# HiromasaYamanishi/furusato_recommend

Measured on AMD Instinct MI355X. Metric: BPR positive-edges/sec (LightGCN-3 d=64, 1000000 x 100000 / 20000000 edges), higher is better.
Workload: dtype f32; 1 GPU; C2: LightGCN 3-layer d=64, synthetic 1000000 users x 100000 items / 20000000 edges (uniform); users=1000000, items=100000, edges=20000000, graph=uniform, dim=64, layers=3, bpr_batch_per_rank=2048, global_batch=2048, ranks=1, parallelism=dp1 (user-sharded, RCCL none gradient exchange)

## Files before the change

### furusato_recommend_amd/_lib.py

```python
from __future__ import annotations

import ctypes
import os
from ctypes import (POINTER, Structure, c_float, c_int, c_int32, c_int64,
                    c_size_t, c_uint64, c_void_p, c_char_p)

import torch

_HERE = os.path.dirname(os.path.abspath(__file__))
LIB_PATH = os.environ.get("MIREC_LIB") or os.path.join(_HERE, "libmirec.so")

MIREC_OK = 0
ERR_WORKSPACE = 4
IN_PRESCALED, IN_RAW, IN_SPARSE, IN_NONE = 0, 1, 2, 3
SUPPORTED_DIMS = (4, 8, 16, 32, 64, 128, 256)


class MirecError(RuntimeError):
    pass


class CSR(Structure):
    _fields_ = [
        ("rowptr", c_void_p), ("col", c_void_p), ("dinv", c_void_p),
        ("n_rows", c_int64), ("nnz", c_int64), ("split", c_int32),
        ("_pad", c_int32), ("n_long", c_int64), ("n_seg", c_int64),
        ("long_rows", c_void_p), ("long_segptr", c_void_p),
        ("seg_row", c_void_p), ("seg_beg", c_void_p),
        ("col_sorted", c_void_p), ("n_sorted", c_int64), ("val", c_void_p),
    ]


class AdamH(Structure):
    _fields_ = [
        ("one_minus_beta1", c_float), ("beta2", c_float),
        ("one_minus_beta2", c_float), ("neg_step_size", c_float),
        ("bc2_sqrt", c_float), ("eps", c_float),
    ]


class Prop(Structure):
    _fields_ = [
        ("dim", c_int32), ("in_mode", c_int32), ("x_in", c_void_p),
        ("slot", c_void_p), ("seed_in", c_void_p), ("seed", c_void_p),
        ("addend", c_void_p), ("seed2", c_void_p), ("divisor", c_float),
        ("_pad", c_float), ("out", c_void_p), ("xs_out", c_void_p),
        ("param", c_void_p), ("exp_avg", c_void_p), ("exp_avg_sq", c_void_p),
        ("adam", AdamH), ("partial", c_void_p), ("row_mask", c_void_p),
        ("in_mask", c_void_p), ("out_mask", c_void_p), ("row_list", c_void_p),
        ("row_count", c_void_p),
        ("row_list_cap", c_int64), ("narrow_max", c_int32), ("_pad2", c_int32),
        ("wide_list", c_void_p), ("wide_count", c_void_p),
        ("scale_src", c_void_p), ("scale_dst", c_void_p), ("scale_next", c_void_p),
    ]


class Drop(Structure):
    _fields_ = [("keep_prob", c_float), ("transposed", c_int32), ("seed", c_uint64)]


class Sweep(Structure):
    _fields_ = [
        ("row0", c_int64), ("n_rows", c_int64), ("n_src", c_int64),
        ("tile_rows", c_int32), ("group_rows", c_int32), ("groups", c_int32),
        ("n_tiles", c_int32), ("band_rows", c_int32), ("_pad", c_int32),
        ("gptr", c_void_p), ("ent", c_void_p),
    ]


class SweepWave(Structure):
    _fields_ = [
        ("row0", c_int64), ("n_rows", c_int64), ("src0", c_int64), ("n_src", c_int64),
        ("n_slots", c_int64),
        ("tile_rows", c_int32), ("wave_rows", c_int32), ("n_tiles", c_int32),
        ("band_rows", c_int32), ("grid", c_int32), ("_pad", c_int32),
        ("wptr", c_void_p), ("slot", c_void_p),
    ]


class SweepPace(Structure):
    _fields_ = [("ws", c_void_p), ("lead_bands", c_int32 * 2), ("every", c_int32 * 2),
                ("nap", c_int32 * 2)]


class RowGradGroup(Structure):
    _fields_ = [
        ("ids", c_void_p), ("grad_out", c_void_p), ("n_targets", c_int64), ("k", c_int32),
        ("mean", c_int32), ("dropout_p", c_float), ("_pad", c_int32), ("seed", c_uint64),
    ]


TABLE_GRAD_MAX_GROUPS = 8


class RowBlock(Structure):
    _fields_ = [("ids", c_void_p), ("rows", c_void_p), ("n", c_int64)]

SIGNATURES = {
    "mirec_strerror": (c_char_p, [c_int]),
    "mirec_abi_version": (c_int, []),
    "mirec_last_hip_error": (c_int, []),
    "mirec_struct_sizes": (c_int, [POINTER(c_size_t), POINTER(c_size_t), POINTER(c_size_t)]),
    "mirec_csr_bipartite": (c_int, [c_void_p, c_void_p, c_int64, c_int64, c_int64,
                                    c_void_p, c_void_p, c_void_p]),
    "mirec_csr_sort_rows": (c_int, [c_void_p, c_void_p, c_int64, c_void_p]),
    "mirec_csr_from_coo": (c_int, [c_void_p, c_void_p, c_int64, c_int64, c_void_p,
                                   c_void_p, c_void_p]),
    "mirec_csr_entry_order": (c_int, [c_void_p, c_int64, c_int64, c_void_p]),
    "mirec_parse_interactions": (c_int, [c_void_p, c_int64, c_int64, c_int32, POINTER(c_int64),
                                         POINTER(c_int64), POINTER(c_int64), POINTER(c_int64),
                                         c_void_p, c_void_p, c_void_p]),
    "mirec_csr_long_rows": (c_int, [c_void_p, c_int64, c_int32, POINTER(c_int64),
                                    POINTER(c_int64), c_void_p, c_void_p, c_void_p,
                                    c_void_p]),
    "mirec_propagate": (c_int, [POINTER(CSR), POINTER(Prop), c_void_p]),
    "mirec_propagate_sweep": (c_int, [POINTER(CSR), POINTER(Prop), POINTER(Sweep), c_void_p]),
    "mirec_sweep_sizeof": (c_size_t, []),
    "mirec_sweep_shape": (c_int, [c_int64, c_int32, c_int32, POINTER(c_int32),
                                  POINTER(c_int32)]),
    "mirec_sweep_build": (c_int, [c_void_p, c_void_p, c_int64, c_int64, c_int64, c_int32,
                                  c_int32, c_void_p, c_void_p]),
    "mirec_sweep_groups": (c_int, [c_int32]),
    "mirec_sweep_wave_sizeof": (c_size_t, []),
    "mirec_sweep_wave_build": (c_int, [c_void_p, c_void_p, c_int64, c_int64, c_int64, c_int64,
                                       c_int32, c_void_p, c_void_p, c_int64, POINTER(c_int64)]),
    "mirec_propagate_sweep_wave": (c_int, [POINTER(CSR), POINTER(Prop), POINTER(SweepWave),
                                           POINTER(SweepWave), c_void_p]),
    "mirec_sweep_pace_sizeof": (c_size_t, []),
    "mirec_sweep_pace_ws_bytes": (c_size_t, []),
    "mirec_propagate_sweep_wave_paced": (c_int, [POINTER(CSR), POINTER(Prop), POINTER(SweepWave),
                                                 POINTER(SweepWave), POINTER(SweepPace),
                                                 c_void_p]),
    "mirec_sweep_wave_stamp": (c_int, [POINTER(CSR), POINTER(Prop), POINTER(SweepWave), c_void_p,
                                       c_int64, c_void_p, c_void_p]),
    "mirec_drop_sizeof": (c_size_t, []),
    "mirec_propagate_drop": (c_int, [POINTER(CSR), POINTER(Prop), POINTER(Drop), c_void_p]),
    "mirec_edge_keep_mask": (c_int, [c_void_p, c_void_p, c_int64, c_uint64, c_float, c_int32,
                                     c_void_p]),
    "mirec_edge_dot": (c_int, [POINTER(CSR), c_void_p, c_void_p, c_int32, c_void_p, c_void_p]),
    "mirec_prescale": (c_int, [c_void_p, c_void_p, c_int64, c_int32, c_void_p, c_void_p]),
    "mirec_shard_pack": (c_int, [c_void_p, c_int64, c_int32, c_int32, c_int32, c_int64, c_int64,
                                 c_void_p, c_void_p]),
    "mirec_shard_unpack": (c_int, [c_void_p, c_int64, c_int32, c_int32, c_int32, c_int64,
                                   c_int64, c_void_p, c_void_p, c_void_p, c_void_p]),
    "mirec_frontier": (c_int, [POINTER(CSR), c_void_p, c_int64, c_void_p, c_void_p, c_void_p,
                               c_int64, c_int64, c_void_p, c_void_p, c_void_p, c_void_p,
                               c_void_p, c_int32, c_void_p]),
    "mirec_mask_compact_pair": (c_int, [c_void_p, c_void_p, c_void_p, c_int64, c_void_p, c_void_p,
                                        c_void_p, c_void_p, c_void_p, c_void_p]),
    "mirec_small_sort_workspace": (c_int, [c_int64, POINTER(c_size_t)]),
    "mirec_small_sort_pairs": (c_int, [c_void_p, c_void_p, c_void_p, c_void_p, c_int64, c_void_p,
                                       c_size_t, c_void_p]),
    "mirec_mask_compact": (c_int, [POINTER(CSR), c_void_p, c_int32, c_void_p, c_void_p,
                                   c_void_p, c_void_p, c_int32, c_void_p]),
    "mirec_distinct_rows_workspace": (c_int64, [c_int64]),
    "mirec_distinct_rows": (c_int, [c_void_p, c_int64, c_int64, c_int64, c_int64, c_void_p,
                                    c_void_p, c_void_p, c_size_t, c_void_p]),
    "mirec_distinct_rows_unseen": (c_int, [c_void_p, c_int64, c_int64, c_int64, c_int64, c_void_p,
                                        c_void_p, c_void_p, c_void_p, c_size_t, c_void_p]),
    "mirec_stamped_rows": (c_int, [c_void_p, c_int64, c_int32, c_int32, c_void_p, c_void_p,
                                   c_void_p, c_size_t, c_void_p]),
    "mirec_scatter_rows": (c_int, [c_void_p, c_void_p, c_int64, c_int32, c_void_p, c_void_p]),
    "mirec_owner_sum_workspace": (c_int64, [c_int32, c_int64]),
    "mirec_owner_sum": (c_int, [POINTER(RowBlock), c_int32, c_int64, c_int64, c_int32, c_void_p,
                                c_size_t, c_void_p, c_void_p]),
    "mirec_gather_rows_counted": (c_int, [c_void_p, c_void_p, c_void_p, c_int64, c_int32,
                                          c_void_p, c_void_p]),
    "mirec_route_pack": (c_int, [c_void_p, c_void_p, c_int64, c_int64, c_int32, c_int32, c_int64,
                                 c_void_p, c_void_p]),
    "mirec_gather_rows_routed": (c_int, [c_void_p, c_int64, c_void_p, c_int32, c_int32, c_int64,
                                         c_int32, c_void_p, c_void_p]),
    "mirec_bpr_forward": (c_int, [c_void_p, c_void_p, c_int64, c_int64, c_int32, c_int64,
                                  c_void_p, c_void_p, c_void_p, c_float, c_void_p, c_void_p,
                                  c_void_p, c_void_p, c_void_p, c_void_p]),
    "mirec_bpr_loss": (c_int, [c_void_p, c_void_p, c_int64, c_float, c_void_p, c_void_p,
                               c_void_p]),
    "mirec_bpr_seed_workspace": (c_int, [c_int64, c_int64, POINTER(c_size_t)]),
    "mirec_bpr_seed": (c_int, [c_void_p, c_void_p, c_int64, c_int64, c_int32, c_int64,
                               c_void_p, c_void_p, c_void_p, c_void_p, c_void_p, c_void_p,
                               c_float, c_float, c_int32, c_void_p, c_void_p, c_void_p,
                               c_void_p, c_void_p, c_size_t, c_void_p]),
    "mirec_bpr_seed_reset": (c_int, [c_void_p, c_void_p, c_int64, c_void_p]),
    "mirec_seed_dense": (c_int, [c_void_p, c_void_p, c_int64, c_void_p, c_void_p, c_void_p,
                                 c_int32, c_void_p, c_int32, c_void_p]),
    "mirec_seed_pack": (c_int, [c_void_p, c_int64, c_int64, c_void_p, c_void_p]),
    "mirec_seed_merge_workspace": (c_int, [c_int64, c_int64, POINTER(c_size_t)]),
    "mirec_seed_merge": (c_int, [c_void_p, c_void_p, c_void_p, c_int64, c_int32, c_int64,
                                 c_void_p, c_void_p, c_void_p, c_void_p, c_void_p, c_size_t,
                                 c_void_p]),
    "mirec_ssm_forward": (c_int, [c_void_p, c_void_p, c_int64, c_int64, c_int32, c_int64, c_int32,
                                  c_void_p, c_void_p, c_void_p, c_float, c_float, c_void_p,
                                  c_void_p, c_void_p, c_void_p, c_void_p, c_void_p, c_void_p,
                                  c_void_p]),
    "mirec_ssm_keys": (c_int, [c_void_p, c_void_p, c_void_p, c_int64, c_int32, c_int64, c_void_p,
                               c_void_p]),
    "mirec_ssm_seed_workspace": (c_int, [c_int64, c_int32, c_int64, POINTER(c_size_t)]),
    "mirec_ssm_seed": (c_int, [c_void_p, c_void_p, c_int64, c_int64, c_int32, c_int64, c_int32,
                               c_void_p, c_void_p, c_void_p, c_void_p, c_void_p, c_void_p,
                               c_float, c_float, c_int32, c_void_p, c_void_p, c_void_p,
                               c_void_p, c_void_p, c_size_t, c_void_p]),
    "mirec_ssm_sample": (c_int, [POINTER(CSR), c_void_p, c_int64, c_int64, c_int64, c_int32,
                                 c_uint64, c_uint64, c_int32, c_int32, c_void_p, c_void_p,
                                 c_void_p, c_void_p, c_void_p]),
    "mirec_cpu_ssm_sample": (c_int, [c_void_p, c_void_p, c_void_p, c_void_p, c_int64, c_int64,
                                     c_int64, c_int32, c_uint64, c_uint64, c_int32, c_int32,
                                     c_void_p, c_void_p, c_void_p, c_void_p, c_int32]),
    "mirec_ssm_shared_keys": (c_int, [c_void_p, c_void_p, c_void_p, c_int64, c_int64, c_int64,
                                      c_void_p, c_void_p]),
    "mirec_ssm_shared_mask": (c_int, [POINTER(CSR), c_void_p, c_int64, c_void_p, c_void_p,
                                      c_int64, c_int64, c_void_p, c_void_p]),
    "mirec_ssm_shared_forward": (c_int, [c_void_p, c_void_p, c_int64, c_int64, c_int32, c_int64,
                                         c_int64, c_void_p, c_void_p, c_void_p, c_void_p, c_float,
                                         c_float, c_void_p, c_void_p, c_void_p, c_void_p,
                                         c_void_p, c_void_p, c_void_p, c_void_p, c_void_p]),
    "mirec_ssm_shared_loss": (c_int, [c_void_p, c_void_p, c_void_p, c_int64, c_int64, c_float,
                                      c_void_p, c_void_p, c_void_p]),
    "mirec_ssm_shared_seed_workspace": (c_int, [c_int64, c_int64, c_int64, POINTER(c_size_t)]),
    "mirec_ssm_shared_seed": (c_int, [c_void_p, c_void_p, c_int64, c_int64, c_int32, c_int64,
                                      c_int64, c_void_p, c_void_p, c_void_p, c_void_p, c_void_p,
                                      c_float, c_float, c_int32, c_void_p, c_void_p, c_void_p,
                                      c_void_p, c_void_p, c_size_t, c_void_p]),
    "mirec_shared_sample": (c_int, [c_int64, c_int64, c_int64, c_uint64, c_uint64, c_void_p,
                                    c_void_p]),
    "mirec_cpu_shared_sample": (c_int, [c_int64, c_int64, c_int64, c_uint64, c_uint64, c_void_p,
                                        c_int32]),
    "mirec_adam_multi": (c_int, [c_int32, c_void_p, c_void_p, c_void_p, c_void_p, c_void_p,
                                 POINTER(AdamH), c_void_p]),
    "mirec_adam_dense": (c_int, [c_void_p, c_void_p, c_void_p, c_void_p, c_int64,
                                 POINTER(AdamH), c_void_p]),
    "mirec_adam_multi_dev": (c_int, [c_int32, c_void_p, c_void_p, c_void_p, c_void_p, c_void_p,
                                     c_void_p, c_void_p]),
    "mirec_adam_dense_dev": (c_int, [c_void_p, c_void_p, c_void_p, c_void_p, c_int64, c_void_p,
                                     c_void_p]),
    "mirec_sample_fanout": (c_int, [POINTER(CSR), c_void_p, c_int64, c_int32, c_uint64,
                                    c_uint64, c_void_p, c_void_p]),
    "mirec_pack_seed_nodes": (c_int, [c_void_p, c_void_p, c_void_p, c_int64, c_int64, c_void_p,
                                      c_void_p]),
    "mirec_sample_fanout_norep": (c_int, [POINTER(CSR), c_void_p, c_int64, c_int32, c_uint64,
                                          c_uint64, c_void_p, c_void_p]),
    "mirec_gather_rows": (c_int, [c_void_p, c_void_p, c_int64, c_int32, c_void_p, c_void_p]),
    "mirec_scatter_add_rows": (c_int, [c_void_p, c_void_p, c_int64, c_int32, c_void_p,
                                       c_void_p]),
    "mirec_fanout_mean": (c_int, [c_void_p, c_void_p, c_int64, c_int32, c_int32, c_float,
                                  c_uint64, c_void_p, c_void_p]),
    "mirec_fanout_mean_bwd": (c_int, [c_void_p, c_void_p, c_int64, c_int32, c_int32, c_float,
                                      c_uint64, c_void_p, c_void_p]),
    "mirec_fanout_mean_gather": (c_int, [c_void_p, c_void_p, c_int64, c_int32, c_int32,
                                         c_float, c_uint64, c_void_p, c_void_p]),
    "mirec_fanout_mean_gather_bwd": (c_int, [c_void_p, c_void_p, c_int64, c_int32, c_int32,
                                             c_float, c_uint64, c_void_p, c_void_p]),
    "mirec_fanout_mean_gather_bwd_sorted_workspace": (c_int, [c_int64, c_int32, c_int32,
                                                              POINTER(c_size_t)]),
    "mirec_fanout_mean_gather_bwd_sorted": (c_int, [c_void_p, c_void_p, c_int64, c_int32, c_int32,
                                                    c_float, c_uint64, c_int32, c_void_p,
                                                    c_void_p, c_size_t, c_void_p]),
    "mirec_fanout_gat": (c_int, [c_void_p, c_void_p, c_void_p, c_void_p, c_void_p, c_void_p,
                                 c_int64, c_int32, c_int32, c_int32, c_float, c_void_p, c_void_p,
                                 c_void_p]),
    "mirec_fanout_gat_bwd_work_floats": (c_int64, [c_int64, c_int32, c_int32, c_int32]),
    "mirec_fanout_gat_bwd": (c_int, [c_void_p, c_void_p, c_void_p, c_void_p, c_void_p, c_void_p,
                                     c_void_p, c_int64, c_int32, c_int32, c_int32, c_float,
                                     c_void_p, c_void_p, c_void_p, c_void_p, c_void_p, c_void_p]),
    "mirec_csr_gat": (c_int, [POINTER(CSR), c_void_p, c_void_p, c_void_p, c_void_p, c_int32,
                              c_int32, c_float, c_void_p, c_void_p, c_void_p]),
    "mirec_fanout_tattn": (c_int, [c_void_p, c_void_p, c_int64, c_void_p, c_void_p, c_int64,
                                   c_void_p, c_int64, c_int32, c_int32, c_int32, c_float,
                                   c_void_p, c_void_p, c_void_p]),
    "mirec_fanout_tattn_bwd": (c_int, [c_void_p, c_void_p, c_int64, c_void_p, c_void_p, c_int64,
                                       c_void_p, c_void_p, c_int64, c_int32, c_int32, c_int32,
                                       c_float, c_void_p, c_void_p, c_int64, c_void_p, c_void_p,
                                       c_int64, c_void_p]),
    "mirec_csr_tattn": (c_int, [POINTER(CSR), c_void_p, c_void_p, c_int64, c_void_p, c_void_p,
                                c_int64, c_int32, c_int32, c_float, c_void_p, c_void_p]),
    "mirec_row_grad_group_size": (c_int64, []),
    "mirec_table_grad_workspace": (c_int, [POINTER(RowGradGroup), c_int32, c_int32, c_int32,
                                           POINTER(c_size_t)]),
    "mirec_table_grad_sorted": (c_int, [POINTER(RowGradGroup), c_int32, c_int32, c_int32,
                                        c_void_p, c_void_p, c_int32, c_void_p, c_size_t,
                                        c_void_p]),
    "mirec_table_grad_sorted_rows": (c_int, [POINTER(RowGradGroup), c_int32, c_int32, c_int32,
                                             c_int32, c_void_p, c_void_p, c_void_p, c_void_p,
                                             c_size_t, c_void_p]),
    "mirec_table_grad_atomic": (c_int, [c_void_p, c_int32, c_int32, c_int32, c_void_p, c_void_p,
                                        c_int32, c_void_p]),
    "mirec_table_grad_dense": (c_int, [c_void_p, c_void_p, c_int64, c_void_p, c_void_p, c_int32,
                                       c_int64, c_int32, c_void_p, c_void_p]),
    "mirec_adam_table_sumsq_floats": (c_int64, [c_int64, c_int32]),
    "mirec_owner_adam": (c_int, [POINTER(RowBlock), c_int32, c_int64, c_int64, c_int32, c_void_p,
                                 c_void_p, c_void_p, c_void_p, c_int64, POINTER(AdamH), c_void_p,
                                 c_void_p, c_void_p, c_size_t, c_void_p]),
    "mirec_adam_table": (c_int, [c_void_p, c_void_p, c_void_p, c_void_p, c_int64, c_void_p,
                                 c_void_p, c_int32, c_int64, c_int32, POINTER(AdamH), c_void_p,
                                 c_void_p, c_void_p]),
    "mirec_adam_table_dev": (c_int, [c_void_p, c_void_p, c_void_p, c_void_p, c_int64, c_void_p,
                                     c_void_p, c_int32, c_int64, c_int32, c_void_p, c_void_p,
                                     c_void_p, c_void_p]),
    "mirec_norm_coef": (c_int, [c_void_p, c_int32, c_void_p, c_int32, c_int32, c_void_p,
                                c_void_p]),
    "mirec_attention_fwd": (c_int, [c_void_p, c_int64, c_int32, c_int32, c_int32, c_void_p,
                                    c_void_p]),
# ... 3 lines not shown
                                           c_void_p, c_void_p]),
    "mirec_attention_varlen_bwd": (c_int, [c_void_p, c_void_p, c_void_p, c_int64, c_int32,
                                           c_int32, c_void_p, c_void_p]),
    "mirec_attention_bucketed_fwd": (c_int, [c_void_p, c_void_p, c_void_p, c_int32, c_int32,
                                             c_void_p, c_void_p]),
    "mirec_attention_bucketed_bwd": (c_int, [c_void_p, c_void_p, c_void_p, c_void_p, c_int32,
                                             c_int32, c_void_p, c_void_p]),
    "mirec_attention_wave_supported": (c_int, [c_int32]),
    "mirec_attention_ordered_fwd": (c_int, [c_void_p, c_void_p, c_void_p, c_int64, c_int32,
                                            c_int32, c_void_p, c_void_p]),
    "mirec_attention_ordered_bwd": (c_int, [c_void_p, c_void_p, c_void_p, c_void_p, c_int64,
                                            c_int32, c_int32, c_void_p, c_void_p]),
    "mirec_attention_length_order": (c_int, [c_void_p, c_int64, c_void_p, c_void_p, c_void_p,
                                             c_int64, c_int32, c_void_p]),
    "mirec_attention_packed_bwd": (c_int, [c_void_p, c_void_p, c_void_p, c_void_p, c_int64,
                                           c_int32, c_int32, c_void_p, c_int64, c_void_p]),
    "mirec_attention_packed_bwd_lse": (c_int, [c_void_p, c_void_p, c_void_p, c_void_p,
                                               c_void_p, c_int64, c_int32, c_int32, c_void_p,
                                               c_int64, c_void_p]),
    "mirec_attention_wave_fwd": (c_int, [c_void_p, c_void_p, c_void_p, c_int64, c_int32, c_int32,
                                         c_int32, c_void_p, c_void_p, c_int64, c_void_p]),
    "mirec_attention_wave_bwd": (c_int, [c_void_p, c_void_p, c_void_p, c_void_p, c_void_p,
                                         c_void_p, c_int64, c_int32, c_int32, c_int32, c_void_p,
                                         c_void_p, c_void_p]),
    "mirec_resnorm_fwd": (c_int, [c_void_p, c_void_p, c_void_p, c_void_p, c_void_p, c_int64,
                                  c_int32, c_int32, c_float, c_uint64, c_void_p, c_float,
                                  c_void_p, c_void_p, c_void_p, c_void_p, c_void_p]),
    "mirec_gemm_resnorm": (c_int, [c_void_p, c_void_p, c_int64, c_int32, c_int32, c_void_p,
                                   c_void_p, c_void_p, c_void_p, c_int32, c_float, c_uint64,
                                   c_void_p, c_float, c_void_p, c_void_p, c_void_p, c_void_p,
                                   c_void_p]),
    "mirec_gemm_nn_resnorm_bwd_work_floats": (c_int64, [c_int64, c_int32]),
    "mirec_gemm_nn_resnorm_bwd": (c_int, [c_void_p, c_void_p, c_int64, c_int32, c_int32,
                                          c_void_p, c_void_p, c_void_p, c_void_p, c_void_p,
                                          c_int32, c_float, c_uint64, c_void_p, c_void_p,
                                          c_void_p, c_void_p, c_void_p, c_void_p, c_void_p,
                                          c_void_p]),
    "mirec_resnorm_reduce_partials": (c_int, [c_void_p, c_int64, c_int32, c_void_p, c_void_p,
                                              c_void_p, c_void_p]),
    "mirec_resnorm_work_floats": (c_int64, [c_int64, c_int32]),
    "mirec_segment_mean": (c_int, [c_void_p, c_void_p, c_void_p, c_int64, c_int32, c_void_p,
                                   c_void_p]),
    "mirec_segment_mean_bwd": (c_int, [c_void_p, c_void_p, c_void_p, c_int64, c_int64, c_int32,
                                       c_void_p, c_void_p]),
    "mirec_bpr_rows_loss": (c_int, [c_void_p, c_void_p, c_void_p, c_int64, c_int32, c_void_p,
                                    c_float, c_void_p, c_void_p, c_void_p]),
    "mirec_bpr_rows_loss_bwd": (c_int, [c_void_p, c_void_p, c_void_p, c_void_p, c_int64, c_int32,
                                        c_void_p, c_float, c_void_p, c_void_p, c_void_p, c_void_p,
                                        c_void_p]),
    "mirec_slice_norms_work_floats": (c_int64, []),
    "mirec_slice_norms": (c_int, [c_void_p, c_int64, c_int64, c_void_p, c_void_p, c_void_p]),
    "mirec_norm_terms": (c_int, [c_void_p, c_void_p, c_void_p, c_int32, c_void_p, c_void_p,
                                 c_int32, c_void_p, c_void_p, c_void_p]),
    "mirec_norm_terms_bwd": (c_int, [c_void_p, c_void_p, c_void_p, c_void_p, c_int32, c_void_p,
                                     c_void_p, c_void_p, c_int32, c_void_p, c_void_p]),
    "mirec_norm_terms_bwd_acc": (c_int, [c_void_p, c_void_p, c_void_p, c_void_p, c_int32,
                                         c_void_p, c_void_p, c_void_p]),
    "mirec_seq_sample": (c_int, [c_void_p, c_int64, c_void_p, c_int32, c_void_p, c_int64,
                                 c_uint64, c_uint64, c_void_p, c_void_p]),
    "mirec_seq_pack": (c_int, [c_void_p, c_int64, c_void_p, c_int32, c_void_p, c_void_p,
                               c_void_p, c_int64, c_void_p, c_void_p, c_void_p, c_void_p,
                               c_void_p]),
    "mirec_zero_tail_rows": (c_int, [c_void_p, c_void_p, c_int64, c_int64, c_int32, c_void_p]),
    "mirec_gemm_nt": (c_int, [c_void_p, c_void_p, c_void_p, c_void_p, c_int64, c_int32, c_int32,
                              c_void_p]),
    "mirec_gemm_nn_ex": (c_int, [c_void_p, c_void_p, c_void_p, c_void_p, c_void_p, c_int32,
                                 c_int64, c_int32, c_int32, c_void_p]),
    "mirec_gemm_nt_ex": (c_int, [c_void_p, c_void_p, c_int32, c_void_p, c_void_p, c_void_p,
                                 c_void_p, c_void_p, c_int32, c_int32, c_int64, c_int32, c_int32,
                                 c_void_p]),
    "mirec_gemm_tn_ex": (c_int, [c_void_p, c_void_p, c_void_p, c_void_p, c_int32, c_void_p,
                                 c_void_p, c_int64, c_int32, c_int32, c_void_p, c_void_p]),
    "mirec_gemm_tn_work_floats": (c_int64, [c_int64, c_int32, c_int32]),
    "mirec_col_sums_work_floats": (c_int64, [c_int64, c_int32]),
    "mirec_col_sums": (c_int, [c_void_p, c_int64, c_int32, c_void_p, c_void_p, c_void_p]),
    "mirec_gemm_tn": (c_int, [c_void_p, c_void_p, c_void_p, c_void_p, c_int64, c_int32, c_int32,
                              c_void_p, c_void_p]),
    "mirec_resnorm_bwd": (c_int, [c_void_p, c_void_p, c_void_p, c_void_p, c_void_p, c_void_p,
                                  c_int64, c_int32, c_int32, c_float, c_uint64, c_void_p,
                                  c_void_p, c_void_p, c_void_p, c_void_p, c_void_p, c_void_p,
                                  c_void_p]),
    "mirec_score_topk_workspace": (c_int64, [c_int64, c_int64, c_int32]),
    "mirec_score_topk": (c_int, [c_void_p, c_int64, c_void_p, c_int64, c_int32, c_void_p,
                                 c_void_p, c_int64, c_int32, c_void_p, c_void_p, c_void_p,
                                 c_size_t, c_void_p]),
    "mirec_score_rank_workspace": (c_int64, [c_int64, c_int64, c_int64, c_int32]),
    "mirec_score_rank": (c_int, [c_void_p, c_int64, c_void_p, c_int64, c_int32, c_void_p,
                                 c_void_p, c_void_p, c_void_p, c_int64, c_void_p, c_void_p,
                                 c_void_p, c_void_p, c_void_p, c_void_p, c_size_t, c_void_p]),
    "mirec_topk_masked": (c_int, [c_void_p, c_int64, c_int64, c_void_p, c_void_p, c_int64,
                                  c_int32, c_void_p, c_void_p, c_void_p]),
    "mirec_bpr_sample_capped_workspace": (c_int, [c_int64, c_int64, POINTER(c_size_t)]),
    "mirec_bpr_sample_capped": (c_int, [POINTER(CSR), c_int64, c_int64, c_int64, c_int32,
                                        c_uint64, c_uint64, c_int32, c_int32, c_void_p,
                                        c_void_p, c_void_p, c_void_p, c_void_p, c_void_p,
                                        c_void_p, c_void_p, c_size_t, c_void_p]),
    "mirec_bpr_sample": (c_int, [POINTER(CSR), c_int64, c_int64, c_int64, c_uint64,
                                 c_uint64, c_int32, c_int32, c_void_p, c_void_p, c_void_p,
                                 c_void_p, c_void_p]),
    "mirec_bpr_sample_ex": (c_int, [POINTER(CSR), c_void_p, c_int64, c_int64, c_int64, c_uint64,
                                    c_uint64, c_int32, c_int32, c_void_p, c_void_p, c_void_p,
                                    c_void_p, c_void_p]),
    "mirec_bpr_sample_capped_ex": (c_int, [POINTER(CSR), c_void_p, c_int64, c_int64, c_int64,
                                           c_int32, c_uint64, c_uint64, c_int32, c_int32, c_void_p,
                                           c_void_p, c_void_p, c_void_p, c_void_p, c_void_p,
                                           c_void_p, c_void_p, c_size_t, c_void_p]),
    "mirec_pos_cdf_build": (c_int, [c_void_p, c_int64, c_void_p, c_void_p]),
    "mirec_cpu_bpr_sample": (c_int, [c_void_p, c_void_p, c_void_p, c_void_p, c_int64, c_int64,
                                     c_int64, c_uint64, c_uint64, c_int32, c_int32, c_void_p,
                                     c_void_p, c_void_p, c_void_p, c_int32]),
    "mirec_cpu_bpr_sample_capped": (c_int, [c_void_p, c_void_p, c_void_p, c_void_p, c_int64,
                                            c_int64, c_int64, c_int32, c_uint64, c_uint64,
                                            c_int32, c_int32, c_void_p, c_void_p, c_void_p,
                                            c_void_p, c_void_p, c_void_p, c_void_p, c_int32]),
    "mirec_cpu_bpr_step": (c_int, [c_void_p, c_void_p, c_void_p, c_void_p, c_int64, c_int32,
                                   c_int64, c_void_p, c_void_p, c_void_p, c_int64, c_float,
                                   c_void_p, c_void_p, c_int32]),
    "mirec_cpu_bpr_grad": (c_int, [c_void_p, c_void_p, c_int64, c_int32, c_int64, c_void_p,
                                   c_void_p, c_void_p, c_int64, c_float, c_float, c_void_p,
                                   c_int32]),
    "mirec_cpu_adam": (c_int, [c_void_p, c_void_p, c_void_p, c_void_p, c_int64, c_void_p,
                               c_int32]),
}


def _load():
    if not os.path.exists(LIB_PATH):
        raise ImportError(
            f"{LIB_PATH} not found: the HIP engine is not built. Run "
            "`make -C furusato_recommend_amd/csrc` (or __graft_entry__.build()). "
            "There is no CPU fallback.")
    lib = ctypes.CDLL(LIB_PATH)
    for name, (res, args) in SIGNATURES.items():
        fn = getattr(lib, name)
        fn.restype = res
        fn.argtypes = args
    if lib.mirec_abi_version() != 1:
        raise ImportError("libmirec.so ABI version mismatch")
    sizes = [c_size_t(0) for _ in range(3)]
    lib.mirec_struct_sizes(*(ctypes.byref(x) for x in sizes))
    want = (ctypes.sizeof(CSR), ctypes.sizeof(Prop), ctypes.sizeof(AdamH))
    if tuple(x.value for x in sizes) != want:
        raise ImportError(f"struct layout mismatch: lib {[x.value for x in sizes]} vs {want}")
    if lib.mirec_row_grad_group_size() != ctypes.sizeof(RowGradGroup):
        raise ImportError("struct layout mismatch: mirec_row_grad_group_t")
    if lib.mirec_drop_sizeof() != ctypes.sizeof(Drop):
        raise ImportError("struct layout mismatch: mirec_drop_t")
    if lib.mirec_sweep_sizeof() != ctypes.sizeof(Sweep):
        raise ImportError("struct layout mismatch: mirec_sweep_t")
    if lib.mirec_sweep_wave_sizeof() != ctypes.sizeof(SweepWave):
        raise ImportError("struct layout mismatch: mirec_sweep_wave_t")
    if lib.mirec_sweep_pace_sizeof() != ctypes.sizeof(SweepPace):
        raise ImportError("struct layout mismatch: mirec_sweep_pace_t")
    return lib


lib = _load()


def check(rc: int, what: str = "") -> None:
    if rc != MIREC_OK:
        msg = lib.mirec_strerror(rc).decode()
        if rc == 3:
            msg += f" (hipError {lib.mirec_last_hip_error()})"
        raise MirecError(f"{what}: {msg}")


def ptr(t) -> int | None:
    return None if t is None else t.data_ptr()


def stream_handle(device=None) -> int:
    if device is None:
        return _raw_stream(_cur_device())
    return torch.cuda.current_stream(device).cuda_stream


_raw_stream = torch._C._cuda_getCurrentRawStream
_cur_device = torch._C._cuda_getDevice


def adam_hparams(lr: float, beta1: float, beta2: float, eps: float, step: int) -> AdamH:
    bc1 = 1 - beta1 ** step
    bc2 = 1 - beta2 ** step
    return AdamH(one_minus_beta1=1 - beta1, beta2=beta2, one_minus_beta2=1 - beta2,
                 neg_step_size=-(lr / bc1), bc2_sqrt=bc2 ** 0.5, eps=eps)
```

### furusato_recommend_amd/csrc/common.h

```cpp
#pragma once

#include <hip/hip_runtime.h>
#include <stdint.h>

#include "mirec.h"

namespace mirec {

extern thread_local int g_last_hip_error;

#define MIREC_CHECK_ARG(cond)                                                  \
  do {                                                                         \
    if (!(cond)) return MIREC_ERR_ARG;                                         \
  } while (0)

#define MIREC_LAUNCH_CHECK()                                                   \
  do {                                                                         \
    hipError_t e_ = hipGetLastError();                                         \
    if (e_ != hipSuccess) {                                                    \
      ::mirec::g_last_hip_error = (int)e_;                                     \
      return MIREC_ERR_HIP;                                                    \
    }                                                                          \
  } while (0)

#define MIREC_HIP(call)                                                        \
  do {                                                                         \
    hipError_t e_ = (call);                                                    \
    if (e_ != hipSuccess) {                                                    \
      ::mirec::g_last_hip_error = (int)e_;                                     \
      return MIREC_ERR_HIP;                                                    \
    }                                                                          \
  } while (0)

inline bool dim_supported(int d) {
  return d == 4 || d == 8 || d == 16 || d == 32 || d == 64 || d == 128 ||
         d == 256;
}

__device__ __forceinline__ float4 f4_zero() { return make_float4(0.f, 0.f, 0.f, 0.f); }

__device__ __forceinline__ float4 f4_add(float4 a, float4 b) {
  return make_float4(a.x + b.x, a.y + b.y, a.z + b.z, a.w + b.w);
}
__device__ __forceinline__ float4 f4_sub(float4 a, float4 b) {
  return make_float4(a.x - b.x, a.y - b.y, a.z - b.z, a.w - b.w);
}
__device__ __forceinline__ float4 f4_scale(float s, float4 a) {
  return make_float4(s * a.x, s * a.y, s * a.z, s * a.w);
}
__device__ __forceinline__ float4 f4_fma(float s, float4 a, float4 c) {
  return make_float4(fmaf(s, a.x, c.x), fmaf(s, a.y, c.y), fmaf(s, a.z, c.z),
                     fmaf(s, a.w, c.w));
}
__device__ __forceinline__ float4 f4_div(float4 a, float d) {
  return make_float4(a.x / d, a.y / d, a.z / d, a.w / d);
}
__device__ __forceinline__ float f4_dot(float4 a, float4 b) {
  return a.x * b.x + a.y * b.y + a.z * b.z + a.w * b.w;
}
__device__ __forceinline__ float4 ld4(const float *p) {
  return *reinterpret_cast<const float4 *>(p);
}
__device__ __forceinline__ void st4(float *p, float4 v) {
  *reinterpret_cast<float4 *>(p) = v;
}
constexpr int kRowRounds = 4;
inline int row_lg(int64_t d4) {
  int lg = 0;
  while ((int64_t(1) << lg) < d4) ++lg;
  return lg;
}
inline int64_t row_blocks(int64_t n, int lg) {
  const int64_t per = int64_t(256 >> lg) * kRowRounds;
  return (n + per - 1) / per;
}

__device__ __forceinline__ float4 f4_shfl_xor(float4 v, int m) {
  return make_float4(__shfl_xor(v.x, m), __shfl_xor(v.y, m),
                     __shfl_xor(v.z, m), __shfl_xor(v.w, m));
}

template <int LPR>
__device__ __forceinline__ float group_sum(float v) {
#pragma unroll
  for (int m = 1; m < LPR; m <<= 1) v += __shfl_xor(v, m);
  return v;
}

constexpr float kLog2e = 1.4426950408889634f;
__device__ __forceinline__ float exp2_hw(float x) { return __builtin_amdgcn_exp2f(x); }
__device__ __forceinline__ float log2_hw(float x) { return __builtin_amdgcn_logf(x); }

#if defined(__HIP_DEVICE_COMPILE__)
#define MIREC_NO_PK_F32 __attribute__((target("no-packed-fp32-ops")))
#else
#define MIREC_NO_PK_F32
#endif

__host__ __device__ __forceinline__ uint64_t mix64(uint64_t x) {
  x += 0x9E3779B97F4A7C15ull;
  x = (x ^ (x >> 30)) * 0xBF58476D1CE4E5B9ull;
  x = (x ^ (x >> 27)) * 0x94D049BB133111EBull;
  return x ^ (x >> 31);
}

__host__ __device__ __forceinline__ uint64_t edge_drop_key(uint64_t seed) {
  return mix64(seed ^ 0xD6E8FEB86659FD93ull);
}

__host__ __device__ __forceinline__ bool edge_keep(uint64_t key, uint32_t dst, uint32_t src,
                                                   uint32_t thresh_m1) {
  const uint64_t h = mix64(key ^ (((uint64_t)dst << 32) | (uint64_t)src));
  return (uint32_t)(h >> 32) <= thresh_m1;
}

static inline bool edge_drop_thresh(float keep_prob, uint32_t *thresh_m1) {
  if (!(keep_prob > 0.f && keep_prob <= 1.f)) return false;
  uint64_t t = (uint64_t)((double)keep_prob * 4294967296.0);
  if (t < 1) t = 1;
  if (t > 4294967296ull) t = 4294967296ull;
  *thresh_m1 = (uint32_t)(t - 1);
  return true;
}

__device__ __forceinline__ bool keep(uint64_t key, uint64_t idx, uint32_t thresh) {
  const uint64_t h = mix64(key + (idx >> 2));
  return (uint32_t)((h >> (16 * (idx & 3))) & 0xffffu) >= thresh;
}

__device__ __forceinline__ float4 drop4_hq(float4 v, uint64_t hq, uint32_t thresh, float scale) {
  const uint64_t h = mix64(hq);
  v.x = (uint32_t)(h & 0xffffu) >= thresh ? v.x * scale : 0.f;
  v.y = (uint32_t)((h >> 16) & 0xffffu) >= thresh ? v.y * scale : 0.f;
  v.z = (uint32_t)((h >> 32) & 0xffffu) >= thresh ? v.z * scale : 0.f;
  v.w = (uint32_t)(h >> 48) >= thresh ? v.w * scale : 0.f;
  return v;
}

__device__ __forceinline__ float4 drop4(float4 v, uint64_t key, uint64_t idx, uint32_t thresh,
                                        float scale) {
  return drop4_hq(v, key + (idx >> 2), thresh, scale);
}

__device__ __forceinline__ uint64_t run_key(uint64_t key, const uint64_t *key_base) {
  return key_base ? mix64(key ^ *key_base) : key;
}

static inline bool dropout_params(float p, uint64_t seed, uint64_t *key, uint32_t *thresh, float *scale) {
  if (!(p >= 0.f && p < 1.f)) return false;
  *key = mix64(seed ^ 0xA24BAED4963EE407ull);
  *thresh = (uint32_t)((double)p * 65536.0 + 0.5);
  *scale = p > 0.f ? 1.f / (1.f - p) : 1.f;
  if (p > 0.f && *thresh == 0u) *thresh = 1u;
  if (*thresh > 65535u) *thresh = 65535u;
  return true;
}

__device__ __forceinline__ void adam1(float &p, float &m, float &v, float g,
                                      const mirec_adam_hparams_t &h) {
  m = fmaf(h.one_minus_beta1, g - m, m);
  v = fmaf(v, h.beta2, h.one_minus_beta2 * (g * g));
  const float denom = sqrtf(v) / h.bc2_sqrt + h.eps;
  p = fmaf(h.neg_step_size, m / denom, p);
}

typedef __bf16 bf16x8 __attribute__((ext_vector_type(8)));
typedef __bf16 bf16x2 __attribute__((ext_vector_type(2)));
typedef float f32x2 __attribute__((ext_vector_type(2)));
typedef uint32_t u32x4 __attribute__((ext_vector_type(4)));

struct Split3 {
  bf16x8 h, m, l;
};

__device__ __forceinline__ uint32_t pk_bf16(float a, float b) {
  return __builtin_bit_cast(uint32_t, __builtin_convertvector((f32x2){a, b}, bf16x2));
}

__device__ __forceinline__ Split3 split3(const float (&x)[8]) {
  u32x4 H, M, L;
#pragma unroll
  for (int p = 0; p < 4; ++p) {
    const float a = x[2 * p], b = x[2 * p + 1];
    const uint32_t ph = pk_bf16(a, b);
    const float ra = a - __uint_as_float(ph << 16), rb = b - __uint_as_float(ph & 0xffff0000u);
    const uint32_t pm = pk_bf16(ra, rb);
    const float sa = ra - __uint_as_float(pm << 16), sb = rb - __uint_as_float(pm & 0xffff0000u);
    H[p] = ph;
    M[p] = pm;
    L[p] = pk_bf16(sa, sb);
  }
  return Split3{__builtin_bit_cast(bf16x8, H), __builtin_bit_cast(bf16x8, M),
                __builtin_bit_cast(bf16x8, L)};
}

typedef float f32x16 __attribute__((ext_vector_type(16)));

__device__ __forceinline__ f32x16 mfma_x6(const Split3 &a, const Split3 &b, f32x16 c) {
  c = __builtin_amdgcn_mfma_f32_32x32x16_bf16(a.l, b.h, c, 0, 0, 0);
  c = __builtin_amdgcn_mfma_f32_32x32x16_bf16(a.h, b.l, c, 0, 0, 0);
  c = __builtin_amdgcn_mfma_f32_32x32x16_bf16(a.m, b.m, c, 0, 0, 0);
  c = __builtin_amdgcn_mfma_f32_32x32x16_bf16(a.m, b.h, c, 0, 0, 0);
  c = __builtin_amdgcn_mfma_f32_32x32x16_bf16(a.h, b.m, c, 0, 0, 0);
  c = __builtin_amdgcn_mfma_f32_32x32x16_bf16(a.h, b.h, c, 0, 0, 0);
  return c;
}

__device__ __forceinline__ int x6_k(int h, int e) { return 4 * h + (e & 3) + 8 * (e >> 2); }

}
```

### furusato_recommend_amd/csrc/frontier.hip

```cpp
#include <algorithm>

#include "common.h"

namespace mirec {

constexpr int kWaves = 4;

__device__ __forceinline__ bool test_and_set(uint8_t *bm, int64_t i) {
  const uint32_t b = 1u << (8 * (i & 3));
  return (atomicOr(reinterpret_cast<uint32_t *>(bm) + (i >> 2), b) & b) == 0u;
}

__device__ __forceinline__ int32_t block_reserve(int c, int32_t *count) {
  __shared__ int wsum[kWaves];
  __shared__ int base;
  const int lane = threadIdx.x & 63, wid = threadIdx.x >> 6;
  __syncthreads();
  int incl = c;
#pragma unroll
  for (int d = 1; d < 64; d <<= 1) {
    const int t = __shfl_up(incl, d);
    if (lane >= d) incl += t;
  }
  if (lane == 63) wsum[wid] = incl;
  __syncthreads();
  if (threadIdx.x == 0) {
    int t = 0;
#pragma unroll
    for (int k = 0; k < kWaves; ++k) t += wsum[k];
    base = t > 0 ? atomicAdd(count, t) : 0;
  }
  __syncthreads();
  int off = base + incl - c;
  for (int k = 0; k < wid; ++k) off += wsum[k];
  return off;
}

__device__ __forceinline__ int64_t key_node(int64_t i, const int32_t *keys, int64_t n_keys,
                                            const int32_t *users, const int32_t *pos,
                                            const int32_t *neg, int64_t batch, int64_t n_users) {
  if (keys != nullptr) return i < n_keys ? (int64_t)keys[i] : -1;
  if (i >= 3 * batch) return -1;
  return i < batch ? (int64_t)users[i]
                   : (i < 2 * batch ? n_users + pos[i - batch] : n_users + neg[i - 2 * batch]);
}

__global__ __launch_bounds__(256) void frontier_self_kernel(
    int64_t n_rows, const int32_t *__restrict__ keys, int64_t n_keys,
    const int32_t *__restrict__ users, const int32_t *__restrict__ pos,
    const int32_t *__restrict__ neg, int64_t batch, int64_t n_users, uint8_t *bm_self,
    uint8_t *bm_hop, int32_t *self_list, int32_t *self_count) {
  const int64_t i = (int64_t)blockIdx.x * blockDim.x + threadIdx.x;
  const int64_t node = key_node(i, keys, n_keys, users, pos, neg, batch, n_users);
  const bool valid = node >= 0 && node < n_rows;
  const bool first = valid && test_and_set(bm_self, node);
  if (valid) bm_hop[node] = 1;
  const int32_t off = block_reserve(first ? 1 : 0, self_count);
  if (first) self_list[off] = (int32_t)node;
}

__global__ __launch_bounds__(256) void frontier_clear_kernel(uint4 *__restrict__ maps, int64_t n16,
                                                             int32_t *__restrict__ self_count,
                                                             int32_t *__restrict__ zero,
                                                             int32_t n_zero) {
  const int64_t i = (int64_t)blockIdx.x * blockDim.x + threadIdx.x;
  for (int64_t j = i; j < n16; j += (int64_t)gridDim.x * blockDim.x) maps[j] = make_uint4(0, 0, 0, 0);
  if (i == 0 && self_count != nullptr) *self_count = 0;
  if (i < n_zero) zero[i] = 0;
}

__global__ __launch_bounds__(256) void frontier_expand_kernel(
    const int64_t *__restrict__ rowptr, const int32_t *__restrict__ col, int32_t split,
    const int32_t *__restrict__ self_list, const int32_t *__restrict__ self_count,
    uint8_t *bm_hop) {
  const int lane = threadIdx.x & 63;
  const int64_t i = (int64_t)blockIdx.x * kWaves + (threadIdx.x >> 6);
  if (i >= *self_count) return;
  const int64_t node = self_list[i];
  const int64_t beg = rowptr[node], end = rowptr[node + 1];
  if (split > 0 && end - beg > split) return;
  for (int64_t e = beg + lane; e < end; e += 64) bm_hop[col[e]] = 1;
}

__global__ __launch_bounds__(256) void frontier_keys_kernel(
    const int64_t *__restrict__ rowptr, const int32_t *__restrict__ col, int64_t n_rows,
    int32_t split, const int32_t *__restrict__ keys, int64_t n_keys,
    const int32_t *__restrict__ users, const int32_t *__restrict__ pos,
    const int32_t *__restrict__ neg, int64_t batch, int64_t n_users, uint8_t *bm_self,
    uint8_t *bm_hop) {
  const int lane = threadIdx.x & 63;
  const int64_t i = (int64_t)blockIdx.x * kWaves + (threadIdx.x >> 6);
  const int64_t node = key_node(i, keys, n_keys, users, pos, neg, batch, n_users);
  if (node < 0 || node >= n_rows) return;
  if (lane == 0) {
    bm_self[node] = 1;
    bm_hop[node] = 1;
  }
  const int64_t beg = rowptr[node], end = rowptr[node + 1];
  if (split > 0 && end - beg > split) return;
  for (int64_t e = beg + lane; e < end; e += 64) bm_hop[col[e]] = 1;
}

__global__ __launch_bounds__(256) void frontier_segments_kernel(
    const int64_t *__restrict__ rowptr, const int32_t *__restrict__ col,
    const int32_t *__restrict__ seg_row, const int64_t *__restrict__ seg_beg, int64_t n_seg,
    int32_t split, const uint8_t *bm_self, uint8_t *bm_hop) {
  const int lane = threadIdx.x & 63;
  const int64_t sg = (int64_t)blockIdx.x * kWaves + (threadIdx.x >> 6);
  if (sg >= n_seg) return;
  const int64_t row = seg_row[sg];
  if (bm_self[row] == 0) return;
  const int64_t beg = seg_beg[sg];
  const int64_t end = min(beg + (int64_t)split, rowptr[row + 1]);
  for (int64_t e = beg + lane; e < end; e += 64) bm_hop[col[e]] = 1;
}

__global__ __launch_bounds__(256) void mask_compact_kernel(
    const uint8_t *__restrict__ bm, const int64_t *__restrict__ rowptr, int64_t n,
    int32_t narrow_max, int32_t *list, int32_t *count, int32_t *wide_list,
    int32_t *wide_count) {
  const int64_t t = (int64_t)blockIdx.x * blockDim.x + threadIdx.x;
  const int64_t b0 = t * 16;
  uint32_t w[4] = {0u, 0u, 0u, 0u};
  if (b0 + 16 <= n) {
    const uint4 v = *reinterpret_cast<const uint4 *>(bm + b0);
    w[0] = v.x; w[1] = v.y; w[2] = v.z; w[3] = v.w;
  } else if (b0 < n) {
    for (int k = 0; b0 + k < n; ++k)
      if (bm[b0 + k]) w[k >> 2] |= 1u << (8 * (k & 3));
  }
  uint32_t set = 0u, wide = 0u;
#pragma unroll
  for (int k = 0; k < 16; ++k) {
    if ((w[k >> 2] >> (8 * (k & 3))) & 0xffu) {
      set |= 1u << k;
      if (wide_list != nullptr && rowptr[b0 + k + 1] - rowptr[b0 + k] > narrow_max)
        wide |= 1u << k;
    }
  }
  const uint32_t narrow = set & ~wide;
  int32_t off = block_reserve(__popc(narrow), count);
  int32_t woff = wide_list != nullptr ? block_reserve(__popc(wide), wide_count) : 0;
#pragma unroll
  for (int k = 0; k < 16; ++k) {
    if ((narrow >> k) & 1u) list[off++] = (int32_t)(b0 + k);
    if ((wide >> k) & 1u) wide_list[woff++] = (int32_t)(b0 + k);
  }
}

__device__ __forceinline__ uint32_t map_bits32(const uint8_t *__restrict__ bm, int64_t b0,
                                               int64_t n) {
  uint32_t set = 0u;
  if (b0 + 32 <= n) {
    const uint4 v0 = *reinterpret_cast<const uint4 *>(bm + b0);
    const uint4 v1 = *reinterpret_cast<const uint4 *>(bm + b0 + 16);
    const uint32_t w[8] = {v0.x, v0.y, v0.z, v0.w, v1.x, v1.y, v1.z, v1.w};
#pragma unroll
    for (int k = 0; k < 32; ++k)
      if ((w[k >> 2] >> (8 * (k & 3))) & 0xffu) set |= 1u << k;
  } else {
    for (int k = 0; b0 + k < n; ++k)
      if (bm[b0 + k]) set |= 1u << k;
  }
  return set;
}

__global__ __launch_bounds__(256) void mask_compact_pair_kernel(
    const uint8_t *__restrict__ bm_a, const uint8_t *__restrict__ bm_b,
    const uint32_t *__restrict__ wide_bits, int64_t n, int32_t *__restrict__ list_a,
    int32_t *__restrict__ wide_a, int32_t *__restrict__ list_b, int32_t *__restrict__ wide_b,
    int32_t *__restrict__ counts) {
  __shared__ int4 wsum[kWaves];
  __shared__ int4 base;
  const int64_t t = (int64_t)blockIdx.x * blockDim.x + threadIdx.x;
  const int64_t b0 = t * 32;
  uint32_t sa = 0u, sb = 0u, wd = 0u;
  if (b0 < n) {
    sa = map_bits32(bm_a, b0, n);
    sb = map_bits32(bm_b, b0, n);
    wd = wide_bits[t];
  }
  const uint32_t na = sa & ~wd, wa = sa & wd, nb = sb & ~wd, wb = sb & wd;
  const int lane = threadIdx.x & 63, wid = threadIdx.x >> 6;
  int4 c = make_int4(__popc(na), __popc(wa), __popc(nb), __popc(wb)), incl = c;
#pragma unroll
  for (int d = 1; d < 64; d <<= 1) {
    const int x = __shfl_up(incl.x, d), y = __shfl_up(incl.y, d);
    const int z = __shfl_up(incl.z, d), w = __shfl_up(incl.w, d);
    if (lane >= d) incl = make_int4(incl.x + x, incl.y + y, incl.z + z, incl.w + w);
  }
  if (lane == 63) wsum[wid] = incl;
  __syncthreads();
  if (threadIdx.x == 0) {
    int4 tot = make_int4(0, 0, 0, 0);
#pragma unroll
    for (int k = 0; k < kWaves; ++k)
      tot = make_int4(tot.x + wsum[k].x, tot.y + wsum[k].y, tot.z + wsum[k].z, tot.w + wsum[k].w);
    base = make_int4(tot.x ? atomicAdd(counts, tot.x) : 0, tot.y ? atomicAdd(counts + 1, tot.y) : 0,
                     tot.z ? atomicAdd(counts + 2, tot.z) : 0,
                     tot.w ? atomicAdd(counts + 3, tot.w) : 0);
  }
  __syncthreads();
  int4 off = make_int4(base.x + incl.x - c.x, base.y + incl.y - c.y, base.z + incl.z - c.z,
                       base.w + incl.w - c.w);
  for (int k = 0; k < wid; ++k)
    off = make_int4(off.x + wsum[k].x, off.y + wsum[k].y, off.z + wsum[k].z, off.w + wsum[k].w);
#pragma unroll 4
  for (int k = 0; k < 32; ++k) {
    const int32_t v = (int32_t)(b0 + k);
    if ((na >> k) & 1u) list_a[off.x++] = v;
    if ((wa >> k) & 1u) wide_a[off.y++] = v;
    if ((nb >> k) & 1u) list_b[off.z++] = v;
    if ((wb >> k) & 1u) wide_b[off.w++] = v;
  }
}

constexpr int kDrBlock = 4096;

__global__ __launch_bounds__(256) void dr_mark_kernel(const int32_t *__restrict__ ids, int64_t n,
                                                      int64_t n_rows, int64_t lo, int64_t hi,
                                                      const uint8_t *__restrict__ have,
                                                      uint8_t *__restrict__ bm) {
  const int64_t i = (int64_t)blockIdx.x * blockDim.x + threadIdx.x;
  if (i >= n) return;
  const int64_t id = ids[i];
  if (id >= 0 && id < n_rows && (id < lo || id >= hi) && (have == nullptr || !have[id]))
    bm[id] = 1;
}

__device__ __forceinline__ uint32_t dr_bits(const uint8_t *__restrict__ bm, int64_t n_rows,
                                            int64_t b0) {
  uint32_t w[4] = {0u, 0u, 0u, 0u};
  if (b0 + 16 <= n_rows) {
    const uint4 v = *reinterpret_cast<const uint4 *>(bm + b0);
    w[0] = v.x; w[1] = v.y; w[2] = v.z; w[3] = v.w;
  } else {
    for (int k = 0; b0 + k < n_rows; ++k)
      if (bm[b0 + k]) w[k >> 2] |= 1u << (8 * (k & 3));
  }
  uint32_t set = 0u;
#pragma unroll
  for (int k = 0; k < 16; ++k)
    if ((w[k >> 2] >> (8 * (k & 3))) & 0xffu) set |= 1u << k;
  return set;
}

__device__ __forceinline__ int dr_block_scan(int c, int *tot) {
  __shared__ int wsum[4];
  const int lane = threadIdx.x & 63, w = threadIdx.x >> 6;
// ... 191 lines not shown
    }
  }
  float4 x[kRowRounds];
#pragma unroll
  for (int k = 0; k < kRowRounds; ++k) x[k] = id[k] >= 0 ? table[(int64_t)id[k] * d4 + c] : f4_zero();
#pragma unroll
  for (int k = 0; k < kRowRounds; ++k)
    if (id[k] != -1) out[(r0 + k * per) * d4 + c] = x[k];
}

}

extern "C" int64_t mirec_distinct_rows_workspace(int64_t n_rows) {
  using namespace mirec;
  if (n_rows < 0) return -1;
  const int64_t map = (n_rows + 15) / 16 * 16;
  const int64_t nb = (n_rows + kDrBlock - 1) / kDrBlock;
  return map + 4 * (nb + 1);
}

extern "C" int mirec_distinct_rows(const int32_t *ids, int64_t n, int64_t n_rows, int64_t lo,
                                   int64_t hi, int32_t *out, int32_t *count, void *workspace,
                                   size_t workspace_bytes, mirec_stream_t stream) {
  return mirec_distinct_rows_unseen(ids, n, n_rows, lo, hi, nullptr, out, count, workspace,
                                 workspace_bytes, stream);
}

extern "C" int mirec_distinct_rows_unseen(const int32_t *ids, int64_t n, int64_t n_rows, int64_t lo,
                                       int64_t hi, uint8_t *have, int32_t *out, int32_t *count,
                                       void *workspace, size_t workspace_bytes,
                                       mirec_stream_t stream) {
  using namespace mirec;
  MIREC_CHECK_ARG(n >= 0 && n_rows >= 0 && out && count && workspace);
  MIREC_CHECK_ARG(n == 0 || ids);
  MIREC_CHECK_ARG(((uintptr_t)workspace & 15u) == 0);
  const int64_t need = mirec_distinct_rows_workspace(n_rows);
  if ((int64_t)workspace_bytes < need) return MIREC_ERR_WORKSPACE;
  hipStream_t st = reinterpret_cast<hipStream_t>(stream);
  uint8_t *bm = static_cast<uint8_t *>(workspace);
  const int64_t map = (n_rows + 15) / 16 * 16;
  int32_t *cnt = reinterpret_cast<int32_t *>(bm + map);
  const int64_t nb = (n_rows + kDrBlock - 1) / kDrBlock;
  if (nb == 0) {
    MIREC_HIP(hipMemsetAsync(count, 0, 4, st));
    return MIREC_OK;
  }
  MIREC_HIP(hipMemsetAsync(bm, 0, (size_t)map, st));
  if (n > 0) {
    hipLaunchKernelGGL(dr_mark_kernel, dim3((unsigned)((n + 255) / 256)), dim3(256), 0, st, ids, n,
                       n_rows, lo, hi, have, bm);
    MIREC_LAUNCH_CHECK();
  }
  hipLaunchKernelGGL(dr_count_kernel, dim3((unsigned)nb), dim3(256), 0, st, bm, n_rows, cnt);
  MIREC_LAUNCH_CHECK();
  hipLaunchKernelGGL(dr_scan_kernel, dim3(1), dim3(256), 0, st, cnt, nb, count);
  MIREC_LAUNCH_CHECK();
  hipLaunchKernelGGL(dr_write_kernel, dim3((unsigned)nb), dim3(256), 0, st, bm, n_rows, cnt, out,
                     have);
  MIREC_LAUNCH_CHECK();
  return MIREC_OK;
}

extern "C" int mirec_stamped_rows(const int32_t *stamp, int64_t n_rows, int32_t gen,
                                  int32_t parts, int32_t *rows, int32_t *counts, void *workspace,
                                  size_t workspace_bytes, mirec_stream_t stream) {
  using namespace mirec;
  MIREC_CHECK_ARG(n_rows >= 0 && parts >= 1 && rows && counts && workspace);
  MIREC_CHECK_ARG(n_rows == 0 || stamp);
  MIREC_CHECK_ARG(((uintptr_t)workspace & 15u) == 0);
  const int64_t need = mirec_distinct_rows_workspace(n_rows);
  if ((int64_t)workspace_bytes < need) return MIREC_ERR_WORKSPACE;
  hipStream_t st = reinterpret_cast<hipStream_t>(stream);
  const int64_t nb = (n_rows + kDrBlock - 1) / kDrBlock;
  if (nb == 0) {
    MIREC_HIP(hipMemsetAsync(counts, 0, 4 * (size_t)(1 + parts), st));
    return MIREC_OK;
  }
  uint8_t *bm = static_cast<uint8_t *>(workspace);
  int32_t *cnt = reinterpret_cast<int32_t *>(bm + (n_rows + 15) / 16 * 16);
  hipLaunchKernelGGL(sr_mark_kernel, dim3((unsigned)((n_rows + 255) / 256)), dim3(256), 0, st,
                     stamp, n_rows, gen, bm);
  MIREC_LAUNCH_CHECK();
  hipLaunchKernelGGL(dr_count_kernel, dim3((unsigned)nb), dim3(256), 0, st, bm, n_rows, cnt);
  MIREC_LAUNCH_CHECK();
  hipLaunchKernelGGL(dr_scan_kernel, dim3(1), dim3(256), 0, st, cnt, nb, counts);
  MIREC_LAUNCH_CHECK();
  hipLaunchKernelGGL(dr_write_kernel, dim3((unsigned)nb), dim3(256), 0, st, bm, n_rows, cnt, rows,
                     nullptr);
  MIREC_LAUNCH_CHECK();
  hipLaunchKernelGGL(sr_parts_kernel, dim3(1), dim3(256), 0, st, rows, n_rows, parts, counts);
  MIREC_LAUNCH_CHECK();
  return MIREC_OK;
}

extern "C" int mirec_gather_rows_counted(const float *src, const int32_t *rows,
                                         const int32_t *count, int64_t capacity, int32_t dim,
                                         float *out, mirec_stream_t stream) {
  using namespace mirec;
  MIREC_CHECK_ARG(capacity >= 0 && dim > 0 && dim % 4 == 0 && count);
  MIREC_CHECK_ARG(capacity == 0 || (src && rows && out));
  MIREC_CHECK_ARG(((uintptr_t)src & 15u) == 0 && ((uintptr_t)out & 15u) == 0);
  if (capacity == 0) return MIREC_OK;
  hipStream_t st = reinterpret_cast<hipStream_t>(stream);
  const int lg = row_lg(dim / 4);
  MIREC_CHECK_ARG(lg <= 8);
  hipLaunchKernelGGL(gather_counted_kernel, dim3((unsigned)row_blocks(capacity, lg)), dim3(256), 0,
                     st, reinterpret_cast<const float4 *>(src), rows, count, dim / 4, lg,
                     reinterpret_cast<float4 *>(out));
  MIREC_LAUNCH_CHECK();
  return MIREC_OK;
}

extern "C" int mirec_route_pack(const int32_t *ids, const int32_t *count, int64_t capacity,
                                int64_t n_rows, int32_t parts, int32_t cap, int64_t stride,
                                int32_t *blocks, mirec_stream_t stream) {
  using namespace mirec;
  MIREC_CHECK_ARG(count && blocks && capacity >= 0 && n_rows >= 0 && cap >= 0);
  MIREC_CHECK_ARG(capacity == 0 || ids);
  MIREC_CHECK_ARG(parts >= 1 && parts <= kRouteMaxParts && stride >= (int64_t)cap + 1);
  MIREC_CHECK_ARG(n_rows >= parts);
  hipStream_t st = reinterpret_cast<hipStream_t>(stream);
  const int64_t nb = std::min<int64_t>(std::max<int64_t>((capacity + 255) / 256, 1), 4096);
  hipLaunchKernelGGL(rp_pack_kernel, dim3((unsigned)nb), dim3(256), 0, st, ids, count, n_rows,
                     parts, cap, stride, blocks);
  MIREC_LAUNCH_CHECK();
  return MIREC_OK;
}

extern "C" int mirec_gather_rows_routed(const float *table, int64_t n_rows, const int32_t *blocks,
                                        int32_t parts, int32_t cap, int64_t stride, int32_t dim,
                                        float *out, mirec_stream_t stream) {
  using namespace mirec;
  MIREC_CHECK_ARG(table && blocks && out && n_rows >= 0 && cap >= 0 && dim > 0 && dim % 4 == 0);
  MIREC_CHECK_ARG(parts >= 1 && parts <= kRouteMaxParts && stride >= (int64_t)cap + 1);
  MIREC_CHECK_ARG(((uintptr_t)table & 15u) == 0 && ((uintptr_t)out & 15u) == 0);
  const int64_t slots = (int64_t)parts * cap;
  if (slots == 0) return MIREC_OK;
  hipStream_t st = reinterpret_cast<hipStream_t>(stream);
  const int lg = row_lg(dim / 4);
  MIREC_CHECK_ARG(lg <= 8);
  hipLaunchKernelGGL(rp_gather_kernel, dim3((unsigned)row_blocks(slots, lg)), dim3(256), 0, st,
                     reinterpret_cast<const float4 *>(table), n_rows, blocks, parts, cap, stride,
                     dim / 4, lg, reinterpret_cast<float4 *>(out));
  MIREC_LAUNCH_CHECK();
  return MIREC_OK;
}

extern "C" int mirec_frontier(const mirec_csr_t *c, const int32_t *keys, int64_t n_keys,
                              const int32_t *users, const int32_t *pos, const int32_t *neg,
                              int64_t batch, int64_t n_users, uint8_t *bm_self,
                              uint8_t *bm_hop, int32_t *self_list, int32_t *self_count,
                              int32_t *zero_counts, int32_t n_zero_counts,
                              mirec_stream_t stream) {
  using namespace mirec;
  MIREC_CHECK_ARG(c && c->rowptr && c->col && bm_self && bm_hop);
  MIREC_CHECK_ARG(keys != nullptr || (users && pos && neg && batch >= 0 && n_users >= 0));
  MIREC_CHECK_ARG(self_list == nullptr || self_count != nullptr);
  MIREC_CHECK_ARG(n_zero_counts >= 0 && n_zero_counts <= 256 &&
                  (n_zero_counts == 0 || zero_counts != nullptr));
  hipStream_t st = reinterpret_cast<hipStream_t>(stream);
  const size_t bytes = (size_t)((c->n_rows + 3) / 4) * 4;
  const size_t bytes16 = (bytes + 15) / 16 * 16;
  int32_t *sc = self_list != nullptr ? self_count : nullptr;
  if (bm_hop == bm_self + bytes16 && ((uintptr_t)bm_self & 15u) == 0) {
    const int64_t n16 = (int64_t)(2 * bytes16 / 16);
    const unsigned blocks = (unsigned)std::max<int64_t>(1, std::min<int64_t>((n16 + 255) / 256, 1024));
    hipLaunchKernelGGL(frontier_clear_kernel, dim3(blocks), dim3(256), 0, st,
                       reinterpret_cast<uint4 *>(bm_self), n16, sc, zero_counts, n_zero_counts);
    MIREC_LAUNCH_CHECK();
  } else {
    MIREC_HIP(hipMemsetAsync(bm_self, 0, bytes, st));
    MIREC_HIP(hipMemsetAsync(bm_hop, 0, bytes, st));
    if (sc != nullptr) MIREC_HIP(hipMemsetAsync(sc, 0, 4, st));
    if (n_zero_counts > 0) MIREC_HIP(hipMemsetAsync(zero_counts, 0, 4 * (size_t)n_zero_counts, st));
  }
  const int64_t n = keys != nullptr ? n_keys : 3 * batch;
  const int32_t split = c->n_seg > 0 ? c->split : 0;
  if (self_list != nullptr) {
    if (n > 0) {
      hipLaunchKernelGGL(frontier_self_kernel, dim3((n + 255) / 256), dim3(256), 0, st, c->n_rows,
                         keys, n_keys, users, pos, neg, batch, n_users, bm_self, bm_hop,
                         self_list, self_count);
      MIREC_LAUNCH_CHECK();
      hipLaunchKernelGGL(frontier_expand_kernel, dim3((n + kWaves - 1) / kWaves), dim3(256), 0,
                         st, c->rowptr, c->col, split, self_list, self_count, bm_hop);
      MIREC_LAUNCH_CHECK();
    }
  } else if (n > 0) {
    hipLaunchKernelGGL(frontier_keys_kernel, dim3((n + kWaves - 1) / kWaves), dim3(256), 0, st,
                       c->rowptr, c->col, c->n_rows, split, keys, n_keys, users, pos, neg, batch,
                       n_users, bm_self, bm_hop);
    MIREC_LAUNCH_CHECK();
  }
  if (c->n_seg > 0 && n > 0) {
    hipLaunchKernelGGL(frontier_segments_kernel, dim3((c->n_seg + kWaves - 1) / kWaves), dim3(256),
                       0, st, c->rowptr, c->col, c->seg_row, c->seg_beg, c->n_seg, c->split,
                       bm_self, bm_hop);
    MIREC_LAUNCH_CHECK();
  }
  return MIREC_OK;
}

extern "C" int mirec_mask_compact(const mirec_csr_t *c, const uint8_t *bm, int32_t narrow_max,
                                  int32_t *list, int32_t *count, int32_t *wide_list,
                                  int32_t *wide_count, int32_t counts_zeroed,
                                  mirec_stream_t stream) {
  using namespace mirec;
  MIREC_CHECK_ARG(c && c->rowptr && bm && list && count && c->n_rows >= 0);
  MIREC_CHECK_ARG(wide_list == nullptr || wide_count != nullptr);
  MIREC_CHECK_ARG(((uintptr_t)bm & 15u) == 0);
  hipStream_t st = reinterpret_cast<hipStream_t>(stream);
  if (counts_zeroed) {
  } else if (wide_count == count + 1) {
    MIREC_HIP(hipMemsetAsync(count, 0, 8, st));
  } else {
    MIREC_HIP(hipMemsetAsync(count, 0, 4, st));
    if (wide_count != nullptr) MIREC_HIP(hipMemsetAsync(wide_count, 0, 4, st));
  }
  const int64_t threads = (c->n_rows + 15) / 16;
  if (threads > 0) {
    hipLaunchKernelGGL(mask_compact_kernel, dim3((threads + 255) / 256), dim3(256), 0, st, bm,
                       c->rowptr, c->n_rows, narrow_max, list, count, wide_list, wide_count);
    MIREC_LAUNCH_CHECK();
  }
  return MIREC_OK;
}

extern "C" int mirec_mask_compact_pair(const uint8_t *bm_a, const uint8_t *bm_b,
                                       const uint32_t *wide_bits, int64_t n_rows,
                                       int32_t *list_a, int32_t *wide_a, int32_t *list_b,
                                       int32_t *wide_b, int32_t *counts, mirec_stream_t stream) {
  using namespace mirec;
  MIREC_CHECK_ARG(bm_a && bm_b && wide_bits && list_a && wide_a && list_b && wide_b && counts &&
                  n_rows >= 0);
  MIREC_CHECK_ARG((((uintptr_t)bm_a | (uintptr_t)bm_b) & 15u) == 0);
  const int64_t threads = (n_rows + 31) / 32;
  if (threads == 0) return MIREC_OK;
  hipLaunchKernelGGL(mask_compact_pair_kernel, dim3((unsigned)((threads + 255) / 256)), dim3(256),
                     0, reinterpret_cast<hipStream_t>(stream), bm_a, bm_b, wide_bits, n_rows,
                     list_a, wide_a, list_b, wide_b, counts);
  MIREC_LAUNCH_CHECK();
  return MIREC_OK;
}

extern "C" int mirec_scatter_rows(const float *src, const int32_t *ids, int64_t n, int32_t dim,
                                  float *dst, mirec_stream_t stream) {
  using namespace mirec;
  MIREC_CHECK_ARG(n >= 0 && dim > 0 && dim % 4 == 0);
  if (n == 0) return MIREC_OK;
  MIREC_CHECK_ARG(src && ids && dst);
  MIREC_CHECK_ARG(((uintptr_t)src & 15u) == 0 && ((uintptr_t)dst & 15u) == 0);
  const int lg = row_lg(dim / 4);
  MIREC_CHECK_ARG(lg <= 8);
  hipLaunchKernelGGL(scatter_rows_kernel, dim3((unsigned)row_blocks(n, lg)), dim3(256), 0,
                     reinterpret_cast<hipStream_t>(stream), reinterpret_cast<const float4 *>(src),
                     ids, n, dim / 4, lg, reinterpret_cast<float4 *>(dst));
  MIREC_LAUNCH_CHECK();
  return MIREC_OK;
}
```

### furusato_recommend_amd/csrc/prop.hip

```cpp
#include "common.h"

namespace mirec {

struct PropK {
  const int64_t *rowptr;
  const int32_t *col;
  const float *dinv;
  int64_t n_rows;
  int64_t n_seg;
  const int32_t *seg_row;
  const int64_t *seg_beg;
  int32_t split;
  const float *x_in;
  const int32_t *slot;
  const float *seed_in;
  const float *seed;
  const float *addend;
  const float *seed2;
  float divisor;
  float *out;
  float *xs_out;
  float *param;
  float *m;
  float *v;
// ... 142 lines not shown
    adam1(p.x, m.x, v.x, o.x, a.adam);
    adam1(p.y, m.y, v.y, o.y, a.adam);
    adam1(p.z, m.z, v.z, o.z, a.adam);
    adam1(p.w, m.w, v.w, o.w, a.adam);
    st4(a.param + off, p);
    st4(a.m + off, m);
    st4(a.v + off, v);
    if (a.out != nullptr) st4(a.out + off, o);
    if (a.xs_out != nullptr) st4(a.xs_out + off, f4_scale(dn, p));
  } else {
    st4(a.out + off, o);
  }
}

constexpr int kWavesPerBlock = 4;

template <int D, int UNROLL, int MODE, bool MASKED, bool ROWMASK, bool WEIGHTED, bool SCALED,
          bool DROPOUT>
__device__ __forceinline__ void prop_work(const PropK &a, int64_t w, int64_t nrows,
                                          int64_t row_waves) {
  constexpr int LPR = D / 4;
  constexpr int G = 64 / LPR;
  constexpr int NARROW_UNROLL = UNROLL < 4 ? 4 : UNROLL;
  const int lane = threadIdx.x & 63;
  const int sub = lane % LPR;
  const int grp = lane / LPR;
  if (w < row_waves) {
    const int64_t idx = w * G + grp;
    bool have = idx < nrows;
    int32_t row = 0;
    if (have) row = (ROWMASK && a.row_list != nullptr) ? a.row_list[idx] : (int32_t)idx;
    if (ROWMASK && have) have = bit_set(a.row_mask, row);
    int64_t beg = 0, end = 0;
    if (have) {
      beg = a.rowptr[row];
      end = a.rowptr[row + 1];
      if (a.split > 0 && end - beg > a.split) {
        have = false;
        beg = end = 0;
      }
    }
    const int64_t deg = have ? end - beg : 0;
    if (G > 1 && __ballot(deg > a.narrow_max) == 0ull) {
      float4 s = gather<D, NARROW_UNROLL, MODE, MASKED, WEIGHTED, true, SCALED, DROPOUT>(
          a, beg, end, lane, row);
      if (have) row_epilogue<D, SCALED>(a, row, s, sub);
      return;
    }
#pragma unroll 1
    for (int g = 0; g < G; ++g) {
      const int src = g * LPR;
      if (!__shfl((int)have, src)) continue;
      const int32_t r = __shfl(row, src);
      const int64_t rb = __shfl((long long)beg, src);
      const int64_t re = __shfl((long long)end, src);
      float4 s =
          gather<D, UNROLL, MODE, MASKED, WEIGHTED, false, SCALED, DROPOUT>(a, rb, re, lane, r);
      s = combine_groups<D>(s);
      if (lane < LPR) row_epilogue<D, SCALED>(a, r, s, sub);
    }
  } else {
    const int64_t sg = w - row_waves;
    if (sg >= a.n_seg) return;
    const int64_t row = a.seg_row[sg];
    if (ROWMASK && !bit_set(a.row_mask, row)) return;
    const int64_t beg = a.seg_beg[sg];
    const int64_t end = min(beg + (int64_t)a.split, a.rowptr[row + 1]);
    float4 s =
        gather<D, UNROLL, MODE, MASKED, WEIGHTED, false, SCALED, DROPOUT>(a, beg, end, lane,
                                                                          (int32_t)row);
    s = combine_groups<D>(s);
    if (lane < LPR) st4(a.partial + sg * D + sub * 4, s);
  }
}

template <int D, int UNROLL, int MODE, bool MASKED, bool WEIGHTED, bool SCALED, bool DROPOUT>
__device__ __forceinline__ void block_row(const PropK &a, int32_t row) {
  constexpr int LPR = D / 4;
  __shared__ float4 red[kWavesPerBlock - 1][LPR];
  const int lane = threadIdx.x & 63;
  const int wid = threadIdx.x >> 6;
  const int sub = lane % LPR;
  const int64_t beg = a.rowptr[row], end = a.rowptr[row + 1];
  if (a.split > 0 && end - beg > a.split) return;
  const int64_t q = (end - beg + kWavesPerBlock - 1) / kWavesPerBlock;
  const int64_t wb = min(beg + wid * q, end), we = min(wb + q, end);
  float4 s =
      gather<D, UNROLL, MODE, MASKED, WEIGHTED, false, SCALED, DROPOUT>(a, wb, we, lane, row);
  s = combine_groups<D>(s);
  if (wid > 0 && lane < LPR) red[wid - 1][sub] = s;
  __syncthreads();
  if (wid == 0 && lane < LPR) {
#pragma unroll
    for (int k = 0; k < kWavesPerBlock - 1; ++k) s = f4_add(s, red[k][sub]);
    row_epilogue<D, SCALED>(a, row, s, sub);
  }
  __syncthreads();
}

template <int D, int UNROLL, int MODE, bool MASKED, bool WEIGHTED, bool SCALED, bool DROPOUT>
__device__ __forceinline__ void wave_row(const PropK &a, int32_t row) {
  constexpr int LPR = D / 4;
  const int lane = threadIdx.x & 63;
  const int64_t beg = a.rowptr[row], end = a.rowptr[row + 1];
  if (a.split > 0 && end - beg > a.split) return;
  float4 s =
      gather<D, UNROLL, MODE, MASKED, WEIGHTED, false, SCALED, DROPOUT>(a, beg, end, lane, row);
  s = combine_groups<D>(s);
  if (lane < LPR) row_epilogue<D, SCALED>(a, row, s, lane % LPR);
}

constexpr int64_t kListBlocks = 8192;

template <int D, int UNROLL, int MODE_W, bool MASKED, bool ROWMASK>
__global__ __launch_bounds__(256) __attribute__((amdgpu_waves_per_eu(7, 8)))
MIREC_NO_PK_F32 void prop_kernel(PropK a) {
  constexpr int MODE = MODE_W & 3;
  constexpr bool WEIGHTED = (MODE_W & kWeighted) != 0;
  constexpr bool SCALED = (MODE_W & kScaled) != 0;
  constexpr bool DROPOUT = (MODE_W & kDropout) != 0;
  constexpr int G = 64 / (D / 4);
  const int wid = __builtin_amdgcn_readfirstlane(threadIdx.x >> 6);
  if (!ROWMASK || a.row_list == nullptr) {
    prop_work<D, UNROLL, MODE, MASKED, ROWMASK, WEIGHTED, SCALED, DROPOUT>(
        a, (int64_t)blockIdx.x * kWavesPerBlock + wid, a.n_rows, a.row_waves);
    return;
  }
  constexpr int WPB = (MODE == MIREC_IN_SPARSE) ? kWavesPerBlock : 1;
  const int64_t n_wide = a.wide_list != nullptr ? (int64_t)*a.wide_count : 0;
  const int64_t wide_blocks = (n_wide + WPB - 1) / WPB;
  const int64_t nrows = *a.row_count;
  const int64_t row_waves = (nrows + G - 1) / G;
  const int64_t waves = row_waves + a.n_seg;
  const int64_t total = wide_blocks + (waves + kWavesPerBlock - 1) / kWavesPerBlock;
#pragma unroll 1
  for (int64_t b = blockIdx.x; b < total; b += gridDim.x) {
    if (b < wide_blocks) {
      if constexpr (WPB == 1) {
        block_row<D, UNROLL, MODE, MASKED, WEIGHTED, SCALED, DROPOUT>(a, a.wide_list[b]);
      } else {
        const int64_t i = b * WPB + wid;
        if (i < n_wide)
          wave_row<D, UNROLL, MODE, MASKED, WEIGHTED, SCALED, DROPOUT>(a, a.wide_list[i]);
      }
    } else {
      const int64_t w = (b - wide_blocks) * kWavesPerBlock + wid;
      if (w < waves)
        prop_work<D, UNROLL, MODE, MASKED, ROWMASK, WEIGHTED, SCALED, DROPOUT>(a, w, nrows,
                                                                               row_waves);
    }
  }
}

template <int D, bool SCALED>
__global__ __launch_bounds__(256) MIREC_NO_PK_F32 void prop_finalize(PropK a, const int32_t *long_rows,
                                                     const int64_t *long_segptr, int64_t n_long) {
  constexpr int LPR = D / 4;
  constexpr int NG = 256 / LPR;
  constexpr int kF = 4;
  __shared__ float4 red[NG][LPR];
  const int sub = threadIdx.x % LPR, grp = threadIdx.x / LPR;
  const int64_t li = blockIdx.x;
  if (li >= n_long) return;
  const int64_t row = long_rows[li];
  if (a.row_mask != nullptr && !bit_set(a.row_mask, row)) return;
  const int64_t s0 = long_segptr[li], s1 = long_segptr[li + 1];
  float4 s = f4_zero();
  for (int64_t sg = s0 + grp; sg < s1; sg += (int64_t)kF * NG) {
    float4 x[kF];
#pragma unroll
    for (int u = 0; u < kF; ++u) {
      const int64_t q = sg + (int64_t)u * NG;
      x[u] = q < s1 ? ld4(a.partial + q * D + sub * 4) : f4_zero();
    }
#pragma unroll
    for (int u = 0; u < kF; ++u)
      if (sg + (int64_t)u * NG < s1) s = f4_add(s, x[u]);
  }
  red[grp][sub] = s;
  __syncthreads();
  if (grp != 0) return;
  float4 t = red[0][sub];
#pragma unroll
  for (int k = 1; k < NG; ++k) t = f4_add(t, red[k][sub]);
  row_epilogue<D, SCALED>(a, row, t, sub);
}

constexpr int kSweepThreads = 512;
constexpr int kSweepLdsMax = 64 * 1024;

struct SweepK {
  const int64_t *gptr;
  const long long *ent;
  int64_t row0;
  int64_t n_rows;
  int32_t tile_rows;
  int32_t group_rows;
  int32_t groups;
  int32_t band_rows;
  int32_t n_bands;
};

template <int D, int U, bool SCALED>
__device__ __forceinline__ void sweep_work(const PropK &a, const SweepK &s) {
  constexpr int LPR = D / 4;
  static_assert(LPR % U == 0 && LPR <= 64, "a chunk of LPR entries is U-row batches");
  extern __shared__ float4 sweep_acc[];
  const int lane = threadIdx.x & 63;
  const int sub = threadIdx.x % LPR;
  const int grp = threadIdx.x / LPR;
  const int gbase = (lane / LPR) * LPR;
  const int64_t tile_row0 = (int64_t)blockIdx.x * s.tile_rows;
  const int tile_len = (int)min((int64_t)s.tile_rows, s.n_rows - tile_row0);
  const bool active = grp < s.groups;
  const int lr0 = active ? min(grp * s.group_rows, tile_len) : 0;
  const int lr1 = active ? min(lr0 + s.group_rows, tile_len) : 0;
  for (int lr = lr0; lr < lr1; ++lr) sweep_acc[lr * LPR + sub] = f4_zero();
  int64_t pos = 0, end = 0;
  if (active) {
    const int64_t sidx = (int64_t)blockIdx.x * s.groups + grp;
    pos = s.gptr[sidx];
    end = s.gptr[sidx + 1];
  }
  constexpr long long kNone = 0x7fffffffll;
  const int64_t last = max(end - 1, (int64_t)0);
  long long cur = __builtin_nontemporal_load(s.ent + min(pos + sub, last));
  if (pos + sub >= end) cur = kNone;
  int band = 0;
  int64_t hi = s.band_rows;
  float4 pv[U];
  int pr[U];
#pragma unroll
  for (int u = 0; u < U; ++u) {
    pv[u] = f4_zero();
    pr[u] = -1;
  }
  int n_chunks = (int)((end - pos + LPR - 1) / LPR);
#pragma unroll
  for (int m = LPR; m < 64; m <<= 1) n_chunks = max(n_chunks, __shfl_xor(n_chunks, m));
  n_chunks = __builtin_amdgcn_readfirstlane(n_chunks);
#pragma unroll 1
  for (int c = 0; c < n_chunks; ++c) {
    long long nxt = __builtin_nontemporal_load(s.ent + min(pos + LPR + sub, last));
    if (pos + LPR + sub >= end) nxt = kNone;
    const int ccol = (int)(cur & 0xffffffffll);
    const int crow = (int)(cur >> 32);
#pragma unroll
    for (int k = 0; k < LPR; k += U) {
      const int nc = __shfl(ccol, gbase + k);
      while (band + 1 < s.n_bands && __ballot((int64_t)nc < hi) == 0ull) {
        __builtin_amdgcn_s_barrier();
        ++band;
        hi += s.band_rows;
      }
      float4 v[U];
      int r[U];
#pragma unroll
      for (int u = 0; u < U; ++u) {
        const int j = __shfl(ccol, gbase + k + u);
        const int rr = __shfl(crow, gbase + k + u);
        const bool ok = pos + k + u < end;
        r[u] = ok ? rr : -1;
        v[u] = ld4(a.x_in + (int64_t)(ok ? j : 0) * D + sub * 4);
      }
#pragma unroll
      for (int u = 0; u < U; ++u) {
        if (pr[u] >= 0) {
          float4 *p = &sweep_acc[pr[u] * LPR + sub];
          *p = f4_add(*p, pv[u]);
        }
      }
#pragma unroll
      for (int u = 0; u < U; ++u) {
        pv[u] = v[u];
        pr[u] = r[u];
      }
    }
    pos += LPR;
    cur = nxt;
  }
  while (band + 1 < s.n_bands) {
    __builtin_amdgcn_s_barrier();
    ++band;
  }
#pragma unroll
  for (int u = 0; u < U; ++u) {
    if (pr[u] >= 0) {
      float4 *p = &sweep_acc[pr[u] * LPR + sub];
      *p = f4_add(*p, pv[u]);
    }
  }
  for (int lr = lr0; lr < lr1; ++lr)
    row_epilogue<D, SCALED>(a, s.row0 + tile_row0 + lr, sweep_acc[lr * LPR + sub], sub);
}

template <int D, int U, bool SCALED>
__global__ __launch_bounds__(kSweepThreads) __attribute__((amdgpu_waves_per_eu(4, 4)))
MIREC_NO_PK_F32 void prop_sweep_kernel(PropK a, SweepK s) {
  sweep_work<D, U, SCALED>(a, s);
}

struct SweepWaveK {
  const int64_t *wptr;
  const long long *slot;
  int64_t n_slots;
  int64_t row0;
// ... 119 lines not shown
          pace();
          __builtin_amdgcn_s_barrier();
          ++band;
          hi += s.band_rows;
          stamp(band);
        }
        float4 v[U];
        int r[U];
#pragma unroll
        for (int u = 0; u < U; ++u) {
          const int src = k * U * G + u * G + g;
          const int j = __shfl(ccol, src);
          r[u] = __shfl(crow, src);
          v[u] = ld4(a.x_in + (int64_t)j * D + sub * 4);
        }
#pragma unroll
        for (int u = 0; u < U; ++u) {
          if (pr[u] >= 0) {
            float4 *p = &sweep_acc[pr[u] * LPR + sub];
            *p = f4_add(*p, pv[u]);
          }
        }
#pragma unroll
        for (int u = 0; u < U; ++u) {
          pv[u] = v[u];
          pr[u] = r[u];
        }
      }
      pos += 64;
      cur = nxt;
    }
    while (band + 1 < s.n_bands) {
      pace();
      __builtin_amdgcn_s_barrier();
      ++band;
      stamp(band);
    }
#pragma unroll
    for (int u = 0; u < U; ++u) {
      if (pr[u] >= 0) {
        float4 *p = &sweep_acc[pr[u] * LPR + sub];
        *p = f4_add(*p, pv[u]);
      }
    }
    for (int lr = lr0 + g; lr < lr1; lr += G)
      row_epilogue<D, SCALED>(a, s.row0 + tile_row0 + lr, sweep_acc[lr * LPR + sub], sub);
    if constexpr (AUX == kAuxStamp) {
      stamp(s.n_bands);
      if (wid == 0) {
        long long *o = x.stamps + (int64_t)tile * (s.n_bands + 1);
        for (int b = lane; b <= s.n_bands; b += 64) o[b] = stamp_lds[b];
        if (lane == 0) {
          x.meta[2 * tile] = (int32_t)blockIdx.x;
          x.meta[2 * tile + 1] = (int32_t)__builtin_amdgcn_s_getreg(kXccIdReg);
        }
      }
    }
    __syncthreads();
  }
  if constexpr (AUX == kAuxPace) {
    if (wid == 0 && lane == 0) {
      (void)__hip_atomic_fetch_add(pace_sum, 0u - (unsigned)told, __ATOMIC_RELAXED,
                                   __HIP_MEMORY_SCOPE_AGENT);
      (void)__hip_atomic_fetch_add(pace_reg, 0u - 1u, __ATOMIC_RELAXED, __HIP_MEMORY_SCOPE_AGENT);
      asm volatile("s_waitcnt vmcnt(0)" ::: "memory");
      unsigned *done = x.ws + 2 * kPaceLabels * kPaceLineWords;
      const unsigned left = __hip_atomic_fetch_add(done, 1u, __ATOMIC_RELAXED,
                                                   __HIP_MEMORY_SCOPE_AGENT);
      if (left == gridDim.x - 1) {
        for (int i = 0; i <= 2 * kPaceLabels; ++i)
          __hip_atomic_store(x.ws + i * kPaceLineWords, 0u, __ATOMIC_RELAXED,
                             __HIP_MEMORY_SCOPE_AGENT);
      }
    }
  }
}

template <int D, int U, bool SCALED>
__global__ __launch_bounds__(kSweepThreads) __attribute__((amdgpu_waves_per_eu(4, 4)))
MIREC_NO_PK_F32 void prop_sweep_wave_kernel(PropK a, SweepWaveK s) {
  sweep_wave_work<D, U, SCALED>(a, s);
}

template <int D, int U, bool SCALED, int AUX>
__global__ __launch_bounds__(kSweepThreads) __attribute__((amdgpu_waves_per_eu(4, 4)))
MIREC_NO_PK_F32 void prop_sweep_wave_aux_kernel(PropK a, SweepWaveK s, SweepAuxK x) {
  sweep_wave_work<D, U, SCALED, AUX>(a, s, x);
}

using PropFn = void (*)(PropK);

template <int D, int UNROLL>
static PropFn prop_kernel_for(int mode, bool masked, bool rowmask, bool weighted, bool scaled,
                              bool dropout) {
  if (mode == MIREC_IN_SPARSE) masked = true;
  if (mode == MIREC_IN_NONE) weighted = dropout = false;
#define MIREC_PROP_CASE(MODE_W, MASKED)                               \
  case (MODE_W) * 2 + (MASKED):                                       \
    return rowmask ? prop_kernel<D, UNROLL, (MODE_W), MASKED, true>   \
                   : prop_kernel<D, UNROLL, (MODE_W), MASKED, false>;
  switch ((mode | (weighted ? kWeighted : 0) | (scaled ? kScaled : 0) |
           (dropout ? kDropout : 0)) * 2 + masked) {
    MIREC_PROP_CASE(MIREC_IN_PRESCALED | kWeighted, false)
    MIREC_PROP_CASE(MIREC_IN_PRESCALED, false)
    MIREC_PROP_CASE(MIREC_IN_PRESCALED | kWeighted, true)
    MIREC_PROP_CASE(MIREC_IN_PRESCALED, true)
    MIREC_PROP_CASE(MIREC_IN_RAW | kWeighted, false)
    MIREC_PROP_CASE(MIREC_IN_RAW, false)
    MIREC_PROP_CASE(MIREC_IN_RAW | kWeighted, true)
    MIREC_PROP_CASE(MIREC_IN_RAW, true)
    MIREC_PROP_CASE(MIREC_IN_SPARSE | kWeighted, true)
    MIREC_PROP_CASE(MIREC_IN_SPARSE, true)
    MIREC_PROP_CASE(MIREC_IN_PRESCALED | kScaled, false)
    MIREC_PROP_CASE(MIREC_IN_PRESCALED | kScaled, true)
    MIREC_PROP_CASE(MIREC_IN_RAW | kScaled, false)
    MIREC_PROP_CASE(MIREC_IN_RAW | kScaled, true)
    MIREC_PROP_CASE(MIREC_IN_SPARSE | kScaled, true)
    MIREC_PROP_CASE(MIREC_IN_NONE | kScaled, false)
    MIREC_PROP_CASE(MIREC_IN_PRESCALED | kDropout, false)
    MIREC_PROP_CASE(MIREC_IN_PRESCALED | kDropout, true)
    MIREC_PROP_CASE(MIREC_IN_RAW | kDropout, false)
    MIREC_PROP_CASE(MIREC_IN_RAW | kDropout, true)
    MIREC_PROP_CASE(MIREC_IN_SPARSE | kDropout, true)
    default:
    MIREC_PROP_CASE(MIREC_IN_NONE, false)
  }
#undef MIREC_PROP_CASE
}

template <int D, int UNROLL>
static int launch_prop(const mirec_csr_t *c, PropK k, int64_t list_cap, int mode,
                       hipStream_t st, bool dropout = false) {
  constexpr int G = 64 / (D / 4);
  const int64_t rows = k.row_list != nullptr ? list_cap : c->n_rows;
  k.row_waves = (rows + G - 1) / G;
  const int64_t work = k.row_waves + c->n_seg;
  const bool scaled = !dropout && k.scale_next != nullptr;
  int64_t blocks = (work + kWavesPerBlock - 1) / kWavesPerBlock;
  if (k.row_list != nullptr) {
    if (k.wide_list != nullptr) blocks += list_cap;
    blocks = std::min(blocks, kListBlocks);
  }
  if (blocks > 0) {
    const PropFn kernel =
        prop_kernel_for<D, UNROLL>(mode, k.in_mask != nullptr, k.row_mask != nullptr,
                                   !dropout && k.val != nullptr, scaled, dropout);
    hipLaunchKernelGGL(kernel, dim3((unsigned)blocks), dim3(256), 0, st, k);
    MIREC_LAUNCH_CHECK();
  }
  if (c->n_long > 0) {
    const auto fin = scaled ? prop_finalize<D, true> : prop_finalize<D, false>;
    hipLaunchKernelGGL(fin, dim3((unsigned)c->n_long), dim3(256), 0, st, k, c->long_rows,
                       c->long_segptr, c->n_long);
    MIREC_LAUNCH_CHECK();
  }
  return MIREC_OK;
}

__global__ __launch_bounds__(256) void prescale_kernel(const float *__restrict__ x,
                                                       const float *__restrict__ dinv, int64_t n4,
                                                       int32_t d4, float *__restrict__ out) {
  const int64_t stride = (int64_t)gridDim.x * blockDim.x;
  for (int64_t i = (int64_t)blockIdx.x * blockDim.x + threadIdx.x; i < n4; i += stride)
    st4(out + 4 * i, f4_scale(dinv[i / d4], ld4(x + 4 * i)));
}

constexpr int kDotChunk = 256;

__device__ __forceinline__ int32_t row_of_entry(const int64_t *rowptr, int32_t lo, int32_t hi,
                                                int64_t e) {
  while (lo < hi) {
    const int32_t mid = lo + (hi - lo + 1) / 2;
    if (rowptr[mid] <= e)
      lo = mid;
    else
      hi = mid - 1;
  }
  return lo;
}

template <int D, int UNROLL>
__global__ __launch_bounds__(256) MIREC_NO_PK_F32 void edge_dot_kernel(
    const int64_t *__restrict__ rowptr, const int32_t *__restrict__ col, int64_t n_rows,
    int64_t nnz, const float *__restrict__ a, const float *__restrict__ b,
    float *__restrict__ out) {
  constexpr int LPR = D / 4;
  constexpr int G = 64 / LPR;
  const int lane = threadIdx.x & 63;
  const int grp = lane / LPR;
  const int sub = lane % LPR;
  const int64_t wave = (int64_t)blockIdx.x * kWavesPerBlock + (threadIdx.x >> 6);
  const int64_t e0 = wave * kDotChunk;
  if (e0 >= nnz) return;
  const int64_t e1 = min(e0 + (int64_t)kDotChunk, nnz);
  const int32_t r_lo = row_of_entry(rowptr, 0, (int32_t)(n_rows - 1), e0);
  const int32_t r_hi = row_of_entry(rowptr, r_lo, (int32_t)(n_rows - 1), e1 - 1);
  for (int64_t base = e0; base < e1; base += 64) {
    const int cnt = (int)min((int64_t)64, e1 - base);
    const int myc = lane < cnt ? col[base + lane] : 0;
    const int myrow = lane < cnt ? row_of_entry(rowptr, r_lo, r_hi, base + lane) : r_lo;
    float res = 0.f;
    for (int k = 0; k < cnt; k += G * UNROLL) {
      float4 va[UNROLL], vb[UNROLL];
#pragma unroll
      for (int u = 0; u < UNROLL; ++u) {
        const int idx = k + u * G + grp;
        const int j = __shfl(myc, idx & 63);
        const int r = __shfl(myrow, idx & 63);
        if (idx < cnt) {
          va[u] = ld4(a + (int64_t)r * D + sub * 4);
          vb[u] = ld4(b + (int64_t)j * D + sub * 4);
        } else {
          va[u] = f4_zero();
          vb[u] = f4_zero();
        }
      }
#pragma unroll
      for (int u = 0; u < UNROLL; ++u) {
        const float d = group_sum<LPR>(f4_dot(va[u], vb[u]));
        const float t = __shfl(d, (lane & (G - 1)) * LPR);
        if (lane >= k + u * G && lane < k + (u + 1) * G) res = t;
      }
    }
    if (lane < cnt) out[base + lane] = res;
  }
}

template <int D, int UNROLL>
static int launch_edge_dot(const mirec_csr_t *c, const float *a, const float *b, float *out,
                           hipStream_t st) {
  const int64_t waves = (c->nnz + kDotChunk - 1) / kDotChunk;
  const int64_t blocks = (waves + kWavesPerBlock - 1) / kWavesPerBlock;
  hipLaunchKernelGGL((edge_dot_kernel<D, UNROLL>), dim3((unsigned)blocks), dim3(256), 0, st,
                     c->rowptr, c->col, c->n_rows, c->nnz, a, b, out);
  MIREC_LAUNCH_CHECK();
  return MIREC_OK;
}

static bool sweep_launch_qualifies(const mirec_csr_t *c, const mirec_prop_t *p) {
  if (p->dim != 64) return false;
  if (c->val != nullptr) return false;
  if (p->in_mode != MIREC_IN_PRESCALED) return false;
  if (p->in_mask != nullptr || p->row_mask != nullptr || p->row_list != nullptr) return false;
  return c->n_seg == 0;
}

static bool sweep_qualifies(const mirec_csr_t *c, const mirec_prop_t *p, const mirec_sweep_t *sw) {
  if (sw == nullptr || !sweep_launch_qualifies(c, p)) return false;
  if (sw->gptr == nullptr || sw->ent == nullptr || sw->n_rows <= 0 || sw->n_tiles <= 0)
    return false;
  if (sw->row0 < 0 || sw->row0 + sw->n_rows != c->n_rows || sw->n_src > c->n_rows) return false;
  if (sw->tile_rows <= 0 || sw->group_rows <= 0 || sw->band_rows <= 0) return false;
  if (sw->groups <= 0 || sw->groups > kSweepThreads / (64 / 4)) return false;
  if ((int64_t)sw->groups * sw->group_rows < sw->tile_rows) return false;
  if ((int64_t)sw->n_tiles * sw->tile_rows < sw->n_rows) return false;
  if ((int64_t)sw->tile_rows * 64 * 4 > kSweepLdsMax) return false;
  return true;
}

template <int D, int UNROLL>
static int launch_head(const mirec_csr_t *c, const PropK &k, int64_t row0, hipStream_t st) {
  mirec_csr_t head = *c;
  head.n_rows = row0;
  PropK kh = k;
  kh.n_rows = row0;
  return launch_prop<D, UNROLL>(&head, kh, 0, MIREC_IN_PRESCALED, st);
}

template <int D, int UNROLL>
static int launch_sweep(const mirec_csr_t *c, const PropK &k, const mirec_sweep_t *sw,
                        hipStream_t st) {
  SweepK s;
  s.gptr = sw->gptr;
  s.ent = reinterpret_cast<const long long *>(sw->ent);
  s.row0 = sw->row0;
  s.n_rows = sw->n_rows;
  s.tile_rows = sw->tile_rows;
  s.group_rows = sw->group_rows;
  s.groups = sw->groups;
  s.band_rows = sw->band_rows;
  s.n_bands = (int32_t)std::max<int64_t>(1, (sw->n_src + sw->band_rows - 1) / sw->band_rows);
  const size_t lds = (size_t)sw->tile_rows * D * sizeof(float);
  const auto kernel =
      k.scale_next != nullptr ? prop_sweep_kernel<D, 4, true> : prop_sweep_kernel<D, 4, false>;
  hipLaunchKernelGGL(kernel, dim3((unsigned)sw->n_tiles), dim3(kSweepThreads), lds, st, k, s);
  MIREC_LAUNCH_CHECK();
  if (sw->row0 == 0) return MIREC_OK;
  return launch_head<D, UNROLL>(c, k, sw->row0, st);
}

static bool sweep_wave_valid(const mirec_csr_t *c, const mirec_sweep_wave_t *w, int64_t row0,
                             int64_t n_rows) {
  if (w == nullptr || w->wptr == nullptr || w->slot == nullptr || w->n_slots <= 0) return false;
  if (w->row0 != row0 || w->n_rows != n_rows || n_rows <= 0 || w->n_tiles <= 0) return false;
  if (w->src0 < 0 || w->n_src <= 0 || w->src0 + w->n_src > c->n_rows) return false;
  if (w->tile_rows <= 0 || w->wave_rows <= 0 || w->band_rows <= 0) return false;
  if ((int64_t)w->wave_rows * MIREC_SWEEP_WAVES < w->tile_rows) return false;
  if ((int64_t)w->n_tiles * w->tile_rows < n_rows) return false;
  if ((int64_t)(w->n_tiles - 1) * w->tile_rows >= n_rows) return false;
  if ((int64_t)w->tile_rows * 64 * 4 > kSweepLdsMax) return false;
  return w->grid > 0 && w->grid <= w->n_tiles;
}

struct SweepStamp {
  const mirec_sweep_wave_t *layout;
  int64_t *stamps;
  int64_t stamps_len;
  int32_t *meta;
};

static int32_t sweep_wave_bands(const mirec_sweep_wave_t *w) {
  return (int32_t)std::max<int64_t>(1, (w->n_src + w->band_rows - 1) / w->band_rows);
}

template <int D>
static int launch_sweep_wave(const PropK &k, const mirec_sweep_wave_t *w, hipStream_t st,
                             const mirec_sweep_pace_t *pace = nullptr, int block = 0,
                             const SweepStamp *stamp = nullptr) {
  SweepWaveK s;
  s.wptr = w->wptr;
  s.slot = reinterpret_cast<const long long *>(w->slot);
  s.n_slots = w->n_slots;
  s.row0 = w->row0;
  s.n_rows = w->n_rows;
  s.src0 = w->src0;
  s.tile_rows = w->tile_rows;
  s.wave_rows = w->wave_rows;
  s.n_tiles = w->n_tiles;
  s.band_rows = w->band_rows;
  s.n_bands = sweep_wave_bands(w);
  size_t lds = (size_t)w->tile_rows * D * sizeof(float);
  const bool scaled = k.scale_next != nullptr;
  if (stamp != nullptr) {
    SweepAuxK x = {};
    x.stamps = reinterpret_cast<long long *>(stamp->stamps);
    x.meta = stamp->meta;
    lds += (size_t)(s.n_bands + 1) * sizeof(long long);
    const auto kernel = scaled ? prop_sweep_wave_aux_kernel<D, 4, true, kAuxStamp>
                               : prop_sweep_wave_aux_kernel<D, 4, false, kAuxStamp>;
    if (lds > (size_t)kSweepLdsMax &&
        hipFuncSetAttribute(reinterpret_cast<const void *>(kernel),
                            hipFuncAttributeMaxDynamicSharedMemorySize, (int)lds) != hipSuccess)
      return MIREC_ERR_HIP;
    hipLaunchKernelGGL(kernel, dim3((unsigned)w->grid), dim3(kSweepThreads), lds, st, k, s, x);
  } else if (pace != nullptr && pace->every[block] > 0) {
    SweepAuxK x = {};
    x.ws = reinterpret_cast<unsigned *>(pace->ws) + block * kPaceRegionWords;
    x.lead = pace->lead_bands[block];
    x.every = pace->every[block];
    x.nap = pace->nap[block];
    const auto kernel = scaled ? prop_sweep_wave_aux_kernel<D, 4, true, kAuxPace>
                               : prop_sweep_wave_aux_kernel<D, 4, false, kAuxPace>;
    hipLaunchKernelGGL(kernel, dim3((unsigned)w->grid), dim3(kSweepThreads), lds, st, k, s, x);
  } else {
    const auto kernel = scaled ? prop_sweep_wave_kernel<D, 4, true>
                               : prop_sweep_wave_kernel<D, 4, false>;
    hipLaunchKernelGGL(kernel, dim3((unsigned)w->grid), dim3(kSweepThreads), lds, st, k, s);
  }
  MIREC_LAUNCH_CHECK();
  return MIREC_OK;
}

}

extern "C" int mirec_sweep_groups(int32_t dim) {
  return dim == 64 ? mirec::kSweepThreads / (64 / 4) : 0;
}

namespace mirec {

static int propagate(const mirec_csr_t *c, const mirec_prop_t *p, const mirec_sweep_t *sw,
                     const mirec_sweep_wave_t *wi, const mirec_sweep_wave_t *wu,
                     mirec_stream_t stream, const mirec_drop_t *drop = nullptr,
                     const mirec_sweep_pace_t *pace = nullptr,
                     const SweepStamp *stamp = nullptr) {
  MIREC_CHECK_ARG(c != nullptr && p != nullptr);
  if (pace != nullptr) {
    MIREC_CHECK_ARG(pace->ws != nullptr);
    for (int b = 0; b < 2; ++b)
      MIREC_CHECK_ARG(pace->every[b] >= 0 && pace->lead_bands[b] >= 0 && pace->nap[b] >= 0 &&
                      pace->nap[b] <= kPaceMaxNapUnits);
  }
  MIREC_CHECK_ARG(c->rowptr != nullptr && c->dinv != nullptr && c->n_rows >= 0);
  MIREC_CHECK_ARG(c->nnz == 0 || c->col != nullptr);
  if (!dim_supported(p->dim)) return MIREC_ERR_DIM;
  MIREC_CHECK_ARG(p->in_mode >= 0 && p->in_mode <= 3);
  if (p->in_mode == MIREC_IN_SPARSE)
    MIREC_CHECK_ARG(p->slot != nullptr && p->seed_in != nullptr);
  else if (p->in_mode != MIREC_IN_NONE)
    MIREC_CHECK_ARG(p->x_in != nullptr);
  MIREC_CHECK_ARG(p->in_mode != MIREC_IN_NONE || p->in_mask == nullptr);
  MIREC_CHECK_ARG((p->seed == nullptr && p->seed2 == nullptr) || p->slot != nullptr);
  MIREC_CHECK_ARG(p->param == nullptr || (p->exp_avg != nullptr && p->exp_avg_sq != nullptr));
  MIREC_CHECK_ARG(p->divisor != 0.f);
  MIREC_CHECK_ARG(p->row_list == nullptr ||
                  (p->row_count != nullptr && p->row_list_cap >= 0 && p->row_mask != nullptr));
  MIREC_CHECK_ARG(p->wide_list == nullptr || (p->row_list != nullptr && p->wide_count != nullptr));
  if (c->n_seg > 0) {
    MIREC_CHECK_ARG(c->split > 0 && c->seg_row && c->seg_beg && c->long_rows && c->long_segptr);
    if (p->partial == nullptr) return MIREC_ERR_WORKSPACE;
  }
  PropK k;
  k.rowptr = c->rowptr;
  k.col = c->col;
  k.dinv = c->dinv;
  k.n_rows = c->n_rows;
  k.n_seg = c->n_seg;
  k.seg_row = c->seg_row;
  k.seg_beg = c->seg_beg;
  k.split = c->n_seg > 0 ? c->split : 0;
  k.x_in = p->x_in;
  k.slot = p->slot;
  k.seed_in = p->seed_in;
  k.seed = p->seed;
  k.addend = p->addend;
  k.seed2 = p->seed2;
  k.divisor = p->divisor;
  k.out = p->out;
  k.xs_out = p->xs_out;
  k.param = p->param;
  k.m = p->exp_avg;
  k.v = p->exp_avg_sq;
  k.adam = p->adam;
  k.partial = p->partial;
  k.row_mask = p->row_mask;
  k.in_mask = p->in_mask;
  k.out_mask = p->out_mask;
  k.row_list = p->row_list;
  k.row_count = p->row_count;
  k.row_waves = 0;
  k.narrow_max = p->narrow_max;
  k.wide_list = p->wide_list;
  k.wide_count = p->wide_count;
  k.val = c->val;
  const bool scaled =
      p->scale_src != nullptr || p->scale_dst != nullptr || p->scale_next != nullptr;
  MIREC_CHECK_ARG(!scaled || c->val == nullptr);
  k.scale_src = k.scale_next = nullptr;
  if (scaled) {
    k.scale_src = p->scale_src != nullptr ? p->scale_src : c->dinv;
    k.dinv = p->scale_dst != nullptr ? p->scale_dst : c->dinv;
    k.scale_next = p->scale_next != nullptr ? p->scale_next : c->dinv;
  }
  const bool dropout = drop != nullptr && drop->keep_prob != 0.f;
  if (dropout) {
    uint32_t thresh_m1 = 0;
    MIREC_CHECK_ARG(edge_drop_thresh(drop->keep_prob, &thresh_m1));
    MIREC_CHECK_ARG(c->val == nullptr && !scaled);
    k.drop_key = edge_drop_key(drop->seed);
    k.drop_thresh_m1 = thresh_m1;
    k.drop_transposed = drop->transposed != 0;
    k.scale_next = nullptr;
    k.drop_scale = 1.f / drop->keep_prob;
  }
  const int64_t cap = p->row_list_cap;
  hipStream_t st = reinterpret_cast<hipStream_t>(stream);
  if (stamp != nullptr) {
    const mirec_sweep_wave_t *w = stamp->layout;
    MIREC_CHECK_ARG(w != nullptr && stamp->stamps != nullptr && stamp->meta != nullptr);
    MIREC_CHECK_ARG(sweep_launch_qualifies(c, p) && w->row0 >= 0 && w->n_rows > 0 &&
                    w->row0 + w->n_rows <= c->n_rows &&
                    sweep_wave_valid(c, w, w->row0, w->n_rows));
    MIREC_CHECK_ARG(stamp->stamps_len >= (int64_t)w->n_tiles * (sweep_wave_bands(w) + 1));
    return launch_sweep_wave<64>(k, w, st, nullptr, 0, stamp);
  }
  if (sweep_qualifies(c, p, sw)) return launch_sweep<64, 4>(c, k, sw, st);
  if (wi != nullptr && sweep_launch_qualifies(c, p) &&
      sweep_wave_valid(c, wi, wi->row0, c->n_rows - wi->row0)) {
    const int rc = launch_sweep_wave<64>(k, wi, st, pace, 0);
    if (rc != MIREC_OK || wi->row0 == 0) return rc;
    if (sweep_wave_valid(c, wu, 0, wi->row0)) return launch_sweep_wave<64>(k, wu, st, pace, 1);
    return launch_head<64, 4>(c, k, wi->row0, st);
  }
  switch (p->dim) {
    case 4: return launch_prop<4, 1>(c, k, cap, p->in_mode, st, dropout);
    case 8: return launch_prop<8, 1>(c, k, cap, p->in_mode, st, dropout);
    case 16: return launch_prop<16, 1>(c, k, cap, p->in_mode, st, dropout);
    case 32: return launch_prop<32, 2>(c, k, cap, p->in_mode, st, dropout);
    case 64: return launch_prop<64, 4>(c, k, cap, p->in_mode, st, dropout);
    case 128: return launch_prop<128, 4>(c, k, cap, p->in_mode, st, dropout);
    case 256: return launch_prop<256, 8>(c, k, cap, p->in_mode, st, dropout);
  }
  return MIREC_ERR_DIM;
}

}

extern "C" int mirec_propagate(const mirec_csr_t *c, const mirec_prop_t *p,
                               mirec_stream_t stream) {
  return mirec_propagate_sweep(c, p, nullptr, stream);
}

extern "C" int mirec_propagate_sweep(const mirec_csr_t *c, const mirec_prop_t *p,
                                     const mirec_sweep_t *sw, mirec_stream_t stream) {
  return mirec::propagate(c, p, sw, nullptr, nullptr, stream);
}

extern "C" int mirec_propagate_sweep_wave(const mirec_csr_t *c, const mirec_prop_t *p,
                                          const mirec_sweep_wave_t *items,
                                          const mirec_sweep_wave_t *users,
                                          mirec_stream_t stream) {
  return mirec::propagate(c, p, nullptr, items, users, stream);
}

extern "C" size_t mirec_sweep_pace_sizeof(void) { return sizeof(mirec_sweep_pace_t); }

extern "C" size_t mirec_sweep_pace_ws_bytes(void) {
  return 2 * (size_t)mirec::kPaceRegionWords * sizeof(unsigned);
}

extern "C" int mirec_propagate_sweep_wave_paced(const mirec_csr_t *c, const mirec_prop_t *p,
                                                const mirec_sweep_wave_t *items,
                                                const mirec_sweep_wave_t *users,
                                                const mirec_sweep_pace_t *pace,
                                                mirec_stream_t stream) {
  return mirec::propagate(c, p, nullptr, items, users, stream, nullptr, pace);
}

extern "C" int mirec_sweep_wave_stamp(const mirec_csr_t *c, const mirec_prop_t *p,
                                      const mirec_sweep_wave_t *layout, int64_t *stamps,
                                      int64_t stamps_len, int32_t *meta, mirec_stream_t stream) {
  const mirec::SweepStamp s = {layout, stamps, stamps_len, meta};
  return mirec::propagate(c, p, nullptr, nullptr, nullptr, stream, nullptr, nullptr, &s);
}

extern "C" size_t mirec_drop_sizeof(void) { return sizeof(mirec_drop_t); }

extern "C" int mirec_propagate_drop(const mirec_csr_t *c, const mirec_prop_t *p,
                                    const mirec_drop_t *drop, mirec_stream_t stream) {
  return mirec::propagate(c, p, nullptr, nullptr, nullptr, stream, drop);
}

extern "C" int mirec_edge_keep_mask(const int64_t *rowptr, const int32_t *col, int64_t n_rows,
                                    uint64_t seed, float keep_prob, int32_t transposed,
                                    uint8_t *keep) {
  using namespace mirec;
  MIREC_CHECK_ARG(rowptr != nullptr && n_rows >= 0);
  uint32_t thresh_m1 = 0;
  MIREC_CHECK_ARG(edge_drop_thresh(keep_prob, &thresh_m1));
  if (n_rows == 0 || rowptr[n_rows] == rowptr[0]) return MIREC_OK;
  MIREC_CHECK_ARG(col != nullptr && keep != nullptr);
  const uint64_t key = edge_drop_key(seed);
  for (int64_t i = 0; i < n_rows; ++i) {
    for (int64_t e = rowptr[i]; e < rowptr[i + 1]; ++e) {
      const uint32_t r = (uint32_t)i, c = (uint32_t)col[e];
      keep[e] = edge_keep(key, transposed ? c : r, transposed ? r : c, thresh_m1) ? 1 : 0;
    }
  }
  return MIREC_OK;
}

extern "C" int mirec_edge_dot(const mirec_csr_t *c, const float *a, const float *b, int32_t dim,
                              float *out, mirec_stream_t stream) {
  using namespace mirec;
  MIREC_CHECK_ARG(c != nullptr && c->rowptr != nullptr && c->n_rows >= 0 && c->nnz >= 0);
  if (!dim_supported(dim)) return MIREC_ERR_DIM;
  if (c->nnz == 0) return MIREC_OK;
  MIREC_CHECK_ARG(c->n_rows > 0 && c->col != nullptr && a != nullptr && b != nullptr &&
                  out != nullptr);
  hipStream_t st = reinterpret_cast<hipStream_t>(stream);
  switch (dim) {
    case 4: return launch_edge_dot<4, 1>(c, a, b, out, st);
    case 8: return launch_edge_dot<8, 1>(c, a, b, out, st);
    case 16: return launch_edge_dot<16, 1>(c, a, b, out, st);
    case 32: return launch_edge_dot<32, 2>(c, a, b, out, st);
    case 64: return launch_edge_dot<64, 4>(c, a, b, out, st);
    case 128: return launch_edge_dot<128, 4>(c, a, b, out, st);
    case 256: return launch_edge_dot<256, 4>(c, a, b, out, st);
  }
  return MIREC_ERR_DIM;
}

extern "C" int mirec_prescale(const float *x, const float *dinv, int64_t n_rows, int32_t dim,
                              float *out, mirec_stream_t stream) {
  using namespace mirec;
  MIREC_CHECK_ARG(x && dinv && out && n_rows >= 0);
  if (!dim_supported(dim)) return MIREC_ERR_DIM;
  const int64_t n4 = n_rows * dim / 4;
  if (n4 == 0) return MIREC_OK;
  const int64_t blocks = std::min<int64_t>((n4 + 255) / 256, 256 * 16);
  hipLaunchKernelGGL(prescale_kernel, dim3(blocks), dim3(256), 0,
                     reinterpret_cast<hipStream_t>(stream), x, dinv, n4, dim / 4, out);
  MIREC_LAUNCH_CHECK();
  return MIREC_OK;
}
```

### furusato_recommend_amd/engine.py

```python
from __future__ import annotations

import ctypes
import math
import os

import torch

from . import _lib
from ._lib import (IN_NONE, IN_PRESCALED, IN_RAW, IN_SPARSE, Prop, adam_hparams,
                   check, lib, ptr)
from .graph import Graph

SWEEP_FORM = "wave"
SWEEP_USERS = True
LAYER_SUM_ROWS = "self"
SWEEP_PACE = {"items": (8, 16, 16), "users": (4, 4, 16)}


def prop_launch_bytes(in_mode: int, n_nodes: int, nnz: int, dim: int, *, slot=False,
                      xs_out=False, addend=False, out=False, adam=False, weighted=False,
                      scaled=False) -> int:
    N, D = n_nodes, dim
    row = N * D * 4
    b = (N + 1) * 8 + N * 4
    if in_mode == IN_PRESCALED:
        b += nnz * (D * 4 + 4)
    elif in_mode == IN_RAW:
        b += nnz * (D * 4 + 4 + 4)
    elif in_mode == IN_SPARSE:
        b += nnz * (4 + 4 + 4)
    if weighted and in_mode != IN_NONE:
        b += nnz * 4
    if slot:
        b += N * 4
    if scaled:
        b += N * 4
    b += row * (int(xs_out) + int(addend) + int(out))
    if adam:
        b += 6 * row
    return b


_raw_writes = 0


def _note_raw_write():
    global _raw_writes
    _raw_writes += 1


class AdamState:

    def __init__(self, param: torch.Tensor, lr: float, betas=(0.9, 0.999), eps: float = 1e-8):
        self.param = param
        self.lr = float(lr)
        self.betas = (float(betas[0]), float(betas[1]))
        self.eps = float(eps)
        self.n_steps = 0
        self.exp_avg = torch.zeros_like(param)
        self.exp_avg_sq = torch.zeros_like(param)
        self.stale_rows = False

    def next_hparams(self):
        self.n_steps += 1
        return adam_hparams(self.lr, self.betas[0], self.betas[1], self.eps, self.n_steps)

    def zero_grad(self, set_to_none: bool = True):
        if self.param.grad is not None:
            if set_to_none:
                self.param.grad = None
            else:
                self.param.grad.zero_()

    @torch.no_grad()
    def step(self):
        g = self.param.grad
        if g is None:
            return
        hp = self.next_hparams()
        _note_raw_write()
        check(lib.mirec_adam_dense(self.param.data_ptr(), g.contiguous().data_ptr(),
                                   self.exp_avg.data_ptr(), self.exp_avg_sq.data_ptr(),
                                   self.param.numel(), ctypes.byref(hp), _lib.stream_handle()),
              "adam_dense")

    def _launch(self, hp):
        g = self.param.grad.contiguous()
        check(lib.mirec_adam_dense(self.param.data_ptr(), g.data_ptr(),
                                   self.exp_avg.data_ptr(), self.exp_avg_sq.data_ptr(),
                                   self.param.numel(), ctypes.byref(hp), _lib.stream_handle()),
              "adam_dense")

    def state_dict(self, param_id: int = 0) -> dict:
        if self.stale_rows:
            raise RuntimeError("Adam moments are sharded over the data-parallel ranks: call "
                               "gather_optimizer_state() on every rank before state_dict()")
        return {
            "state": {param_id: {"step": torch.tensor(float(self.n_steps)),
                                 "exp_avg": self.exp_avg, "exp_avg_sq": self.exp_avg_sq}},
            "param_groups": [{"lr": self.lr, "betas": self.betas, "eps": self.eps,
                              "weight_decay": 0, "amsgrad": False, "maximize": False,
                              "foreach": None, "capturable": False, "differentiable": False,
                              "fused": None, "params": [param_id]}],
        }

    def load_state_dict(self, sd: dict) -> None:
        st = next(iter(sd["state"].values())) if sd["state"] else None
        if st is not None:
            self.n_steps = int(float(st["step"]))
            self.exp_avg.copy_(st["exp_avg"])
            self.exp_avg_sq.copy_(st["exp_avg_sq"])
        g = sd["param_groups"][0]
        self.lr, self.betas, self.eps = float(g["lr"]), tuple(g["betas"]), float(g["eps"])


class AdamGroup:

    LARGE = 1 << 20

    def __init__(self, states):
        self.states = list(states)

    def __iter__(self):
        return iter(self.states)

    def __len__(self):
        return len(self.states)

    def zero_grad(self, set_to_none: bool = True):
        for s in self.states:
            s.zero_grad(set_to_none)

    @torch.no_grad()
    def step(self):
        groups = {}
        for s in self.states:
            if s.param.grad is None:
                continue
            hp = s.next_hparams()
            if s.param.numel() >= self.LARGE:
                s._launch(hp)
                continue
            key = (s.n_steps, s.lr, s.betas, s.eps)
            groups.setdefault(key, (hp, []))[1].append(s)
        if not groups and not any(s.param.grad is not None for s in self.states):
            return
        _note_raw_write()
        for hp, members in groups.values():
            n = len(members)
            grads = [m.param.grad.contiguous() for m in members]
            arr = lambda xs: (ctypes.c_void_p * n)(*[x.data_ptr() for x in xs])
            numel = (ctypes.c_int64 * n)(*[m.param.numel() for m in members])
            check(lib.mirec_adam_multi(n, arr([m.param for m in members]), arr(grads),
                                       arr([m.exp_avg for m in members]),
                                       arr([m.exp_avg_sq for m in members]), numel,
                                       ctypes.byref(hp), _lib.stream_handle()), "adam_multi")

    def next_shared_hparams(self, require_grad: bool = True):
        keys = {(s.n_steps, s.lr, s.betas, s.eps) for s in self.states}
        if len(keys) != 1 or (require_grad and any(s.param.grad is None for s in self.states)):
            raise RuntimeError("device-scalar Adam needs one shared step for every parameter")
        hps = [s.next_hparams() for s in self.states]
        return hps[0]

    @torch.no_grad()
    def step_device(self, h_dev: torch.Tensor):
        _note_raw_write()
        large = [s for s in self.states if s.param.numel() >= self.LARGE]
        small = [s for s in self.states if s.param.numel() < self.LARGE]
        for s in large:
            g = s.param.grad.contiguous()
            check(lib.mirec_adam_dense_dev(s.param.data_ptr(), g.data_ptr(), s.exp_avg.data_ptr(),
                                           s.exp_avg_sq.data_ptr(), s.param.numel(),
                                           h_dev.data_ptr(), _lib.stream_handle()),
                  "adam_dense_dev")
        if small:
            n = len(small)
            grads = [m.param.grad.contiguous() for m in small]
            arr = lambda xs: (ctypes.c_void_p * n)(*[x.data_ptr() for x in xs])
            numel = (ctypes.c_int64 * n)(*[m.param.numel() for m in small])
            check(lib.mirec_adam_multi_dev(n, arr([m.param for m in small]), arr(grads),
                                           arr([m.exp_avg for m in small]),
                                           arr([m.exp_avg_sq for m in small]), numel,
                                           h_dev.data_ptr(), _lib.stream_handle()),
                  "adam_multi_dev")


class PropagationEngine:

    def __init__(self, graph: Graph, dim: int, n_layers: int, max_batch: int,
                 prune: bool = True, n_neg: int = 1, n_shared: int = 0):
        if int(n_neg) < 1:
            raise ValueError(f"n_neg must be at least 1, got {n_neg!r}")
        if int(n_shared) < 0:
            raise ValueError(f"n_shared must not be negative, got {n_shared!r}")
        if dim not in _lib.SUPPORTED_DIMS:
            raise ValueError(f"recdim={dim} not supported by the HIP engine "
                             f"(supported: {_lib.SUPPORTED_DIMS})")
        if graph.device.type != "cuda":
            raise RuntimeError("PropagationEngine needs a HIP device (no CPU fallback)")
        self.g = graph
        self.dim = int(dim)
        self.L = int(n_layers)
        self.max_batch = int(max_batch)
        self.prune = bool(prune)
        self.n_neg = int(n_neg)
        self.n_shared = int(n_shared)
        self.loss_name = "bpr"
        dev = graph.device
        N, D = graph.n_nodes, self.dim
        f32 = dict(dtype=torch.float32, device=dev)
        i32 = dict(dtype=torch.int32, device=dev)
        self.acc = torch.empty(N, D, **f32)
        self.x0s = torch.empty(N, D, **f32) if self.L > 0 else None
        self.xs = [torch.empty(N, D, **f32), torch.empty(N, D, **f32)] if self.L > 1 else \
            [torch.empty(N, D, **f32)] if self.L == 1 else []
        self.slot = torch.full((N,), -1, **i32)
        words = (N + 15) // 16 * 4
        self._bm = torch.zeros(2, words, **i32)
        self.bm_self, self.bm_hop = self._bm[0], self._bm[1]
        B3 = max((2 + self.n_neg) * self.max_batch, 2 * self.max_batch + self.n_shared)
        self.self_list = torch.zeros(B3, **i32)
        self.self_count = torch.zeros(1, **i32)
        self._self_cap = 0
        cap = N if self.prune else 1
        self.s_lists = (torch.zeros(cap, **i32), torch.zeros(cap, **i32))
        self.hop_lists = (torch.zeros(cap, **i32), torch.zeros(cap, **i32))
        self.list_counts = torch.zeros(4, **i32)
        self.use_hop_list = True
        self.reuse_prescaled = True
        self.layer_sum_rows = LAYER_SUM_ROWS
        self.use_sweep = True
        self._group_sizes = (None, None, None)
        self._wave_sizes = {"items": (None, None), "users": (None, None), "max_grid": None}
        self.sweep_wave = self.sweep_wave_users = None
        self._sweep_form, self._sweep_users = SWEEP_FORM, SWEEP_USERS
        self.sweep_pace = SWEEP_PACE
        self._pace_ws = None
        self._wave_layouts()
        self.sparse_filter = "auto"
        self._masks_ready = False
        self.narrow_max = 64
        self.seed_p = torch.empty(B3, D, **f32)
        self.seed_e = torch.empty(B3, D, **f32)
        self.coef = torch.empty(self.n_neg * self.max_batch, **f32)
        self.coef_pos = self.g_u = None
        self._shared = None
        self.softplus = torch.empty(self.max_batch, **f32)
        self.reg = torch.empty(self.max_batch, **f32)
        self.keys = torch.empty(B3, **i32)
        self.vals = torch.empty(B3, **i32)
        self.keys_sorted = torch.empty(B3, **i32)
        self.loss = torch.zeros(1, **f32)
        self.partial = graph.partial_buffer(D)
        self._ws = None
        self._ws_bytes = 0
        self._ensure_ws(self.max_batch)
        self.prop_events = None
        self._seeds = None
        self._merged = None
        self._x0s_token = None
        self._acc_full = None
        self.edge_dropout = None
        self._drop = None

    @staticmethod
    def dropout_seed(seed: int, step: int) -> int:
        return ((int(seed) & 0xFFFFFFFF) << 32) | (int(step) & 0xFFFFFFFF)

    def set_dropout(self, keep_prob: float | None, seed: int = 0):
        if keep_prob is None:
            self._drop = None
            return
        kp = float(keep_prob)
        if not (0.0 < kp <= 1.0):
            raise ValueError(f"edge dropout: keep_prob must lie in (0, 1], got {keep_prob!r}")
        if self.g.val is not None or self.g.scale_src is not None:
            raise ValueError("edge dropout is not combined with edge weights or an "
                             "r-adjusted normalisation")
        self._drop = (kp, int(seed) & (2 ** 64 - 1))
        self._acc_full = None

    def _ensure_ws(self, batch: int):
        nb = ctypes.c_size_t(0)
        check(lib.mirec_bpr_seed_workspace(batch, self.g.n_nodes, ctypes.byref(nb)),
              "bpr_seed_workspace")
        if nb.value > self._ws_bytes:
            self._ws = torch.empty(nb.value, dtype=torch.uint8, device=self.g.device)
            self._ws_bytes = nb.value

    def _ensure_ssm(self, batch: int, n_neg: int):
        if self.g_u is None:
            f32 = dict(dtype=torch.float32, device=self.g.device)
            self.coef_pos = torch.empty(self.max_batch, **f32)
            self.g_u = torch.empty(self.max_batch, self.dim, **f32)
        nb = ctypes.c_size_t(0)
        check(lib.mirec_ssm_seed_workspace(batch, n_neg, self.g.n_nodes, ctypes.byref(nb)),
              "ssm_seed_workspace")
        if nb.value > self._ws_bytes:
            self._ws = torch.empty(nb.value, dtype=torch.uint8, device=self.g.device)
            self._ws_bytes = nb.value

    def _ensure_ssm_shared(self, batch: int, m: int):
        if self._shared is None:
            dev, B, M = self.g.device, self.max_batch, self.n_shared
            f32 = dict(dtype=torch.float32, device=dev)
            self._shared = dict(coef=torch.empty(B * M, **f32), coef_pos=torch.empty(B, **f32),
                                g=torch.empty(B + M, self.dim, **f32),
                                reg=torch.empty(M, **f32),
                                mask=torch.empty(B * M, dtype=torch.uint8, device=dev))
        nb = ctypes.c_size_t(0)
        check(lib.mirec_ssm_shared_seed_workspace(batch, m, self.g.n_nodes, ctypes.byref(nb)),
              "ssm_shared_seed_workspace")
        if nb.value > self._ws_bytes:
            self._ws = torch.empty(nb.value, dtype=torch.uint8, device=self.g.device)
            self._ws_bytes = nb.value
        return self._shared

    def _prop(self, *, in_mode, x_in=None, seed_in=None, seed=None, addend=None, seed2=None,
              divisor=1.0, out=None, xs_out=None, adam=None, param=None, graph=None,
              row_mask=None, in_mask=None, row_list=None, row_count=None, row_list_cap=0,
              out_mask=None, wide_list=None, wide_count=None, direction="fwd", stamp=None):
        g = graph or self.g
        p = Prop()
        if g.scale_src is not None:
            a, b = g.scale_src.data_ptr(), g.scale_dst.data_ptr()
            if direction == "fwd":
                p.scale_src, p.scale_dst, p.scale_next = a, b, a
            elif direction in ("bwd", "bwd_last"):
                p.scale_src, p.scale_dst = b, a
                p.scale_next = a if direction == "bwd_last" else b
            else:
                raise ValueError(f"direction: 'fwd', 'bwd' or 'bwd_last', got {direction!r}")
        p.dim = self.dim
        p.in_mode = in_mode
        p.x_in = ptr(x_in)
        p.slot = self.slot.data_ptr() if (seed_in is not None or seed is not None
                                          or seed2 is not None) else None
        p.seed_in = ptr(seed_in)
        p.seed = ptr(seed)
        p.addend = ptr(addend)
        p.seed2 = ptr(seed2)
        p.divisor = float(divisor)
        p.out = ptr(out)
        p.xs_out = ptr(xs_out)
        if adam is not None:
            state, hp = adam
            p.param = param.data_ptr()
            p.exp_avg = state.exp_avg.data_ptr()
            p.exp_avg_sq = state.exp_avg_sq.data_ptr()
            p.adam = hp
        part = g.partial_buffer(self.dim)
        p.partial = ptr(part)
        p.row_mask = ptr(row_mask)
        p.in_mask = ptr(in_mask)
        p.out_mask = ptr(out_mask)
        p.row_list = ptr(row_list)
        p.row_count = ptr(row_count)
        p.row_list_cap = int(row_list_cap)
        p.wide_list = ptr(wide_list)
        p.wide_count = ptr(wide_count)
        p.narrow_max = int(self.narrow_max)
        ev = self.prop_events
        if ev is not None:
            s, e = torch.cuda.Event(enable_timing=True), torch.cuda.Event(enable_timing=True)
            s.record()
        on = self.use_sweep and g is self.g
        if stamp is not None:
            lay, stamps, meta = stamp
            check(lib.mirec_sweep_wave_stamp(g.csr_ptr(), ctypes.byref(p), lay.ptr(),
                                             stamps.data_ptr(), stamps.numel(), meta.data_ptr(),
                                             _lib.stream_handle()), "sweep_wave_stamp")
        elif self._drop is not None:
            if direction not in ("fwd", "bwd", "bwd_last"):
                raise ValueError(f"direction: 'fwd', 'bwd' or 'bwd_last', got {direction!r}")
            drop = _lib.Drop(keep_prob=self._drop[0], transposed=int(direction != "fwd"),
                             seed=self._drop[1])
            check(lib.mirec_propagate_drop(g.csr_ptr(), ctypes.byref(p), ctypes.byref(drop),
                                           _lib.stream_handle()), "propagate_drop")
        elif on and self._sweep_form == "wave":
            wi, wu = self.sweep_wave, self.sweep_wave_users if self._sweep_users else None
            pace = self._pace_struct()
            check(lib.mirec_propagate_sweep_wave_paced(
                g.csr_ptr(), ctypes.byref(p), wi.ptr() if wi is not None else None,
                wu.ptr() if wu is not None else None,
                ctypes.byref(pace) if pace is not None else None, _lib.stream_handle()),
                "propagate")
        else:
            sw = self.sweep if on else None
            check(lib.mirec_propagate_sweep(g.csr_ptr(), ctypes.byref(p),
                                            sw.ptr() if sw is not None else None,
                                            _lib.stream_handle()), "propagate")
        if ev is not None:
            e.record()
            kind = (in_mode, in_mask is not None, row_mask is not None, out_mask is not None)
            ev.append((s, e, kind, self.launch_bytes(p, g)))

    def _pace_struct(self):
        sp = self.sweep_pace
        if sp is None:
            return None
        if self._pace_ws is None:
            self._pace_ws = torch.zeros(int(lib.mirec_sweep_pace_ws_bytes()) // 4,
                                        dtype=torch.int32, device=self.g.device)
        pace = _lib.SweepPace(ws=self._pace_ws.data_ptr())
        for b, block in enumerate(("items", "users")):
            lead, every, nap = sp.get(block) or (0, 0, 0)
            pace.lead_bands[b], pace.every[b], pace.nap[b] = int(lead), int(every), int(nap)
        return pace

    def sweep_stamp(self, block: str, **launch):
        lay = self.sweep_wave if block == "items" else self.sweep_wave_users
        if lay is None:
            raise RuntimeError(f"no wave-form layout of the {block} block")
        d = lay.desc
        bands = max(1, -(-d.n_src // d.band_rows))
        stamps = torch.zeros(d.n_tiles, bands + 1, dtype=torch.int64, device=self.g.device)
        meta = torch.zeros(d.n_tiles, 2, dtype=torch.int32, device=self.g.device)
        self._prop(stamp=(lay, stamps, meta), **launch)
        return stamps, meta

    def launch_bytes(self, p: Prop, g: Graph) -> int:
        om = bool(p.out_mask)
        return prop_launch_bytes(p.in_mode, g.n_nodes, g.nnz, self.dim,
                                 slot=bool(p.slot and (p.seed or p.seed2)),
                                 xs_out=bool(p.xs_out), addend=bool(p.addend) and not om,
                                 out=bool(p.out) and not om, adam=bool(p.param),
                                 weighted=g.val is not None,
                                 scaled=bool(p.scale_next) and bool(p.xs_out)
                                 and p.scale_next != p.scale_dst)

    def compute_frontier(self, users=None, pos=None, neg=None, keys=None, n_keys: int = 0):
        g = self.g
        lists = self.prune and self.use_hop_list
        zc, nz = (self.list_counts.data_ptr(), 4) if lists else (None, 0)
        if keys is not None:
            n = int(n_keys)
            if self.self_list.shape[0] < n:
                self.self_list = torch.zeros(n, dtype=torch.int32, device=g.device)
            check(lib.mirec_frontier(g.csr_ptr(), keys.data_ptr(), n, None, None, None,
                                     0, g.n_users, self.bm_self.data_ptr(),
                                     self.bm_hop.data_ptr(), self.self_list.data_ptr(),
                                     self.self_count.data_ptr(), zc, nz, _lib.stream_handle()),
                  "frontier")
            self._self_cap = n
        else:
            B = int(users.shape[0])
            if B > self.max_batch:
                raise ValueError(f"batch {B} > engine max_batch {self.max_batch}")
            check(lib.mirec_frontier(g.csr_ptr(), None, 0, users.data_ptr(), pos.data_ptr(),
                                     neg.data_ptr(), B, g.n_users,
                                     self.bm_self.data_ptr(), self.bm_hop.data_ptr(),
                                     self.self_list.data_ptr(), self.self_count.data_ptr(),
                                     zc, nz, _lib.stream_handle()), "frontier")
            self._self_cap = 3 * B
        if lists:
            check(lib.mirec_mask_compact_pair(self.bm_self.data_ptr(), self.bm_hop.data_ptr(),
                                              self._wide_bits().data_ptr(), g.n_nodes,
                                              self.s_lists[0].data_ptr(),
                                              self.s_lists[1].data_ptr(),
                                              self.hop_lists[0].data_ptr(),
                                              self.hop_lists[1].data_ptr(),
                                              self.list_counts.data_ptr(), _lib.stream_handle()),
                  "mask_compact_pair")
        self._masks_ready = True

    def set_sweep_sizes(self, tile_rows: int | None = None, group_rows: int | None = None,
                        band_rows: int | None = None, *, wave_items=None, wave_users=None,
                        max_grid: int | None = None):
        self._group_sizes = (tile_rows, group_rows, band_rows)
        self._wave_sizes = {"items": tuple(wave_items or (tile_rows, band_rows)),
                            "users": tuple(wave_users or (None, None)), "max_grid": max_grid}
        self.sweep_wave = self.sweep_wave_users = None
        self._wave_layouts()

    @property
    def sweep(self):
        return self.g.sweep_layout(self.dim, *self._group_sizes)

    def _wave_layouts(self):
        if self._sweep_form != "wave":
            return
        ws = self._wave_sizes
        if self.sweep_wave is None:
            self.sweep_wave = self.g.sweep_wave_layout(self.dim, "items", *ws["items"],
                                                       max_grid=ws["max_grid"])
        if self._sweep_users and self.sweep_wave is not None and self.sweep_wave_users is None:
            self.sweep_wave_users = self.g.sweep_wave_layout(self.dim, "users", *ws["users"],
                                                             max_grid=ws["max_grid"])

    @property
    def sweep_form(self) -> str:
        return self._sweep_form

    @sweep_form.setter
    def sweep_form(self, form: str):
        if form not in ("wave", "group"):
            raise ValueError(f"sweep_form: 'wave' or 'group', got {form!r}")
        self._sweep_form = form
        self._wave_layouts()

    @property
    def sweep_users(self) -> bool:
        return self._sweep_users

    @sweep_users.setter
    def sweep_users(self, on: bool):
        self._sweep_users = bool(on)
        self._wave_layouts()

    def _wide_bits(self) -> torch.Tensor:
        key = int(self.narrow_max)
        wb = getattr(self, "_wide_bits_cache", None)
        if wb is not None and wb[0] == key:
            return wb[1]
        g = self.g
        rp = g.rowptr
        n = g.n_nodes
        wide = (rp[1:n + 1] - rp[:n]) > key
        words = (n + 31) // 32
        bits = torch.zeros(words * 32, dtype=torch.int64, device=wide.device)
        bits[:n] = wide.to(torch.int64)
        shifts = torch.arange(32, dtype=torch.int64, device=wide.device)
        w = (bits.view(words, 32) << shifts).sum(1)
        w = torch.where(w >= 2 ** 31, w - 2 ** 32, w).to(torch.int32)
        self._wide_bits_cache = (key, w.contiguous())
        return self._wide_bits_cache[1]

    def _lists(self, k, bm, lists, cap):
        if not self.use_hop_list:
            return dict(row_mask=bm)
        c = self.list_counts
        return dict(row_mask=bm, row_list=lists[0], row_count=c[2 * k], row_list_cap=cap,
                    wide_list=lists[1], wide_count=c[2 * k + 1])

    def _dense_seeds(self, seed_p, clear: int):
        if getattr(self, "seed_dense", None) is None:
            self.seed_dense = torch.zeros(self.g.n_nodes, self.dim, dtype=torch.float32,
                                          device=self.g.device)
        check(lib.mirec_seed_dense(self.self_list.data_ptr(), self.self_count.data_ptr(),
                                   self._self_cap, self.slot.data_ptr(),
                                   self._scale(backward=True).data_ptr(),
                                   seed_p.data_ptr(), self.dim, self.seed_dense.data_ptr(),
                                   int(clear), _lib.stream_handle()), "seed_dense")
        return self.seed_dense

    def _sparse_filter(self):
        f = self.sparse_filter
        if f == "auto":
            f = "bytemap" if self._self_cap > (2 + self.n_neg) * self.max_batch else "slot"
        return self.bm_self if f == "bytemap" else None

    def static_row_lists(self, bm: torch.Tensor) -> dict:
        g = self.g
        N = g.n_nodes
        dev = g.device
        nl = torch.zeros(max(N, 1), dtype=torch.int32, device=dev)
        wl = torch.zeros(max(N, 1), dtype=torch.int32, device=dev)
        cnt = torch.zeros(2, dtype=torch.int32, device=dev)
        check(lib.mirec_mask_compact(g.csr_ptr(), bm.data_ptr(), int(self.narrow_max),
                                     nl.data_ptr(), cnt[0].data_ptr(), wl.data_ptr(),
                                     cnt[1].data_ptr(), 0, _lib.stream_handle()), "mask_compact")
        return dict(row_mask=bm, row_list=nl, row_count=cnt[0], row_list_cap=N,
                    wide_list=wl, wide_count=cnt[1])

    def _self_rows(self):
        return self._lists(0, self.bm_self, self.s_lists, min(self._self_cap, self.g.n_nodes))

    def _hop_rows(self):
        return self._lists(1, self.bm_hop, self.hop_lists, self.g.n_nodes)

    @staticmethod
    def _token(emb: torch.Tensor):
        return (emb.data_ptr(), emb._version, _raw_writes)

    def invalidate_prescaled(self):
        self._x0s_token = None
        self._acc_full = None

    def mark_prescaled(self, emb: torch.Tensor):
        self._x0s_token = self._token(emb)
        self._acc_full = None

    def _scale(self, backward: bool = False) -> torch.Tensor:
        g = self.g
        if g.scale_src is None:
            return g.dinv
        return g.scale_dst if backward else g.scale_src

    def prescale(self, x: torch.Tensor, out: torch.Tensor):
        check(lib.mirec_prescale(x.data_ptr(), self._scale().data_ptr(), self.g.n_nodes, self.dim,
                                 out.data_ptr(), _lib.stream_handle()), "prescale")

    def forward(self, emb: torch.Tensor, pruned: bool = False) -> torch.Tensor:
        L = self.L
        self._acc_full = None
        if self.layer_sum_rows not in ("self", "hop"):
            raise ValueError(f"layer_sum_rows: 'self' or 'hop', got {self.layer_sum_rows!r}")
        if L == 0:
            self.acc.copy_(emb)
            self._acc_full = self._token(emb)
            return self.acc
        if pruned and not self._masks_ready:
            raise RuntimeError("forward(pruned=True) needs compute_frontier() first")
        if self._x0s_token != self._token(emb):
            self.prescale(emb, self.x0s)
            self._x0s_token = self._token(emb)
        for l in range(1, L + 1):
            last = l == L
            rows = {}
            if pruned and l == L:
                rows = self._self_rows()
            elif pruned and l == L - 1:
                rows = self._hop_rows()
            if pruned and l < L and self.layer_sum_rows == "self":
                rows["out_mask"] = self.bm_self
            elif pruned and l == L - 2:
                rows["out_mask"] = self.bm_hop
            self._prop(in_mode=IN_PRESCALED,
                       x_in=self.x0s if l == 1 else self.xs[(l - 2) % 2],
                       addend=emb if l == 1 else self.acc,
                       divisor=float(L + 1) if last else 1.0,
                       out=self.acc,
                       xs_out=None if last else self.xs[(l - 1) % 2],
                       **rows)
        if not pruned and self._drop is None:
            self._acc_full = self._token(emb)
        return self.acc

    def forward_cached(self, emb: torch.Tensor) -> torch.Tensor:
        if self._acc_full is not None and self._acc_full == self._token(emb):
            return self.acc
        return self.forward(emb)

    def propagate_once(self, x: torch.Tensor, out: torch.Tensor, graph: Graph | None = None):
        self._prop(in_mode=IN_RAW, x_in=x, out=out, graph=graph)

    def propagate_accumulate(self, g_in: torch.Tensor, addend: torch.Tensor,
                             out: torch.Tensor, graph: Graph | None = None,
                             transposed: bool = False):
        self._prop(in_mode=IN_RAW, x_in=g_in, addend=addend, out=out, graph=graph,
                   direction="bwd" if transposed else "fwd")

    def bpr(self, out: torch.Tensor, emb: torch.Tensor, users, pos, neg, decay: float,
            loss_accum: torch.Tensor | None = None, grad_scale: float = 1.0) -> torch.Tensor:
        B = int(users.shape[0])
        if B > self.max_batch:
            raise ValueError(f"batch {B} > engine max_batch {self.max_batch}")
        if not self._masks_ready:
            self.compute_frontier(users, pos, neg)
        self._ensure_ws(B)
        st = _lib.stream_handle()
        g = self.g
        check(lib.mirec_bpr_forward(out.data_ptr(), emb.data_ptr(), g.n_nodes, g.n_users,
                                    self.dim, B, users.data_ptr(), pos.data_ptr(),
                                    neg.data_ptr(), float(grad_scale), self.coef.data_ptr(),
                                    self.softplus.data_ptr(), self.reg.data_ptr(),
                                    self.keys.data_ptr(), self.vals.data_ptr(), st),
              "bpr_forward")
        check(lib.mirec_bpr_loss(self.softplus.data_ptr(), self.reg.data_ptr(), B,
                                 float(decay), self.loss.data_ptr(), ptr(loss_accum), st),
              "bpr_loss")
        check(lib.mirec_bpr_seed(out.data_ptr(), emb.data_ptr(), g.n_nodes, g.n_users,
                                 self.dim, B, users.data_ptr(), pos.data_ptr(),
                                 neg.data_ptr(), self.coef.data_ptr(), self.keys.data_ptr(),
                                 self.vals.data_ptr(), float(decay), float(grad_scale), self.L,
                                 self.slot.data_ptr(), self.seed_p.data_ptr(),
                                 self.seed_e.data_ptr(), self.keys_sorted.data_ptr(),
                                 self._ws.data_ptr(), self._ws_bytes, st), "bpr_seed")
        self._seeds = (self.seed_p, self.seed_e, self.keys_sorted, 3 * B)
        return self.loss

    def _ssm_shape(self, users, neg):
        B = int(users.shape[0])
        if B > self.max_batch:
            raise ValueError(f"batch {B} > engine max_batch {self.max_batch}")
        if neg.dim() != 2 or int(neg.shape[0]) != B or int(neg.shape[1]) < 1:
            raise ValueError(f"ssm: neg must have shape [{B}, K], got {tuple(neg.shape)}")
        K = int(neg.shape[1])
        if K > self.n_neg:
            raise ValueError(f"ssm: {K} negatives per pair > engine n_neg {self.n_neg}")
        if neg.dtype != torch.int32 or not neg.is_contiguous():
            raise ValueError("ssm: neg must be a contiguous int32 tensor")
        return B, K

    def frontier_ssm(self, users, pos, neg):
        B, K = self._ssm_shape(users, neg)
        check(lib.mirec_ssm_keys(users.data_ptr(), pos.data_ptr(), neg.data_ptr(), B, K,
                                 self.g.n_users, self.keys.data_ptr(), _lib.stream_handle()),
              "ssm_keys")
        self.compute_frontier(keys=self.keys, n_keys=(2 + K) * B)

    def ssm(self, out: torch.Tensor, emb: torch.Tensor, users, pos, neg, decay: float,
            temp: float, loss_accum: torch.Tensor | None = None,
            grad_scale: float = 1.0) -> torch.Tensor:
        B, K = self._ssm_shape(users, neg)
        if not (float(temp) > 0.0 and math.isfinite(float(temp))):
            raise ValueError(f"ssm: temp must be positive and finite, got {temp!r}")
        if not self._masks_ready:
            self.frontier_ssm(users, pos, neg)
        self._ensure_ssm(B, K)
        st = _lib.stream_handle()
        g = self.g
        check(lib.mirec_ssm_forward(out.data_ptr(), emb.data_ptr(), g.n_nodes, g.n_users,
                                    self.dim, B, K, users.data_ptr(), pos.data_ptr(),
                                    neg.data_ptr(), float(temp), float(grad_scale),
                                    self.coef.data_ptr(), self.coef_pos.data_ptr(),
                                    self.softplus.data_ptr(), self.reg.data_ptr(),
                                    self.g_u.data_ptr(), self.keys.data_ptr(),
                                    self.vals.data_ptr(), st), "ssm_forward")
        check(lib.mirec_bpr_loss(self.softplus.data_ptr(), self.reg.data_ptr(), B,
                                 float(decay), self.loss.data_ptr(), ptr(loss_accum), st),
              "bpr_loss")
        check(lib.mirec_ssm_seed(out.data_ptr(), emb.data_ptr(), g.n_nodes, g.n_users, self.dim,
                                 B, K, users.data_ptr(), self.coef.data_ptr(),
                                 self.coef_pos.data_ptr(), self.g_u.data_ptr(),
                                 self.keys.data_ptr(), self.vals.data_ptr(), float(decay),
                                 float(grad_scale), self.L, self.slot.data_ptr(),
                                 self.seed_p.data_ptr(), self.seed_e.data_ptr(),
                                 self.keys_sorted.data_ptr(), self._ws.data_ptr(),
                                 self._ws_bytes, st), "ssm_seed")
        self._seeds = (self.seed_p, self.seed_e, self.keys_sorted, (2 + K) * B)
        return self.loss

    def _ssm_shared_shape(self, users, shared):
        B = int(users.shape[0])
        if B > self.max_batch:
            raise ValueError(f"batch {B} > engine max_batch {self.max_batch}")
        if shared.dim() != 1 or int(shared.shape[0]) < 1:
            raise ValueError(f"ssm_shared: shared must have shape [M], M >= 1, got "
                             f"{tuple(shared.shape)}")
        M = int(shared.shape[0])
        if M > self.n_shared:
            raise ValueError(f"ssm_shared: {M} shared negatives > engine n_shared "
                             f"{self.n_shared}")
        if shared.dtype != torch.int32 or not shared.is_contiguous():
            raise ValueError("ssm_shared: shared must be a contiguous int32 tensor")
        return B, M

    def frontier_ssm_shared(self, users, pos, shared):
        B, M = self._ssm_shared_shape(users, shared)
        check(lib.mirec_ssm_shared_keys(users.data_ptr(), pos.data_ptr(), shared.data_ptr(), B, M,
                                        self.g.n_users, self.keys.data_ptr(),
                                        _lib.stream_handle()), "ssm_shared_keys")
        self.compute_frontier(keys=self.keys, n_keys=2 * B + M)

    def ssm_shared(self, out: torch.Tensor, emb: torch.Tensor, users, pos, shared, decay: float,
                   temp: float, loss_accum: torch.Tensor | None = None,
                   grad_scale: float = 1.0) -> torch.Tensor:
        B, M = self._ssm_shared_shape(users, shared)
        if not (float(temp) > 0.0 and math.isfinite(float(temp))):
            raise ValueError(f"ssm_shared: temp must be positive and finite, got {temp!r}")
        if not self._masks_ready:
            self.frontier_ssm_shared(users, pos, shared)
        b = self._ensure_ssm_shared(B, M)
        st = _lib.stream_handle()
        g = self.g
        check(lib.mirec_ssm_shared_mask(g.csr_ptr(), users.data_ptr(), B, pos.data_ptr(),
                                        shared.data_ptr(), M, g.n_users, b["mask"].data_ptr(),
                                        st), "ssm_shared_mask")
        check(lib.mirec_ssm_shared_forward(out.data_ptr(), emb.data_ptr(), g.n_nodes, g.n_users,
                                           self.dim, B, M, users.data_ptr(), pos.data_ptr(),
                                           shared.data_ptr(), b["mask"].data_ptr(), float(temp),
                                           float(grad_scale), b["coef"].data_ptr(),
                                           b["coef_pos"].data_ptr(), self.softplus.data_ptr(),
                                           self.reg.data_ptr(), b["reg"].data_ptr(),
                                           b["g"].data_ptr(), self.keys.data_ptr(),
                                           self.vals.data_ptr(), st), "ssm_shared_forward")
        check(lib.mirec_ssm_shared_loss(self.softplus.data_ptr(), self.reg.data_ptr(),
                                        b["reg"].data_ptr(), B, M, float(decay),
                                        self.loss.data_ptr(), ptr(loss_accum), st),
              "ssm_shared_loss")
        check(lib.mirec_ssm_shared_seed(out.data_ptr(), emb.data_ptr(), g.n_nodes, g.n_users,
                                        self.dim, B, M, users.data_ptr(),
                                        b["coef_pos"].data_ptr(), b["g"].data_ptr(),
                                        self.keys.data_ptr(), self.vals.data_ptr(), float(decay),
                                        float(grad_scale), self.L, self.slot.data_ptr(),
                                        self.seed_p.data_ptr(), self.seed_e.data_ptr(),
                                        self.keys_sorted.data_ptr(), self._ws.data_ptr(),
                                        self._ws_bytes, st), "ssm_shared_seed")
        self._seeds = (self.seed_p, self.seed_e, self.keys_sorted, 2 * B + M)
        return self.loss

    def export_seeds(self):
        seed_p, seed_e, ks, n = self._seeds
        st = _lib.stream_handle()
        packed = self.keys[:n]
        check(lib.mirec_seed_pack(ks.data_ptr(), n, self.g.n_nodes, packed.data_ptr(), st),
              "seed_pack")
        check(lib.mirec_bpr_seed_reset(self.slot.data_ptr(), ks.data_ptr(), n, st),
              "bpr_seed_reset")
        self._masks_ready = False
        return packed, seed_p[:n], seed_e[:n]

    def import_seeds(self, keys, rows_p, rows_e):
        n = int(keys.shape[0])
        if self._merged is None or self._merged[0].shape[0] < n:
            dev, D = self.g.device, self.dim
            self._merged = (torch.empty(n, D, dtype=torch.float32, device=dev),
                            torch.empty(n, D, dtype=torch.float32, device=dev),
                            torch.empty(n, dtype=torch.int32, device=dev))
        mp, me, mk = self._merged
        nb = ctypes.c_size_t(0)
        check(lib.mirec_seed_merge_workspace(n, self.g.n_nodes, ctypes.byref(nb)),
              "seed_merge_workspace")
        if nb.value > self._ws_bytes:
            self._ws = torch.empty(nb.value, dtype=torch.uint8, device=self.g.device)
            self._ws_bytes = nb.value
        check(lib.mirec_seed_merge(keys.data_ptr(), rows_p.data_ptr(), rows_e.data_ptr(), n,
                                   self.dim, self.g.n_nodes, self.slot.data_ptr(), mp.data_ptr(),
                                   me.data_ptr(), mk.data_ptr(), self._ws.data_ptr(),
                                   self._ws_bytes, _lib.stream_handle()), "seed_merge")
        self.compute_frontier(keys=mk, n_keys=n)
        self._seeds = (mp, me, mk, n)

    def backward(self, emb: torch.Tensor, adam: AdamState | None = None,
                 grad_out: torch.Tensor | None = None, last_rows=None, on_chunk=None):
        if (adam is None) == (grad_out is None):
            raise ValueError("exactly one of adam / grad_out")
        self._acc_full = None
        if self._seeds is None or not self._masks_ready:
            raise RuntimeError("backward() needs bpr() (or import_seeds()) first")
        L = self.L
        seed_p, seed_e, keys_sorted, n_keys = self._seeds
        hp = adam.next_hparams() if adam is not None else None
        final = dict(seed2=seed_e, direction="bwd_last")
        if adam is not None:
            final.update(adam=(adam, hp), param=emb)
            if L > 0 and self.reuse_prescaled:
                final.update(xs_out=self.x0s)
        else:
            final.update(out=grad_out)
        chunks = list(last_rows) if isinstance(last_rows, (list, tuple)) else [last_rows]

        def last_layer(**kw):
            for c, rows in enumerate(chunks):
                self._prop(**kw, **final, **(rows or {}))
                if on_chunk is not None:
                    on_chunk(c)
        if L == 0:
            last_layer(in_mode=IN_NONE, seed=seed_p)
        else:
            for l in range(L - 1, -1, -1):
                first = l == L - 1
                if first:
                    rows = self._hop_rows() if (self.prune and l > 0) else {}
                    if self.sparse_filter == "dense":
                        kw = dict(in_mode=IN_PRESCALED, x_in=self._dense_seeds(seed_p, 0),
                                  in_mask=self.bm_self, **rows)
                    else:
                        kw = dict(in_mode=IN_SPARSE, seed_in=seed_p,
                                  in_mask=self._sparse_filter(), **rows)
                else:
                    kw = dict(in_mode=IN_PRESCALED, x_in=self.xs[(L - 2 - l) % 2],
                              in_mask=self.bm_hop if (self.prune and l == L - 2) else None)
                kw["seed"] = seed_p
                if l == 0:
                    last_layer(**kw)
                else:
                    kw.update(xs_out=self.xs[(L - 1 - l) % 2])
                    self._prop(**kw, direction="bwd")
        if self.sparse_filter == "dense" and L > 0:
            self._dense_seeds(seed_p, 1)
        check(lib.mirec_bpr_seed_reset(self.slot.data_ptr(), keys_sorted.data_ptr(), n_keys,
                                       _lib.stream_handle()), "bpr_seed_reset")
        self._seeds = None
        self._masks_ready = False
        self._x0s_token = self._token(emb) if (adam is not None and L > 0 and last_rows is None
                                               and self.reuse_prescaled) else None

    def adam_step(self, param: torch.Tensor, grad: torch.Tensor, adam: AdamState):
        _note_raw_write()
        self._acc_full = None
        hp = adam.next_hparams()
        check(lib.mirec_adam_dense(param.data_ptr(), grad.data_ptr(), adam.exp_avg.data_ptr(),
                                   adam.exp_avg_sq.data_ptr(), param.numel(), ctypes.byref(hp),
                                   _lib.stream_handle()), "adam_dense")

    def forward_for_batch(self, emb: torch.Tensor, users, pos, neg) -> torch.Tensor:
        self.compute_frontier(users, pos, neg)
        return self.forward(emb, pruned=self.prune)

    def train_step(self, emb: torch.Tensor, adam: AdamState, users, pos, neg, decay: float,
                   loss_accum: torch.Tensor | None = None, dropout=None) -> torch.Tensor:
        if dropout is None:
            out = self.forward_for_batch(emb, users, pos, neg)
            loss = self.bpr(out, emb, users, pos, neg, decay, loss_accum)
            self.backward(emb, adam=adam)
            return loss
        self.set_dropout(*dropout)
        try:
            out = self.forward_for_batch(emb, users, pos, neg)
            loss = self.bpr(out, emb, users, pos, neg, decay, loss_accum)
            self.backward(emb, adam=adam)
        finally:
            self.set_dropout(None)
        return loss

    def train_step_ssm(self, emb: torch.Tensor, adam: AdamState, users, pos, neg, decay: float,
                       temp: float, loss_accum: torch.Tensor | None = None,
                       dropout=None) -> torch.Tensor:
        if dropout is not None:
            self.set_dropout(*dropout)
        try:
            self.frontier_ssm(users, pos, neg)
            out = self.forward(emb, pruned=self.prune)
            loss = self.ssm(out, emb, users, pos, neg, decay, temp, loss_accum)
            self.backward(emb, adam=adam)
        finally:
            if dropout is not None:
                self.set_dropout(None)
        return loss

    def train_step_ssm_shared(self, emb: torch.Tensor, adam: AdamState, users, pos, shared,
                              decay: float, temp: float,
                              loss_accum: torch.Tensor | None = None,
                              dropout=None) -> torch.Tensor:
        if dropout is not None:
            self.set_dropout(*dropout)
        try:
            self.frontier_ssm_shared(users, pos, shared)
            out = self.forward(emb, pruned=self.prune)
            loss = self.ssm_shared(out, emb, users, pos, shared, decay, temp, loss_accum)
            self.backward(emb, adam=adam)
        finally:
            if dropout is not None:
                self.set_dropout(None)
        return loss


def sample_shared(m_items: int, n_sets: int, m: int, seed: int, offset: int, out):
    s, o = ctypes.c_uint64(seed & (2**64 - 1)), ctypes.c_uint64(offset & (2**64 - 1))
    if out.device.type == "cuda":
        check(lib.mirec_shared_sample(int(m_items), int(n_sets), int(m), s, o, out.data_ptr(),
                                      _lib.stream_handle()), "shared_sample")
    else:
        check(lib.mirec_cpu_shared_sample(int(m_items), int(n_sets), int(m), s, o,
                                          out.data_ptr(), 1), "cpu_shared_sample")


def edge_dot(graph: Graph, a: torch.Tensor, b: torch.Tensor, out: torch.Tensor):
    n, D = a.shape
    if D not in _lib.SUPPORTED_DIMS or n != graph.n_nodes or b.shape != a.shape:
        raise ValueError(f"edge_dot: a {tuple(a.shape)}, b {tuple(b.shape)}, "
                         f"graph of {graph.n_nodes} nodes")
    if (a.dtype != torch.float32 or b.dtype != torch.float32 or out.dtype != torch.float32
            or not (a.is_contiguous() and b.is_contiguous() and out.is_contiguous())
            or out.numel() < graph.nnz):
        raise ValueError("edge_dot: contiguous float32 tensors, out of nnz entries required")
    check(lib.mirec_edge_dot(graph.csr_ptr(), a.data_ptr(), b.data_ptr(), D, out.data_ptr(),
                             _lib.stream_handle()), "edge_dot")


def propagate(graph: Graph, x: torch.Tensor, out: torch.Tensor, dropout=None,
              transposed: bool = False):
    n, D = x.shape
    if D not in _lib.SUPPORTED_DIMS or n != graph.n_nodes or out.shape != x.shape:
        raise ValueError(f"propagate: x {tuple(x.shape)}, out {tuple(out.shape)}, "
                         f"graph of {graph.n_nodes} nodes")
    if x.dtype != torch.float32 or not (x.is_contiguous() and out.is_contiguous()):
        raise ValueError("propagate: contiguous float32 tensors required")
    p = Prop()
    p.dim = D
    p.in_mode = IN_RAW
    p.x_in = x.data_ptr()
    p.divisor = 1.0
    p.out = out.data_ptr()
    p.partial = ptr(graph.partial_buffer(D))
    p.narrow_max = 64
    if graph.scale_src is not None:
        p.scale_src = graph.scale_src.data_ptr()
        p.scale_dst = graph.scale_dst.data_ptr()
    if dropout is not None:
        kp, seed = dropout
        if not (0.0 < float(kp) <= 1.0):
            raise ValueError(f"edge dropout: keep_prob must lie in (0, 1], got {kp!r}")
        drop = _lib.Drop(keep_prob=float(kp), transposed=int(bool(transposed)),
                         seed=int(seed) & (2 ** 64 - 1))
        check(lib.mirec_propagate_drop(graph.csr_ptr(), ctypes.byref(p), ctypes.byref(drop),
                                       _lib.stream_handle()), "propagate_drop")
        return
    check(lib.mirec_propagate(graph.csr_ptr(), ctypes.byref(p), _lib.stream_handle()),
          "propagate")


def sample_triples(graph: Graph, batch: int, seed: int, offset: int, users, pos, neg, err,
                   shard: int = 0, n_shards: int = 1):
    check(lib.mirec_bpr_sample_ex(graph.csr_ptr(), ptr(getattr(graph, "pos_cdf", None)),
                                  graph.n_users, graph.m_items, int(batch),
                                  ctypes.c_uint64(seed & (2**64 - 1)),
                                  ctypes.c_uint64(offset & (2**64 - 1)), int(shard),
                                  int(n_shards), users.data_ptr(), pos.data_ptr(),
                                  neg.data_ptr(), err.data_ptr(), _lib.stream_handle()),
          "bpr_sample")


def sample_pairs(graph: Graph, batch: int, n_neg: int, seed: int, offset: int, users, pos, neg,
                 err, shard: int = 0, n_shards: int = 1):
    check(lib.mirec_ssm_sample(graph.csr_ptr(), ptr(getattr(graph, "pos_cdf", None)),
                               graph.n_users, graph.m_items, int(batch), int(n_neg),
                               ctypes.c_uint64(seed & (2**64 - 1)),
                               ctypes.c_uint64(offset & (2**64 - 1)), int(shard),
                               int(n_shards), users.data_ptr(), pos.data_ptr(),
                               neg.data_ptr(), err.data_ptr(), _lib.stream_handle()),
          "ssm_sample")


def sample_epoch_capped(graph: Graph, n_candidates: int, cap: int, seed: int, offset: int = 0,
                        shard: int = 0, n_shards: int = 1, return_candidates: bool = False,
                        n_threads: int | None = None):
    dev = graph.device
    n = int(n_candidates)
    i32 = dict(dtype=torch.int32, device=dev)
    users, pos, neg = (torch.empty(max(n, 1), **i32) for _ in range(3))
    count = torch.zeros(1, **i32)
    err = torch.zeros(1, **i32)
    cu = torch.empty(max(n, 1), **i32) if return_candidates else None
    cp = torch.empty(max(n, 1), **i32) if return_candidates else None
    if dev.type == "cpu":
        check(lib.mirec_cpu_bpr_sample_capped(
# ... 33 lines not shown
```

### include/mirec.h

```cpp
#ifndef MIREC_H
#define MIREC_H

#include <stddef.h>
#include <stdint.h>

#ifdef __cplusplus
extern "C" {
#endif

#define MIREC_ABI_VERSION 1

enum mirec_status {
  MIREC_OK = 0,
  MIREC_ERR_ARG = 1,
  MIREC_ERR_DIM = 2,
  MIREC_ERR_HIP = 3,
  MIREC_ERR_WORKSPACE = 4,
  MIREC_ERR_RANGE = 5
};

typedef void *mirec_stream_t;

const char *mirec_strerror(int code);
int mirec_abi_version(void);
// ... 60 lines not shown
  float bc2_sqrt;
  float eps;
} mirec_adam_hparams_t;

typedef struct mirec_prop {
  int32_t dim;
  int32_t in_mode;
  const float *x_in;
  const int32_t *slot;
  const float *seed_in;
  const float *seed;
  const float *addend;
  const float *seed2;
  float divisor;
  float _pad;
  float *out;
  float *xs_out;
  float *param;
  float *exp_avg;
  float *exp_avg_sq;
  mirec_adam_hparams_t adam;
  float *partial;
  const uint8_t *row_mask;
  const uint8_t *in_mask;
  const uint8_t *out_mask;
  const int32_t *row_list;
  const int32_t *row_count;
  int64_t row_list_cap;
  int32_t narrow_max;
  int32_t _pad2;
  const int32_t *wide_list;
  const int32_t *wide_count;
  const float *scale_src;
  const float *scale_dst;
  const float *scale_next;
} mirec_prop_t;

int mirec_propagate(const mirec_csr_t *csr, const mirec_prop_t *p,
                    mirec_stream_t stream);

int mirec_edge_keep_mask(const int64_t *rowptr, const int32_t *col, int64_t n_rows,
                         uint64_t seed, float keep_prob, int32_t transposed,
                         uint8_t *keep);


typedef struct mirec_drop {
  float keep_prob;
  int32_t transposed;
  uint64_t seed;
} mirec_drop_t;

size_t mirec_drop_sizeof(void);

int mirec_propagate_drop(const mirec_csr_t *csr, const mirec_prop_t *p,
                         const mirec_drop_t *drop, mirec_stream_t stream);

typedef struct mirec_sweep {
  int64_t row0;
  int64_t n_rows;
  int64_t n_src;
  int32_t tile_rows;
  int32_t group_rows;
  int32_t groups;
  int32_t n_tiles;
  int32_t band_rows;
  int32_t _pad;
  const int64_t *gptr;
  const int32_t *ent;
} mirec_sweep_t;

size_t mirec_sweep_sizeof(void);

int mirec_sweep_shape(int64_t n_rows, int32_t tile_rows, int32_t group_rows,
                      int32_t *n_tiles, int32_t *groups);

int mirec_sweep_build(const int64_t *rowptr, const int32_t *col, int64_t row0,
                      int64_t n_rows, int64_t n_src, int32_t tile_rows,
                      int32_t group_rows, int64_t *gptr, int32_t *ent);

int mirec_sweep_groups(int32_t dim);

int mirec_propagate_sweep(const mirec_csr_t *csr, const mirec_prop_t *p,
                          const mirec_sweep_t *sw, mirec_stream_t stream);

#define MIREC_SWEEP_WAVES 8
#define MIREC_SWEEP_LOOKAHEAD 16
#define MIREC_SWEEP_BATCH 16

typedef struct mirec_sweep_wave {
  int64_t row0;
  int64_t n_rows;
  int64_t src0;
  int64_t n_src;
  int64_t n_slots;
  int32_t tile_rows;
  int32_t wave_rows;
  int32_t n_tiles;
  int32_t band_rows;
  int32_t grid;
  int32_t _pad;
  const int64_t *wptr;
  const int64_t *slot;
} mirec_sweep_wave_t;

size_t mirec_sweep_wave_sizeof(void);

int mirec_sweep_wave_build(const int64_t *rowptr, const int32_t *col, int64_t row0,
                           int64_t n_rows, int64_t src0, int64_t n_src,
                           int32_t tile_rows, int64_t *wptr, int64_t *slot,
                           int64_t slot_cap, int64_t *n_slots);

int mirec_propagate_sweep_wave(const mirec_csr_t *csr, const mirec_prop_t *p,
                               const mirec_sweep_wave_t *items,
                               const mirec_sweep_wave_t *users, mirec_stream_t stream);

typedef struct mirec_sweep_pace {
  void *ws;
  int32_t lead_bands[2];
  int32_t every[2];
  int32_t nap[2];
} mirec_sweep_pace_t;

size_t mirec_sweep_pace_sizeof(void);
size_t mirec_sweep_pace_ws_bytes(void);

int mirec_propagate_sweep_wave_paced(const mirec_csr_t *csr, const mirec_prop_t *p,
                                     const mirec_sweep_wave_t *items,
                                     const mirec_sweep_wave_t *users,
                                     const mirec_sweep_pace_t *pace, mirec_stream_t stream);

int mirec_sweep_wave_stamp(const mirec_csr_t *csr, const mirec_prop_t *p,
                           const mirec_sweep_wave_t *layout, int64_t *stamps,
                           int64_t stamps_len, int32_t *meta, mirec_stream_t stream);

int mirec_edge_dot(const mirec_csr_t *csr, const float *a, const float *b,
                   int32_t dim, float *out, mirec_stream_t stream);

int mirec_prescale(const float *x, const float *dinv, int64_t n_rows,
                   int32_t dim, float *out, mirec_stream_t stream);

int mirec_shard_pack(const float *table, int64_t n_rows, int32_t dim, int32_t world,
                     int32_t rank, int64_t slot0, int64_t n_slots, float *stage_rank,
                     mirec_stream_t stream);
int mirec_shard_unpack(const float *stage, int64_t n_rows, int32_t dim, int32_t world,
                       int32_t rank, int64_t slot0, int64_t n_slots, const float *dinv,
                       float *table, float *x0s, mirec_stream_t stream);

int mirec_frontier(const mirec_csr_t *csr, const int32_t *keys, int64_t n_keys,
                   const int32_t *users, const int32_t *pos, const int32_t *neg,
                   int64_t batch, int64_t n_users, uint8_t *bm_self,
                   uint8_t *bm_hop, int32_t *self_list, int32_t *self_count,
                   int32_t *zero_counts, int32_t n_zero_counts, mirec_stream_t stream);

int mirec_mask_compact_pair(const uint8_t *bm_a, const uint8_t *bm_b, const uint32_t *wide_bits,
                            int64_t n_rows, int32_t *list_a, int32_t *wide_a, int32_t *list_b,
                            int32_t *wide_b, int32_t *counts, mirec_stream_t stream);

int mirec_small_sort_workspace(int64_t n, size_t *bytes);
int mirec_small_sort_pairs(const int32_t *keys_in, const int32_t *vals_in, int32_t *keys_out,
                           int32_t *vals_out, int64_t n, void *workspace, size_t workspace_bytes,
                           mirec_stream_t stream);

int mirec_mask_compact(const mirec_csr_t *csr, const uint8_t *bm,
                       int32_t narrow_max, int32_t *list, int32_t *count,
                       int32_t *wide_list, int32_t *wide_count, int32_t counts_zeroed,
                       mirec_stream_t stream);

int64_t mirec_distinct_rows_workspace(int64_t n_rows);
int mirec_distinct_rows(const int32_t *ids, int64_t n, int64_t n_rows, int64_t lo,
                        int64_t hi, int32_t *out, int32_t *count, void *workspace,
                        size_t workspace_bytes, mirec_stream_t stream);
int mirec_distinct_rows_unseen(const int32_t *ids, int64_t n, int64_t n_rows, int64_t lo,
                            int64_t hi, uint8_t *have, int32_t *out, int32_t *count,
                            void *workspace, size_t workspace_bytes, mirec_stream_t stream);

int mirec_stamped_rows(const int32_t *stamp, int64_t n_rows, int32_t gen, int32_t parts,
                       int32_t *rows, int32_t *counts, void *workspace,
                       size_t workspace_bytes, mirec_stream_t stream);

int mirec_scatter_rows(const float *src, const int32_t *ids, int64_t n, int32_t dim,
                       float *dst, mirec_stream_t stream);

typedef struct mirec_row_block {
  const int32_t *ids;
  const float *rows;
  int64_t n;
} mirec_row_block_t;

int64_t mirec_owner_sum_workspace(int32_t n_blocks, int64_t n_own);
int mirec_owner_sum(const mirec_row_block_t *blocks, int32_t n_blocks, int64_t lo,
                    int64_t n_own, int32_t dim, void *workspace, size_t workspace_bytes,
                    float *out, mirec_stream_t stream);

int mirec_gather_rows_counted(const float *src, const int32_t *rows, const int32_t *count,
                              int64_t capacity, int32_t dim, float *out,
                              mirec_stream_t stream);

int mirec_route_pack(const int32_t *ids, const int32_t *count, int64_t capacity, int64_t n_rows,
                     int32_t parts, int32_t cap, int64_t stride, int32_t *blocks,
                     mirec_stream_t stream);
int mirec_gather_rows_routed(const float *table, int64_t n_rows, const int32_t *blocks,
                             int32_t parts, int32_t cap, int64_t stride, int32_t dim, float *out,
                             mirec_stream_t stream);


int mirec_bpr_forward(const float *out, const float *emb, int64_t n_nodes,
                      int64_t n_users, int32_t dim, int64_t batch,
                      const int32_t *users, const int32_t *pos,
                      const int32_t *neg, float grad_scale, float *coef,
                      float *softplus, float *reg, int32_t *keys,
                      int32_t *vals, mirec_stream_t stream);

int mirec_bpr_loss(const float *softplus, const float *reg, int64_t batch,
                   float decay, float *loss_out, float *loss_accum,
                   mirec_stream_t stream);

int mirec_bpr_seed_workspace(int64_t batch, int64_t n_nodes, size_t *bytes);

int mirec_bpr_seed(const float *out, const float *emb, int64_t n_nodes,
                   int64_t n_users, int32_t dim, int64_t batch,
                   const int32_t *users, const int32_t *pos,
                   const int32_t *neg, const float *coef,
                   const int32_t *keys, const int32_t *vals, float decay,
                   float grad_scale, int32_t n_layers, int32_t *slot, float *seed_p,
                   float *seed_e, int32_t *keys_sorted, void *workspace,
                   size_t workspace_bytes, mirec_stream_t stream);

int mirec_bpr_seed_reset(int32_t *slot, const int32_t *keys_sorted, int64_t n,
                         mirec_stream_t stream);

int mirec_seed_dense(const int32_t *list, const int32_t *count, int64_t cap,
                     const int32_t *slot, const float *dinv, const float *seed,
                     int32_t dim, float *dense, int32_t clear, mirec_stream_t stream);

int mirec_seed_pack(const int32_t *keys_sorted, int64_t n, int64_t n_nodes,
                    int32_t *keys_packed, mirec_stream_t stream);

int mirec_seed_merge_workspace(int64_t n, int64_t n_nodes, size_t *bytes);

int mirec_seed_merge(const int32_t *keys_packed, const float *rows_p,
                     const float *rows_e, int64_t n, int32_t dim,
                     int64_t n_nodes, int32_t *slot, float *seed_p,
                     float *seed_e, int32_t *keys_sorted, void *workspace,
                     size_t workspace_bytes, mirec_stream_t stream);


int mirec_ssm_forward(const float *out, const float *emb, int64_t n_nodes,
                      int64_t n_users, int32_t dim, int64_t batch, int32_t n_neg,
                      const int32_t *users, const int32_t *pos, const int32_t *neg,
                      float temp, float grad_scale, float *coef, float *coef_pos,
                      float *terms, float *reg, float *g_u, int32_t *keys,
                      int32_t *vals, mirec_stream_t stream);

int mirec_ssm_keys(const int32_t *users, const int32_t *pos, const int32_t *neg,
                   int64_t batch, int32_t n_neg, int64_t n_users, int32_t *keys,
                   mirec_stream_t stream);

int mirec_ssm_seed_workspace(int64_t batch, int32_t n_neg, int64_t n_nodes, size_t *bytes);

int mirec_ssm_seed(const float *out, const float *emb, int64_t n_nodes, int64_t n_users,
                   int32_t dim, int64_t batch, int32_t n_neg, const int32_t *users,
                   const float *coef, const float *coef_pos, const float *g_u,
                   const int32_t *keys, const int32_t *vals, float decay,
                   float grad_scale, int32_t n_layers, int32_t *slot, float *seed_p,
                   float *seed_e, int32_t *keys_sorted, void *workspace,
                   size_t workspace_bytes, mirec_stream_t stream);


int mirec_ssm_shared_keys(const int32_t *users, const int32_t *pos, const int32_t *shared,
                          int64_t batch, int64_t m, int64_t n_users, int32_t *keys,
                          mirec_stream_t stream);

int mirec_ssm_shared_mask(const mirec_csr_t *csr, const int32_t *users, int64_t batch,
                          const int32_t *pos, const int32_t *shared, int64_t m,
                          int64_t n_users, uint8_t *mask, mirec_stream_t stream);

int mirec_ssm_shared_forward(const float *out, const float *emb, int64_t n_nodes,
                             int64_t n_users, int32_t dim, int64_t batch, int64_t m,
                             const int32_t *users, const int32_t *pos, const int32_t *shared,
                             const uint8_t *mask, float temp, float grad_scale, float *coef,
                             float *coef_pos, float *terms, float *reg, float *reg_shared,
                             float *g, int32_t *keys, int32_t *vals, mirec_stream_t stream);

int mirec_ssm_shared_loss(const float *terms, const float *reg, const float *reg_shared,
                          int64_t batch, int64_t m, float decay, float *loss_out,
                          float *loss_accum, mirec_stream_t stream);

int mirec_ssm_shared_seed_workspace(int64_t batch, int64_t m, int64_t n_nodes, size_t *bytes);

int mirec_ssm_shared_seed(const float *out, const float *emb, int64_t n_nodes, int64_t n_users,
                          int32_t dim, int64_t batch, int64_t m, const int32_t *users,
                          const float *coef_pos, const float *g, const int32_t *keys,
                          const int32_t *vals, float decay, float grad_scale, int32_t n_layers,
                          int32_t *slot, float *seed_p, float *seed_e, int32_t *keys_sorted,
                          void *workspace, size_t workspace_bytes, mirec_stream_t stream);

int mirec_shared_sample(int64_t m_items, int64_t n_sets, int64_t m, uint64_t seed,
                        uint64_t offset, int32_t *out, mirec_stream_t stream);


int mirec_adam_dense(float *param, const float *grad, float *exp_avg,
                     float *exp_avg_sq, int64_t n,
                     const mirec_adam_hparams_t *h, mirec_stream_t stream);

int mirec_adam_multi(int32_t count, float *const *params, const float *const *grads,
                     float *const *exp_avg, float *const *exp_avg_sq,
// ... 375 lines not shown
```

Baseline: 578,400 positive-edges/s.

## Filter sparse-seed propagation with an LDS-resident seed bitmap

Adds a compact per-node seed bitmap, possibly coarsened by a shift to fit a shared-memory budget, which is populated during frontier construction. A new seeded propagation kernel loads it into LDS and uses it to skip neighbour gathers for non-seed columns in later sparse layers. The aim is to replace the global bytemap and slot lookups per edge with cheap LDS bit tests and to compact the lanes that remain. It adds clearing and setting work in the frontier kernels, and it can waste LDS or occupancy when the bitmap is coarse or large.

```diff
diff --git a/furusato_recommend_amd/_lib.py b/furusato_recommend_amd/_lib.py
--- a/furusato_recommend_amd/_lib.py
+++ b/furusato_recommend_amd/_lib.py
@@ -57,6 +57,11 @@
 
 class Drop(Structure):
     _fields_ = [("keep_prob", c_float), ("transposed", c_int32), ("seed", c_uint64)]
+
+
+class SeedBits(Structure):
+    _fields_ = [("bits", c_void_p), ("split", c_int64), ("shift", c_int32 * 2),
+                ("words", c_int32 * 2)]
 
 
 class Sweep(Structure):
@@ -146,6 +151,11 @@
     "mirec_frontier": (c_int, [POINTER(CSR), c_void_p, c_int64, c_void_p, c_void_p, c_void_p,
                                c_int64, c_int64, c_void_p, c_void_p, c_void_p, c_void_p,
                                c_void_p, c_int32, c_void_p]),
+    "mirec_seed_bits_sizeof": (c_size_t, []),
+    "mirec_frontier_bits": (c_int, [POINTER(CSR), c_void_p, c_int64, c_void_p, c_void_p, c_void_p,
+                                    c_int64, c_int64, c_void_p, c_void_p, c_void_p, c_void_p,
+                                    c_void_p, c_int32, POINTER(SeedBits), c_void_p]),
+    "mirec_propagate_seeded": (c_int, [POINTER(CSR), POINTER(Prop), POINTER(SeedBits), c_void_p]),
     "mirec_mask_compact_pair": (c_int, [c_void_p, c_void_p, c_void_p, c_int64, c_void_p, c_void_p,
                                         c_void_p, c_void_p, c_void_p, c_void_p]),
     "mirec_small_sort_workspace": (c_int, [c_int64, POINTER(c_size_t)]),
@@ -455,6 +465,8 @@
         raise ImportError("struct layout mismatch: mirec_sweep_wave_t")
     if lib.mirec_sweep_pace_sizeof() != ctypes.sizeof(SweepPace):
         raise ImportError("struct layout mismatch: mirec_sweep_pace_t")
+    if lib.mirec_seed_bits_sizeof() != ctypes.sizeof(SeedBits):
+        raise ImportError("struct layout mismatch: mirec_seed_bits_t")
     return lib
 
 
diff --git a/furusato_recommend_amd/csrc/common.h b/furusato_recommend_amd/csrc/common.h
--- a/furusato_recommend_amd/csrc/common.h
+++ b/furusato_recommend_amd/csrc/common.h
@@ -64,6 +64,33 @@
 __device__ __forceinline__ void st4(float *p, float4 v) {
   *reinterpret_cast<float4 *>(p) = v;
 }
+struct SeedBitsK {
+  uint32_t *bits;
+  int32_t split;
+  int32_t shift0, shift1;
+  int32_t words0, words1;
+};
+__device__ __forceinline__ uint32_t seed_bit_pos(const SeedBitsK &f, int32_t node) {
+  const bool hi = node >= f.split;
+  const uint32_t b = hi ? (uint32_t)(node - f.split) >> f.shift1 : (uint32_t)node >> f.shift0;
+  return (hi ? (uint32_t)f.words0 * 32u : 0u) + b;
+}
+inline bool seed_bits_valid(const mirec_seed_bits_t *s, int64_t n_rows) {
+  if (s->bits == nullptr || ((uintptr_t)s->bits & 3u) != 0) return false;
+  if (s->split < 0 || s->split > n_rows || n_rows > INT32_MAX) return false;
+  const int64_t n[2] = {s->split, n_rows - s->split};
+  for (int r = 0; r < 2; ++r) {
+    if (s->shift[r] < 0 || s->shift[r] > 31 || s->words[r] < 0 || s->words[r] > (1 << 26))
+      return false;
+    if ((((int64_t)s->words[r] * 32) << s->shift[r]) < n[r]) return false;
+  }
+  return true;
+}
+inline SeedBitsK seed_bits_k(const mirec_seed_bits_t *s) {
+  return SeedBitsK{s->bits, (int32_t)s->split, s->shift[0], s->shift[1], s->words[0],
+                   s->words[1]};
+}
+
 constexpr int kRowRounds = 4;
 inline int row_lg(int64_t d4) {
   int lg = 0;
diff --git a/furusato_recommend_amd/csrc/frontier.hip b/furusato_recommend_amd/csrc/frontier.hip
--- a/furusato_recommend_amd/csrc/frontier.hip
+++ b/furusato_recommend_amd/csrc/frontier.hip
@@ -45,16 +45,22 @@
                    : (i < 2 * batch ? n_users + pos[i - batch] : n_users + neg[i - 2 * batch]);
 }
 
+__device__ __forceinline__ void set_seed_bit(const SeedBitsK &sb, int32_t node) {
+  const uint32_t pos = seed_bit_pos(sb, node);
+  atomicOr(sb.bits + (pos >> 5), 1u << (pos & 31u));
+}
+
 __global__ __launch_bounds__(256) void frontier_self_kernel(
     int64_t n_rows, const int32_t *__restrict__ keys, int64_t n_keys,
     const int32_t *__restrict__ users, const int32_t *__restrict__ pos,
     const int32_t *__restrict__ neg, int64_t batch, int64_t n_users, uint8_t *bm_self,
-    uint8_t *bm_hop, int32_t *self_list, int32_t *self_count) {
+    uint8_t *bm_hop, int32_t *self_list, int32_t *self_count, SeedBitsK sb) {
   const int64_t i = (int64_t)blockIdx.x * blockDim.x + threadIdx.x;
   const int64_t node = key_node(i, keys, n_keys, users, pos, neg, batch, n_users);
   const bool valid = node >= 0 && node < n_rows;
   const bool first = valid && test_and_set(bm_self, node);
   if (valid) bm_hop[node] = 1;
+  if (first && sb.bits != nullptr) set_seed_bit(sb, (int32_t)node);
   const int32_t off = block_reserve(first ? 1 : 0, self_count);
   if (first) self_list[off] = (int32_t)node;
 }
@@ -87,7 +93,7 @@
     int32_t split, const int32_t *__restrict__ keys, int64_t n_keys,
     const int32_t *__restrict__ users, const int32_t *__restrict__ pos,
     const int32_t *__restrict__ neg, int64_t batch, int64_t n_users, uint8_t *bm_self,
-    uint8_t *bm_hop) {
+    uint8_t *bm_hop, SeedBitsK sb) {
   const int lane = threadIdx.x & 63;
   const int64_t i = (int64_t)blockIdx.x * kWaves + (threadIdx.x >> 6);
   const int64_t node = key_node(i, keys, n_keys, users, pos, neg, batch, n_users);
@@ -95,6 +101,7 @@
   if (lane == 0) {
     bm_self[node] = 1;
     bm_hop[node] = 1;
+    if (sb.bits != nullptr) set_seed_bit(sb, (int32_t)node);
   }
   const int64_t beg = rowptr[node], end = rowptr[node + 1];
   if (split > 0 && end - beg > split) return;
@@ -592,7 +599,23 @@
                               uint8_t *bm_hop, int32_t *self_list, int32_t *self_count,
                               int32_t *zero_counts, int32_t n_zero_counts,
                               mirec_stream_t stream) {
-  using namespace mirec;
+  return mirec_frontier_bits(c, keys, n_keys, users, pos, neg, batch, n_users, bm_self, bm_hop,
+                             self_list, self_count, zero_counts, n_zero_counts, nullptr, stream);
+}
+
+extern "C" size_t mirec_seed_bits_sizeof(void) { return sizeof(mirec_seed_bits_t); }
+
+extern "C" int mirec_frontier_bits(const mirec_csr_t *c, const int32_t *keys, int64_t n_keys,
+                                   const int32_t *users, const int32_t *pos, const int32_t *neg,
+                                   int64_t batch, int64_t n_users, uint8_t *bm_self,
+                                   uint8_t *bm_hop, int32_t *self_list, int32_t *self_count,
+                                   int32_t *zero_counts, int32_t n_zero_counts,
+                                   const mirec_seed_bits_t *bits, mirec_stream_t stream) {
+  using namespace mirec;
+  MIREC_CHECK_ARG(c != nullptr && (bits == nullptr || seed_bits_valid(bits, c->n_rows)));
+  SeedBitsK sb = {};
+  if (bits != nullptr) sb = seed_bits_k(bits);
+  const size_t bit_bytes = 4 * ((size_t)sb.words0 + (size_t)sb.words1);
   MIREC_CHECK_ARG(c && c->rowptr && c->col && bm_self && bm_hop);
   MIREC_CHECK_ARG(keys != nullptr || (users && pos && neg && batch >= 0 && n_users >= 0));
   MIREC_CHECK_ARG(self_list == nullptr || self_count != nullptr);
@@ -603,7 +626,13 @@
   const size_t bytes16 = (bytes + 15) / 16 * 16;
   int32_t *sc = self_list != nullptr ? self_count : nullptr;
   if (bm_hop == bm_self + bytes16 && ((uintptr_t)bm_self & 15u) == 0) {
-    const int64_t n16 = (int64_t)(2 * bytes16 / 16);
+    int64_t n16 = (int64_t)(2 * bytes16 / 16);
+    if (bit_bytes > 0) {
+      if ((uint8_t *)sb.bits == bm_hop + bytes16 && bit_bytes % 16 == 0)
+        n16 += (int64_t)(bit_bytes / 16);
+      else
+        MIREC_HIP(hipMemsetAsync(sb.bits, 0, bit_bytes, st));
+    }
     const unsigned blocks = (unsigned)std::max<int64_t>(1, std::min<int64_t>((n16 + 255) / 256, 1024));
     hipLaunchKernelGGL(frontier_clear_kernel, dim3(blocks), dim3(256), 0, st,
                        reinterpret_cast<uint4 *>(bm_self), n16, sc, zero_counts, n_zero_counts);
@@ -613,6 +642,7 @@
     MIREC_HIP(hipMemsetAsync(bm_hop, 0, bytes, st));
     if (sc != nullptr) MIREC_HIP(hipMemsetAsync(sc, 0, 4, st));
     if (n_zero_counts > 0) MIREC_HIP(hipMemsetAsync(zero_counts, 0, 4 * (size_t)n_zero_counts, st));
+    if (bit_bytes > 0) MIREC_HIP(hipMemsetAsync(sb.bits, 0, bit_bytes, st));
   }
   const int64_t n = keys != nullptr ? n_keys : 3 * batch;
   const int32_t split = c->n_seg > 0 ? c->split : 0;
@@ -620,7 +650,7 @@
     if (n > 0) {
       hipLaunchKernelGGL(frontier_self_kernel, dim3((n + 255) / 256), dim3(256), 0, st, c->n_rows,
                          keys, n_keys, users, pos, neg, batch, n_users, bm_self, bm_hop,
-                         self_list, self_count);
+                         self_list, self_count, sb);
       MIREC_LAUNCH_CHECK();
       hipLaunchKernelGGL(frontier_expand_kernel, dim3((n + kWaves - 1) / kWaves), dim3(256), 0,
                          st, c->rowptr, c->col, split, self_list, self_count, bm_hop);
@@ -629,7 +659,7 @@
   } else if (n > 0) {
     hipLaunchKernelGGL(frontier_keys_kernel, dim3((n + kWaves - 1) / kWaves), dim3(256), 0, st,
                        c->rowptr, c->col, c->n_rows, split, keys, n_keys, users, pos, neg, batch,
-                       n_users, bm_self, bm_hop);
+                       n_users, bm_self, bm_hop, sb);
     MIREC_LAUNCH_CHECK();
   }
   if (c->n_seg > 0 && n > 0) {
diff --git a/furusato_recommend_amd/csrc/prop.hip b/furusato_recommend_amd/csrc/prop.hip
--- a/furusato_recommend_amd/csrc/prop.hip
+++ b/furusato_recommend_amd/csrc/prop.hip
@@ -318,6 +318,177 @@
   }
 }
 
+struct SeededK {
+  SeedBitsK bits;
+  int64_t last;
+};
+
+template <int D>
+constexpr int seeded_wide_chunks() {
+  return D >= 256 ? 2 : 4;
+}
+template <int D>
+constexpr int seeded_narrow_chunks() {
+  constexpr int n = 64 / (D / 4);
+  return n < 2 ? 2 : (n > 4 ? 4 : n);
+}
+
+template <int D, int UNROLL, bool NARROW>
+__device__ __forceinline__ float4 seeded_chunk(const PropK &a, float4 acc, int cnt, int myr,
+                                               float myw, int lane) {
+  constexpr int LPR = D / 4;
+  constexpr int G = 64 / LPR;
+  constexpr int W = NARROW ? LPR : 64;
+  const int grp = lane / LPR;
+  const int sub = lane % LPR;
+  const int l0 = NARROW ? grp * LPR : 0;
+  const int me = NARROW ? sub : lane;
+  const bool ok = myr >= 0;
+  const unsigned long long bal = __ballot(ok);
+  const unsigned long long m = (W == 64) ? bal : ((bal >> l0) & ((1ull << (W & 63)) - 1ull));
+  const int nv = __popcll(m);
+  if (nv == 0) return acc;
+  if (nv < cnt) {
+    const int below = __popcll(m & ((1ull << me) - 1ull));
+    const int dst = l0 + (ok ? below : nv + (me - below));
+    myr = __builtin_amdgcn_ds_permute(dst << 2, myr);
+    myw = __int_as_float(__builtin_amdgcn_ds_permute(dst << 2, __float_as_int(myw)));
+  }
+  if (myr < 0) {
+    myr = 0;
+    myw = 0.f;
+  }
+  for (int k = 0; k < nv; k += (NARROW ? 1 : G) * UNROLL) {
+    float4 v[UNROLL];
+    float w[UNROLL];
+#pragma unroll
+    for (int u = 0; u < UNROLL; ++u) {
+      const int idx = NARROW ? k + u : k + u * G + grp;
+      const int srcl = l0 + (idx & (W - 1));
+      const int j = __shfl(myr, srcl);
+      w[u] = __shfl(myw, srcl);
+      if (idx < nv)
+        v[u] = ld4(a.seed_in + (int64_t)j * D + sub * 4);
+      else
+        v[u] = f4_zero();
+    }
+#pragma unroll
+    for (int u = 0; u < UNROLL; ++u) acc = f4_fma(w[u], v[u], acc);
+  }
+  return acc;
+}
+
+template <int D, int UNROLL, bool NARROW, int NR>
+__device__ __forceinline__ float4 gather_seeded(const PropK &a, const SeededK &f,
+                                                const uint32_t *bits, int64_t beg, int deg,
+                                                int rounds, int lane) {
+  constexpr int LPR = D / 4;
+  constexpr int W = NARROW ? LPR : 64;
+  const int me = NARROW ? lane % LPR : lane;
+  const int32_t *cp = a.col + beg;
+  const int lim = (int)min(f.last - beg, (int64_t)0x7fffffff);
+  float4 acc = f4_zero();
+#pragma unroll 1
+  for (int it = 0, off = me; it < rounds; ++it, off += NR * W) {
+    int c[NR], s[NR];
+    float w[NR];
+    bool pass[NR];
+#pragma unroll
+    for (int r = 0; r < NR; ++r) c[r] = cp[min(off + r * W, lim)];
+#pragma unroll
+    for (int r = 0; r < NR; ++r) {
+      const uint32_t pos = seed_bit_pos(f.bits, c[r]);
+      pass[r] = off + r * W < deg && ((bits[pos >> 5] >> (pos & 31u)) & 1u) != 0u;
+      const int j = pass[r] ? c[r] : 0;
+      s[r] = a.slot[j];
+      w[r] = a.dinv[j];
+    }
+#pragma unroll
+    for (int r = 0; r < NR; ++r) {
+      const int cnt = max(0, min(W, deg - (off - me + r * W)));
+      acc = seeded_chunk<D, UNROLL, NARROW>(a, acc, cnt, pass[r] ? s[r] : -1, w[r], lane);
+    }
+  }
+  return acc;
+}
+
+template <int D, int UNROLL>
+__device__ __forceinline__ void seeded_wave_row(const PropK &a, const SeededK &f,
+                                                const uint32_t *bits, int32_t row, int64_t beg,
+                                                int deg, int lane) {
+  constexpr int LPR = D / 4;
+  constexpr int NRW = seeded_wide_chunks<D>();
+  const int rounds = __builtin_amdgcn_readfirstlane((deg + NRW * 64 - 1) / (NRW * 64));
+  float4 s = gather_seeded<D, UNROLL, false, NRW>(a, f, bits, beg, deg, rounds, lane);
+  s = combine_groups<D>(s);
+  if (lane < LPR) row_epilogue<D>(a, row, s, lane % LPR);
+}
+
+template <int D, int UNROLL>
+__device__ __forceinline__ void seeded_work(const PropK &a, const SeededK &f) {
+  constexpr int LPR = D / 4;
+  constexpr int G = 64 / LPR;
+  constexpr int NARROW_UNROLL = UNROLL < 4 ? 4 : UNROLL;
+  constexpr int NRN = seeded_narrow_chunks<D>();
+  extern __shared__ uint32_t seeded_bits[];
+  const int n_words = f.bits.words0 + f.bits.words1;
+  for (int i = threadIdx.x; i < n_words; i += 256) seeded_bits[i] = f.bits.bits[i];
+  __syncthreads();
+  const int wid = __builtin_amdgcn_readfirstlane(threadIdx.x >> 6);
+  const int64_t n_wide = a.wide_list != nullptr ? (int64_t)*a.wide_count : 0;
+  const int64_t wide_blocks = (n_wide + kWavesPerBlock - 1) / kWavesPerBlock;
+  const int64_t nrows = *a.row_count;
+  const int64_t row_waves = (nrows + G - 1) / G;
+  const int64_t total = wide_blocks + (row_waves + kWavesPerBlock - 1) / kWavesPerBlock;
+#pragma unroll 1
+  for (int64_t b = blockIdx.x; b < total; b += gridDim.x) {
+    int lane = threadIdx.x & 63;
+    asm volatile("" : "+v"(lane));
+    lane &= 63;
+    const int sub = lane % LPR;
+    const int grp = lane / LPR;
+    if (b < wide_blocks) {
+      const int64_t i = b * kWavesPerBlock + wid;
+      if (i >= n_wide) continue;
+      const int32_t row = a.wide_list[i];
+      const int64_t beg = a.rowptr[row], end = a.rowptr[row + 1];
+      seeded_wave_row<D, UNROLL>(a, f, seeded_bits, row, beg, (int)(end - beg), lane);
+      continue;
+    }
+    const int64_t w = (b - wide_blocks) * kWavesPerBlock + wid;
+    if (w >= row_waves) continue;
+    const int64_t idx = w * G + grp;
+    bool have = idx < nrows;
+    const int32_t row = a.row_list[have ? idx : 0];
+    const int64_t beg = a.rowptr[row], end = a.rowptr[row + 1];
+    have = have && a.row_mask[row] != 0;
+    const int deg = have ? (int)(end - beg) : 0;
+    if (G > 1 && __ballot(deg > a.narrow_max) == 0ull) {
+      int rounds = (deg + NRN * LPR - 1) / (NRN * LPR);
+#pragma unroll
+      for (int m = LPR; m < 64; m <<= 1) rounds = max(rounds, __shfl_xor(rounds, m));
+      rounds = __builtin_amdgcn_readfirstlane(rounds);
+      float4 s = gather_seeded<D, NARROW_UNROLL, true, NRN>(a, f, seeded_bits, beg, deg, rounds,
+                                                            lane);
+      if (have) row_epilogue<D>(a, row, s, sub);
+    } else {
+#pragma unroll 1
+      for (int g = 0; g < G; ++g) {
+        const int src = g * LPR;
+        if (!__shfl((int)have, src)) continue;
+        seeded_wave_row<D, UNROLL>(a, f, seeded_bits, __shfl(row, src),
+                                   __shfl((long long)beg, src), __shfl(deg, src), lane);
+      }
+    }
+  }
+}
+
+template <int D, int UNROLL>
+__global__ __launch_bounds__(256) __attribute__((amdgpu_waves_per_eu(7, 8)))
+MIREC_NO_PK_F32 void prop_seeded_kernel(PropK a, SeededK f) {
+  seeded_work<D, UNROLL>(a, f);
+}
+
 template <int D, bool SCALED>
 __global__ __launch_bounds__(256) MIREC_NO_PK_F32 void prop_finalize(PropK a, const int32_t *long_rows,
                                                      const int64_t *long_segptr, int64_t n_long) {
@@ -743,6 +914,39 @@
     const auto fin = scaled ? prop_finalize<D, true> : prop_finalize<D, false>;
     hipLaunchKernelGGL(fin, dim3((unsigned)c->n_long), dim3(256), 0, st, k, c->long_rows,
                        c->long_segptr, c->n_long);
+    MIREC_LAUNCH_CHECK();
+  }
+  return MIREC_OK;
+}
+
+constexpr size_t kSeededLdsMax = 64 * 1024;
+
+template <int D, int UNROLL>
+static int launch_seeded(PropK k, const mirec_seed_bits_t *sb, int64_t nnz, int64_t list_cap,
+                         hipStream_t st) {
+  constexpr int G = 64 / (D / 4);
+  SeededK f;
+  f.bits = seed_bits_k(sb);
+  f.last = nnz - 1;
+  const size_t lds = 4 * ((size_t)f.bits.words0 + (size_t)f.bits.words1);
+  const auto kernel = prop_seeded_kernel<D, UNROLL>;
+  static thread_local size_t cached_lds = 0;
+  static thread_local int64_t cached_resident = 0;
+  if (cached_resident == 0 || cached_lds != lds) {
+    int dev = 0, cus = 0, per_cu = 0;
+    MIREC_HIP(hipGetDevice(&dev));
+    MIREC_HIP(hipDeviceGetAttribute(&cus, hipDeviceAttributeMultiprocessorCount, dev));
+    MIREC_HIP(hipOccupancyMaxActiveBlocksPerMultiprocessor(
+        &per_cu, reinterpret_cast<const void *>(kernel), 256, lds));
+    cached_resident = (int64_t)std::max(per_cu, 1) * std::max(cus, 1);
+    cached_lds = lds;
+  }
+  const int64_t row_waves = (list_cap + G - 1) / G;
+  int64_t blocks = (row_waves + kWavesPerBlock - 1) / kWavesPerBlock;
+  if (k.wide_list != nullptr) blocks += (list_cap + kWavesPerBlock - 1) / kWavesPerBlock;
+  blocks = std::min(blocks, cached_resident);
+  if (blocks > 0) {
+    hipLaunchKernelGGL(kernel, dim3((unsigned)blocks), dim3(256), lds, st, k, f);
     MIREC_LAUNCH_CHECK();
   }
   return MIREC_OK;
@@ -964,7 +1168,8 @@
                      const mirec_sweep_wave_t *wi, const mirec_sweep_wave_t *wu,
                      mirec_stream_t stream, const mirec_drop_t *drop = nullptr,
                      const mirec_sweep_pace_t *pace = nullptr,
-                     const SweepStamp *stamp = nullptr) {
+                     const SweepStamp *stamp = nullptr,
+                     const mirec_seed_bits_t *seeded = nullptr) {
   MIREC_CHECK_ARG(c != nullptr && p != nullptr);
   if (pace != nullptr) {
     MIREC_CHECK_ARG(pace->ws != nullptr);
@@ -1063,6 +1268,18 @@
     if (sweep_wave_valid(c, wu, 0, wi->row0)) return launch_sweep_wave<64>(k, wu, st, pace, 1);
     return launch_head<64, 4>(c, k, wi->row0, st);
   }
+  if (seeded != nullptr) {
+    switch (p->dim) {
+      case 4: return launch_seeded<4, 1>(k, seeded, c->nnz, cap, st);
+      case 8: return launch_seeded<8, 1>(k, seeded, c->nnz, cap, st);
+      case 16: return launch_seeded<16, 1>(k, seeded, c->nnz, cap, st);
+      case 32: return launch_seeded<32, 2>(k, seeded, c->nnz, cap, st);
+      case 64: return launch_seeded<64, 4>(k, seeded, c->nnz, cap, st);
+      case 128: return launch_seeded<128, 4>(k, seeded, c->nnz, cap, st);
+      case 256: return launch_seeded<256, 4>(k, seeded, c->nnz, cap, st);
+    }
+    return MIREC_ERR_DIM;
+  }
   switch (p->dim) {
     case 4: return launch_prop<4, 1>(c, k, cap, p->in_mode, st, dropout);
     case 8: return launch_prop<8, 1>(c, k, cap, p->in_mode, st, dropout);
@@ -1120,6 +1337,21 @@
 extern "C" int mirec_propagate_drop(const mirec_csr_t *c, const mirec_prop_t *p,
                                     const mirec_drop_t *drop, mirec_stream_t stream) {
   return mirec::propagate(c, p, nullptr, nullptr, nullptr, stream, drop);
+}
+
+extern "C" int mirec_propagate_seeded(const mirec_csr_t *c, const mirec_prop_t *p,
+                                      const mirec_seed_bits_t *filter, mirec_stream_t stream) {
+  using namespace mirec;
+  MIREC_CHECK_ARG(c != nullptr && p != nullptr);
+  const bool shape = filter != nullptr && p->in_mode == MIREC_IN_SPARSE &&
+                     p->row_list != nullptr && p->in_mask == nullptr && c->val == nullptr &&
+                     c->n_seg == 0 && c->nnz > 0 && p->scale_src == nullptr &&
+                     p->scale_dst == nullptr && p->scale_next == nullptr;
+  if (!shape) return mirec_propagate(c, p, stream);
+  MIREC_CHECK_ARG(seed_bits_valid(filter, c->n_rows));
+  const size_t lds = 4 * ((size_t)filter->words[0] + (size_t)filter->words[1]);
+  if (lds == 0 || lds > kSeededLdsMax) return mirec_propagate(c, p, stream);
+  return propagate(c, p, nullptr, nullptr, nullptr, stream, nullptr, nullptr, nullptr, filter);
 }
 
 extern "C" int mirec_edge_keep_mask(const int64_t *rowptr, const int32_t *col, int64_t n_rows,
diff --git a/furusato_recommend_amd/engine.py b/furusato_recommend_amd/engine.py
--- a/furusato_recommend_amd/engine.py
+++ b/furusato_recommend_amd/engine.py
@@ -15,6 +15,28 @@
 SWEEP_USERS = True
 LAYER_SUM_ROWS = "self"
 SWEEP_PACE = {"items": (8, 16, 16), "users": (4, 4, 16)}
+SEEDED_FIRST = True
+SEEDED_LDS_BYTES = 16 * 1024
+
+
+def seed_bit_layout(n0: int, n1: int, budget: int):
+    def words(n, s):
+        return -(-(-(-n // (1 << s))) // 32)
+
+    def fit(n, share):
+        s = 0
+        while s < 31 and words(n, s) > 1 and 4 * words(n, s) > share:
+            s += 1
+        return s
+    n = (int(n0), int(n1))
+    small = 0 if n[0] <= n[1] else 1
+    shift, w = [0, 0], [0, 0]
+    shift[small] = fit(n[small], int(budget) * 7 // 8)
+    w[small] = words(n[small], shift[small])
+    shift[1 - small] = fit(n[1 - small], int(budget) - 4 * w[small])
+    w[1 - small] = words(n[1 - small], shift[1 - small])
+    w[1] += -(w[0] + w[1]) % 4
+    return tuple(shift), tuple(w)
 
 
 def prop_launch_bytes(in_mode: int, n_nodes: int, nnz: int, dim: int, *, slot=False,
@@ -217,8 +239,11 @@
             [torch.empty(N, D, **f32)] if self.L == 1 else []
         self.slot = torch.full((N,), -1, **i32)
         words = (N + 15) // 16 * 4
-        self._bm = torch.zeros(2, words, **i32)
-        self.bm_self, self.bm_hop = self._bm[0], self._bm[1]
+        nu = graph.n_users if graph.m_items > 0 else N
+        self._bit_cap = (-(-nu // 32), -(-(N - nu) // 32))
+        self._bm = torch.zeros(2 * words + (sum(self._bit_cap) + 3) // 4 * 4, **i32)
+        self.bm_self, self.bm_hop = self._bm[:words], self._bm[words:2 * words]
+        self._seed_bits_mem = self._bm[2 * words:]
         B3 = max((2 + self.n_neg) * self.max_batch, 2 * self.max_batch + self.n_shared)
         self.self_list = torch.zeros(B3, **i32)
         self.self_count = torch.zeros(1, **i32)
@@ -239,6 +264,10 @@
         self._pace_ws = None
         self._wave_layouts()
         self.sparse_filter = "auto"
+        self.seeded_first = SEEDED_FIRST
+        self._seeded_lds_bytes = SEEDED_LDS_BYTES
+        self._seed_bits = None
+        self._bits_ready = False
         self._masks_ready = False
         self.narrow_max = 64
         self.seed_p = torch.empty(B3, D, **f32)
@@ -320,7 +349,8 @@
     def _prop(self, *, in_mode, x_in=None, seed_in=None, seed=None, addend=None, seed2=None,
               divisor=1.0, out=None, xs_out=None, adam=None, param=None, graph=None,
               row_mask=None, in_mask=None, row_list=None, row_count=None, row_list_cap=0,
-              out_mask=None, wide_list=None, wide_count=None, direction="fwd", stamp=None):
+              out_mask=None, wide_list=None, wide_count=None, direction="fwd", stamp=None,
+              seeded=False):
         g = graph or self.g
         p = Prop()
         if g.scale_src is not None:
@@ -378,6 +408,11 @@
                              seed=self._drop[1])
             check(lib.mirec_propagate_drop(g.csr_ptr(), ctypes.byref(p), ctypes.byref(drop),
                                            _lib.stream_handle()), "propagate_drop")
+        elif seeded:
+            p.in_mask = None
+            check(lib.mirec_propagate_seeded(g.csr_ptr(), ctypes.byref(p),
+                                             ctypes.byref(self._seed_bits_struct()),
+                                             _lib.stream_handle()), "propagate_seeded")
         elif on and self._sweep_form == "wave":
             wi, wu = self.sweep_wave, self.sweep_wave_users if self._sweep_users else None
             pace = self._pace_struct()
@@ -434,26 +469,28 @@
         g = self.g
         lists = self.prune and self.use_hop_list
         zc, nz = (self.list_counts.data_ptr(), 4) if lists else (None, 0)
+        sb = ctypes.byref(self._seed_bits_struct()) if self._seeded_ok() else None
         if keys is not None:
             n = int(n_keys)
             if self.self_list.shape[0] < n:
                 self.self_list = torch.zeros(n, dtype=torch.int32, device=g.device)
-            check(lib.mirec_frontier(g.csr_ptr(), keys.data_ptr(), n, None, None, None,
-                                     0, g.n_users, self.bm_self.data_ptr(),
-                                     self.bm_hop.data_ptr(), self.self_list.data_ptr(),
-                                     self.self_count.data_ptr(), zc, nz, _lib.stream_handle()),
-                  "frontier")
+            check(lib.mirec_frontier_bits(g.csr_ptr(), keys.data_ptr(), n, None, None, None,
+                                          0, g.n_users, self.bm_self.data_ptr(),
+                                          self.bm_hop.data_ptr(), self.self_list.data_ptr(),
+                                          self.self_count.data_ptr(), zc, nz, sb,
+                                          _lib.stream_handle()), "frontier")
             self._self_cap = n
         else:
             B = int(users.shape[0])
             if B > self.max_batch:
                 raise ValueError(f"batch {B} > engine max_batch {self.max_batch}")
-            check(lib.mirec_frontier(g.csr_ptr(), None, 0, users.data_ptr(), pos.data_ptr(),
-                                     neg.data_ptr(), B, g.n_users,
-                                     self.bm_self.data_ptr(), self.bm_hop.data_ptr(),
-                                     self.self_list.data_ptr(), self.self_count.data_ptr(),
-                                     zc, nz, _lib.stream_handle()), "frontier")
+            check(lib.mirec_frontier_bits(g.csr_ptr(), None, 0, users.data_ptr(), pos.data_ptr(),
+                                          neg.data_ptr(), B, g.n_users,
+                                          self.bm_self.data_ptr(), self.bm_hop.data_ptr(),
+                                          self.self_list.data_ptr(), self.self_count.data_ptr(),
+                                          zc, nz, sb, _lib.stream_handle()), "frontier")
             self._self_cap = 3 * B
+        self._bits_ready = sb is not None
         if lists:
             check(lib.mirec_mask_compact_pair(self.bm_self.data_ptr(), self.bm_hop.data_ptr(),
                                               self._wide_bits().data_ptr(), g.n_nodes,
@@ -550,6 +587,40 @@
         if f == "auto":
             f = "bytemap" if self._self_cap > (2 + self.n_neg) * self.max_batch else "slot"
         return self.bm_self if f == "bytemap" else None
+
+    @property
+    def seeded_lds_bytes(self) -> int:
+        return self._seeded_lds_bytes
+
+    @seeded_lds_bytes.setter
+    def seeded_lds_bytes(self, nbytes: int):
+        if int(nbytes) < 8:
+            raise ValueError(f"seeded_lds_bytes: at least 8, got {nbytes!r}")
+        self._seeded_lds_bytes = int(nbytes)
+        self._seed_bits = None
+        self._bits_ready = False
+
+    def seed_bit_shifts(self):
+        sb = self._seed_bits_struct()
+        return sb.shift[0], sb.shift[1]
+
+    def _seed_bits_struct(self):
+        if self._seed_bits is None:
+            g = self.g
+            nu = g.n_users if g.m_items > 0 else g.n_nodes
+            shift, words = seed_bit_layout(nu, g.n_nodes - nu, self._seeded_lds_bytes)
+            sb = _lib.SeedBits(bits=self._seed_bits_mem.data_ptr(), split=nu)
+            sb.shift[0], sb.shift[1] = shift
+            sb.words[0], sb.words[1] = words
+            self._seed_bits = sb
+        return self._seed_bits
+
+    def _seeded_ok(self) -> bool:
+        g = self.g
+        return bool(self.seeded_first and self.L >= 2 and self.prune and self.use_hop_list
+                    and self.sparse_filter != "dense" and g.n_users > 0 and g.m_items > 0
+                    and g._coo is None and g.n_seg == 0 and g.val is None
+                    and g.scale_src is None and self._drop is None)
 
     def static_row_lists(self, bm: torch.Tensor) -> dict:
         g = self.g
@@ -851,6 +922,8 @@
                     else:
                         kw = dict(in_mode=IN_SPARSE, seed_in=seed_p,
                                   in_mask=self._sparse_filter(), **rows)
+                        if l > 0 and self._bits_ready and self._seeded_ok():
+                            kw["seeded"] = True
                 else:
                     kw = dict(in_mode=IN_PRESCALED, x_in=self.xs[(L - 2 - l) % 2],
                               in_mask=self.bm_hop if (self.prune and l == L - 2) else None)
@@ -865,7 +938,7 @@
         check(lib.mirec_bpr_seed_reset(self.slot.data_ptr(), keys_sorted.data_ptr(), n_keys,
                                        _lib.stream_handle()), "bpr_seed_reset")
         self._seeds = None
-        self._masks_ready = False
+        self._masks_ready = self._bits_ready = False
         self._x0s_token = self._token(emb) if (adam is not None and L > 0 and last_rows is None
                                                and self.reuse_prescaled) else None
 
diff --git a/include/mirec.h b/include/mirec.h
--- a/include/mirec.h
+++ b/include/mirec.h
@@ -236,6 +236,25 @@
                    uint8_t *bm_hop, int32_t *self_list, int32_t *self_count,
                    int32_t *zero_counts, int32_t n_zero_counts, mirec_stream_t stream);
 
+typedef struct mirec_seed_bits {
+  uint32_t *bits;
+  int64_t split;
+  int32_t shift[2];
+  int32_t words[2];
+} mirec_seed_bits_t;
+
+size_t mirec_seed_bits_sizeof(void);
+
+int mirec_frontier_bits(const mirec_csr_t *csr, const int32_t *keys, int64_t n_keys,
+                        const int32_t *users, const int32_t *pos, const int32_t *neg,
+                        int64_t batch, int64_t n_users, uint8_t *bm_self,
+                        uint8_t *bm_hop, int32_t *self_list, int32_t *self_count,
+                        int32_t *zero_counts, int32_t n_zero_counts,
+                        const mirec_seed_bits_t *sb, mirec_stream_t stream);
+
+int mirec_propagate_seeded(const mirec_csr_t *csr, const mirec_prop_t *p,
+                           const mirec_seed_bits_t *filter, mirec_stream_t stream);
+
 int mirec_mask_compact_pair(const uint8_t *bm_a, const uint8_t *bm_b, const uint32_t *wide_bits,
                             int64_t n_rows, int32_t *list_a, int32_t *wide_a, int32_t *list_b,
                             int32_t *wide_b, int32_t *counts, mirec_stream_t stream);
```

After: 593,600 positive-edges/s (median of 6 runs). +2.6%, better.
